# nihofm/volren

Measured on AMD Instinct MI355X. Metric: Msamples/s (pixels x spp / s), volume path tracing, higher is better.
Workload: dtype f32; 1 GPU; BASELINE configs[1] 'c2': smoke.brick, no transfer function, 1024x1024, 1024 spp, seed 42, fov 40; parallelism=1 GPU, 1 fused launch(es)/frame (sample pool budget 64 GiB)

## Files before the change

### volren_amd/csrc/capi.cpp

```cpp
#include "../../include/volren_amd.h"

#include <algorithm>
#include <cmath>
#include <cstring>
#include <filesystem>
#include <functional>
#include <iostream>
#include <stdexcept>
#include <memory>
#include <string>
#include <vector>

#include "imageio.h"
#include "renderer.h"
#include "sharded.h"
#include "vr_device.h"
#include "vr_math_probe.h"

struct vr_renderer {
    vr::RendererHIP impl;
    int device = 0;
};

struct vr_sharded {
// ... 107 lines not shown

int vr_load_envmap(vr_renderer* r, const char* path) {
    NEED(r);
    if (!path) return fail(VR_ERR_ARG, "null path");
    return guard([&] { use_device(r); r->impl.environment = std::make_shared<vr::Environment>(std::string(path)); r->impl.sample = 0; });
}

int vr_load_transferfunc(vr_renderer* r, const char* path) {
    NEED(r);
    if (!path) return fail(VR_ERR_ARG, "null path");
    return guard([&] {
        use_device(r);
        r->impl.transferfunc = std::make_shared<vr::TransferFunction>(std::string(path));
        r->impl.show_environment = false;
        r->impl.sample = 0;
    });
}

static void install_grid(vr_renderer* r, const char* name, const std::shared_ptr<vr::Grid>& grid, int unit_cube) {
    const std::string n = name ? name : "density";
    auto& R = r->impl;
    if (n == "density") {
        R.volume = std::make_shared<vr::Volume>(grid);
        if (unit_cube) { R.density_scale = 1.f; R.scale_and_move_to_unit_cube(); }
    } else {
        if (!R.volume || R.volume->grids.empty()) throw std::runtime_error("set the density grid before '" + n + "'");
        R.volume->update_grid_frame(R.volume->grid_frame_counter, grid, n);
    }
    R.sample = 0;
}

int vr_set_volume_dense(vr_renderer* r, const char* name, const float* voxels, int nx, int ny, int nz, const float* transform, int unit_cube) {
    NEED(r);
    if (!voxels || nx <= 0 || ny <= 0 || nz <= 0) return fail(VR_ERR_ARG, "bad dense grid arguments");
    return guard([&] {
        use_device(r);
        auto g = std::make_shared<vr::DenseGrid>((uint32_t)nx, (uint32_t)ny, (uint32_t)nz, voxels);
        if (transform) memcpy(g->transform.m, transform, 64);
        install_grid(r, name, g, unit_cube);
    });
}

int vr_volume_add_grid_frame_dense(vr_renderer* r, const char* name, const float* voxels, int nx, int ny, int nz, const float* transform) {
    NEED(r);
    if (!voxels || nx <= 0 || ny <= 0 || nz <= 0) return fail(VR_ERR_ARG, "bad dense grid arguments");
    return guard([&] {
        auto g = std::make_shared<vr::DenseGrid>((uint32_t)nx, (uint32_t)ny, (uint32_t)nz, voxels);
        if (transform) memcpy(g->transform.m, transform, 64);
        if (!r->impl.volume) r->impl.volume = std::make_shared<vr::Volume>();
        r->impl.volume->add_grid_frame(g, name ? name : "density");
        r->impl.sample = 0;
    });
}
int vr_volume_update_grid_frame_dense(vr_renderer* r, int frame, const char* name, const float* voxels, int nx, int ny, int nz, const float* transform) {
    NEED(r);
    if (!voxels || nx <= 0 || ny <= 0 || nz <= 0 || frame < 0) return fail(VR_ERR_ARG, "bad dense grid arguments");
    return guard([&] {
        if (!r->impl.volume || (size_t)frame >= r->impl.volume->n_grid_frames()) throw std::out_of_range("vr_volume_update_grid_frame_dense: no such frame");
        auto g = std::make_shared<vr::DenseGrid>((uint32_t)nx, (uint32_t)ny, (uint32_t)nz, voxels);
        if (transform) memcpy(g->transform.m, transform, 64);
        r->impl.volume->update_grid_frame((size_t)frame, g, name ? name : "density");
        r->impl.sample = 0;
    });
}
int vr_volume_n_grid_frames(vr_renderer* r, int* n) {
    NEED(r);
    if (!n) return fail(VR_ERR_ARG, "null output");
    *n = r->impl.volume ? (int)r->impl.volume->n_grid_frames() : 0;
    return VR_OK;
}

int vr_set_volume_dense_f16(vr_renderer* r, const char* name, const uint16_t* voxels, int nx, int ny, int nz, const float* transform, int unit_cube) {
    NEED(r);
    if (!voxels || nx <= 0 || ny <= 0 || nz <= 0) return fail(VR_ERR_ARG, "bad dense grid arguments");
    return guard([&] {
        use_device(r);
        auto g = std::make_shared<vr::DenseGridF16>((uint32_t)nx, (uint32_t)ny, (uint32_t)nz, voxels);
        if (transform) memcpy(g->transform.m, transform, 64);
        install_grid(r, name, g, unit_cube);
    });
}

int vr_set_volume_brick(vr_renderer* r, const char* name, const float* transform, const uint32_t nb[3], const float min_maj[2],
                        const uint32_t* indirection, const uint32_t* range, const uint32_t atlas_dim[3], const uint8_t* atlas,
                        int n_mips, const uint32_t* const* mips, const uint32_t (*mip_dims)[3], int unit_cube) {
    NEED(r);
    if (!nb || !min_maj || !indirection || !range || !atlas_dim || !atlas || n_mips < 0 || n_mips > 3) return fail(VR_ERR_ARG, "bad brick grid arguments");
    return guard([&] {
        use_device(r);
        auto g = std::make_shared<vr::BrickGrid>();
        if (transform) memcpy(g->transform.m, transform, 64);
        g->n_bricks = { nb[0], nb[1], nb[2] };
        g->min_maj = { min_maj[0], min_maj[1] };
        const size_t n = (size_t)nb[0] * nb[1] * nb[2];
        g->indirection = vr::Buf3D<uint32_t>(nb[0], nb[1], nb[2]);
        g->range = vr::Buf3D<uint32_t>(nb[0], nb[1], nb[2]);
        memcpy(g->indirection.data.data(), indirection, n * 4);
        memcpy(g->range.data.data(), range, n * 4);
        if ((atlas_dim[0] % 8) || (atlas_dim[1] % 8) || (atlas_dim[2] % 8)) throw std::runtime_error("atlas dimensions must be multiples of 8");
        g->atlas = vr::Buf3D<uint8_t>(atlas_dim[0], atlas_dim[1], atlas_dim[2]);
        memcpy(g->atlas.data.data(), atlas, g->atlas.data.size());
        uint64_t cnt = 0;
        for (size_t i = 0; i < n; ++i) cnt += (vr::half2float(range[i] & 0xFFFFu) != vr::half2float(range[i] >> 16));
        g->brick_counter = cnt;
        for (int m = 0; m < n_mips; ++m) {
            vr::Buf3D<uint32_t> b(mip_dims[m][0], mip_dims[m][1], mip_dims[m][2]);
            memcpy(b.data.data(), mips[m], b.data.size() * 4);
            g->range_mipmaps.push_back(std::move(b));
        }
        install_grid(r, name, g, unit_cube);
    });
}

int vr_set_envmap(vr_renderer* r, const float* rgb, int w, int h) {
    NEED(r);
    if (!rgb || w <= 0 || h <= 0) return fail(VR_ERR_ARG, "bad envmap arguments");
    return guard([&] { use_device(r); r->impl.environment = std::make_shared<vr::Environment>(rgb, w, h); r->impl.sample = 0; });
}

int vr_set_transferfunc(vr_renderer* r, const float* rgba, int n) {
    NEED(r);
    return guard([&] {
        use_device(r);
        if (n <= 0 || !rgba) { r->impl.transferfunc.reset(); r->impl.sample = 0; return; }
        std::vector<vr::vec4> lut;
        for (int i = 0; i < n; ++i) lut.emplace_back(rgba[4 * i], rgba[4 * i + 1], rgba[4 * i + 2], rgba[4 * i + 3]);
        r->impl.transferfunc = std::make_shared<vr::TransferFunction>(lut);
        r->impl.sample = 0;
    });
}

int vr_set_int(vr_renderer* r, const char* name, int v) {
    NEED(r);
    if (!name) return fail(VR_ERR_ARG, "null name");
    return guard([&] {
        auto& R = r->impl;
        const std::string n = name;
        if (n == "sample") { R.sample = v; R.drop_tile_samples(); }
        else if (n == "sppx") R.sppx = v;
        else if (n == "seed") R.seed = v;
        else if (n == "bounces") R.bounces = v;
        else if (n == "show_environment") R.show_environment = v != 0;
        else if (n == "tonemapping") R.tonemapping = v != 0;
        else if (n == "integrator") R.integrator = v;
        else if (n == "fast_math") R.fast_math = v != 0;
        else if (n == "variance") { if (v < 0 || v > 1) throw std::runtime_error("variance: 0 (off) or 1 (keep the per-pixel second moments)"); R.variance = v; }
        else if (n == "denoise_iterations") {
            if (v < 0 || v > vr::kDenoiseMaxIterations) throw std::runtime_error("denoise_iterations must be in [0, 10]");
            R.denoise_iterations = v;
        }
        else if (n == "coalesce_trace") { R.flush_pending(); R.coalesce_trace = v != 0; }
        else if (n == "majorant_layout") { if (v < -1 || v > 1) throw std::runtime_error("majorant_layout: -1 (per grid, chosen at commit), 0 (linear), 1 (4x4x4-cell blocks)"); R.majorant_layout = v; }
        else if (n == "tf_float_atlas") R.tf_float_atlas = v != 0;
        else if (n == "gpu_encoder") R.gpu_encoder = v != 0;
        else if (n == "sample_pool_mb") { if (v < 16 || v > 65536) throw std::runtime_error("sample_pool_mb must be in [16, 65536] (item indices of a sub-launch are 32-bit: < 2^32 RGBA32F items)"); R.sample_pool_bytes = (size_t)v << 20; }
        else if (n == "launch_target_ms") { if (v < 0) throw std::runtime_error("launch_target_ms must be >= 0 (0 = no sizing by time)"); R.launch_target_ms = v; }
        else if (n == "order_tiles") { if (v < 0 || v > 2) throw std::runtime_error("order_tiles: 0 (never), 1 (tile subsets), 2 (always)"); R.order_tiles = v; }
        else if (n == "grid_frame_counter") {
            if (!R.volume || v < 0 || (size_t)v >= R.volume->n_grid_frames()) throw std::runtime_error("grid_frame_counter out of range");
            R.volume->grid_frame_counter = (size_t)v;
        } else throw std::runtime_error("unknown int parameter: " + n);
    });
}

int vr_get_int(vr_renderer* r, const char* name, int* v) {
    NEED(r);
    if (!name || !v) return fail(VR_ERR_ARG, "null argument");
    return guard([&] {
        auto& R = r->impl;
        const std::string n = name;
        if (n == "sample") *v = R.sample;
        else if (n == "sppx") *v = R.sppx;
        else if (n == "seed") *v = R.seed;
        else if (n == "bounces") *v = R.bounces;
        else if (n == "show_environment") *v = R.show_environment ? 1 : 0;
        else if (n == "tonemapping") *v = R.tonemapping ? 1 : 0;
        else if (n == "integrator") *v = R.integrator;
        else if (n == "fast_math") *v = R.fast_math ? 1 : 0;
        else if (n == "variance") *v = R.variance;
        else if (n == "denoise_iterations") *v = R.denoise_iterations;
        else if (n == "coalesce_trace") *v = R.coalesce_trace ? 1 : 0;
        else if (n == "majorant_layout") *v = R.majorant_layout;
        else if (n == "majorant_blocked") {
            vr::SceneParams P; R.fill_params(P); *v = P.density.maj_blocked;
        }
        else if (n == "kernel_variant" || n == "kernel_variant_reason") {
            vr::SceneParams P; R.fill_params(P);
            int why = 0; const int variant = vr::pathtrace_variant_of(P, &why);
            *v = n == "kernel_variant" ? variant : why;
        }
        else if (n == "env_div_safe") *v = R.environment && R.environment->cdf_div_safe ? 1 : 0;
        else if (n == "env_compact") *v = R.environment && R.environment->envmap_rgbe ? 1 : 0;
        else if (n == "pending_samples") *v = R.pending_samples();
        else if (n == "tf_float_atlas") *v = R.tf_float_atlas ? 1 : 0;
        else if (n == "gpu_encoder") *v = R.gpu_encoder ? 1 : 0;
        else if (n == "sample_pool_mb") *v = (int)(R.sample_pool_bytes >> 20);
        else if (n == "launch_target_ms") *v = R.launch_target_ms;
        else if (n == "order_tiles") *v = R.order_tiles;
        else if (n == "grid_frame_counter") *v = R.volume ? (int)R.volume->grid_frame_counter : 0;
        else if (n == "n_grid_frames") *v = R.volume ? (int)R.volume->n_grid_frames() : 0;
        else if (n == "last_launches") *v = R.last_launches;
        else if (n == "adaptive_rounds") *v = R.adaptive_rounds;
        else if (n == "width") *v = R.resolution.x;
        else if (n == "height") *v = R.resolution.y;
        else throw std::runtime_error("unknown int parameter: " + n);
    });
}

namespace {
struct FloatField { float* ptr; int count; };
FloatField float_field(vr::RendererHIP& R, const std::string& n) {
    if (n == "tonemap_exposure") return { &R.tonemap_exposure, 1 };
    if (n == "tonemap_gamma") return { &R.tonemap_gamma, 1 };
    if (n == "albedo") return { &R.albedo.x, 3 };
    if (n == "phase") return { &R.phase, 1 };
    if (n == "density_scale") return { &R.density_scale, 1 };
    if (n == "emission_scale") return { &R.emission_scale, 1 };
    if (n == "vol_clip_min") return { &R.vol_clip_min.x, 3 };
    if (n == "vol_clip_max") return { &R.vol_clip_max.x, 3 };
    if (n == "cam_pos") return { &R.camera.pos.x, 3 };
    if (n == "cam_dir") return { &R.camera.dir.x, 3 };
    if (n == "cam_up") return { &R.camera.up.x, 3 };
    if (n == "cam_fov") return { &R.camera.fov_degree, 1 };
    if (n == "env_strength") { if (!R.environment) throw std::runtime_error("no environment"); return { &R.environment->strength, 1 }; }
    if (n == "env_transform") { if (!R.environment) throw std::runtime_error("no environment"); return { R.environment->transform.m, 9 }; }
    if (n == "tf_window_left") { if (!R.transferfunc) throw std::runtime_error("no transfer function"); return { &R.transferfunc->window_left, 1 }; }
    if (n == "tf_window_width") { if (!R.transferfunc) throw std::runtime_error("no transfer function"); return { &R.transferfunc->window_width, 1 }; }
    if (n == "volume_transform") { if (!R.volume) throw std::runtime_error("no volume"); return { R.volume->transform.m, 16 }; }
    if (n == "denoise_sigma") return { R.denoise_sigma, 5 };
    if (n == "denoise_alpha") return { &R.denoise_alpha, 1 };
    throw std::runtime_error("unknown float parameter: " + n);
}
}

int vr_set_float(vr_renderer* r, const char* name, const float* values, int count) {
    NEED(r);
    if (!name || !values) return fail(VR_ERR_ARG, "null argument");
    return guard([&] {
        auto& R = r->impl;
        const std::string n = name;
        if (n == "env_rot") {
            if (count != 1) throw std::runtime_error("env_rot takes 1 value");
            if (!R.environment) throw std::runtime_error("no environment");
            R.environment->transform = vr::rotation_axis(values[0], 1);
            return;
        }
        if (n == "albedo" && count == 1) { R.albedo = vr::vec3(values[0]); return; }
        if (n == "denoise_sigma") {
            if (count != 5) throw std::runtime_error("denoise_sigma takes 5 values (colour, normal, depth, coverage, albedo)");
            for (int i = 0; i < 5; ++i)
                if (!(values[i] >= vr::kDenoiseSigmaMin && values[i] <= vr::kDenoiseSigmaMax))
                    throw std::runtime_error("denoise_sigma: every value must be in [2^-60, 2^60]");
        }
        if (n == "denoise_alpha" && count == 1 && !(values[0] >= vr::kTemporalAlphaMin && values[0] <= vr::kTemporalAlphaMax))
            throw std::runtime_error("denoise_alpha must be in [2^-20, 1]");
        const FloatField f = float_field(R, n);
        if (count != f.count) throw std::runtime_error("wrong value count for " + n);
        memcpy(f.ptr, values, sizeof(float) * (size_t)count);
    });
}

int vr_get_float(vr_renderer* r, const char* name, float* values, int count) {
    NEED(r);
    if (!name || !values) return fail(VR_ERR_ARG, "null argument");
    return guard([&] {
        const FloatField f = float_field(r->impl, name);
        if (count != f.count) throw std::runtime_error(std::string("wrong value count for ") + name);
        memcpy(values, f.ptr, sizeof(float) * (size_t)count);
    });
}

int vr_commit(vr_renderer* r) { NEED(r); return guard([&] { use_device(r); r->impl.commit(); }); }
int vr_reset(vr_renderer* r) { NEED(r); return guard([&] { r->impl.reset(); }); }
int vr_scale_and_move_to_unit_cube(vr_renderer* r) { NEED(r); return guard([&] { r->impl.scale_and_move_to_unit_cube(); }); }

int vr_trace(vr_renderer* r) { NEED(r); return guard([&] { use_device(r); r->impl.trace(); }); }
int vr_flush(vr_renderer* r) { NEED(r); return guard([&] { use_device(r); r->impl.flush_pending(); }); }
int vr_render(vr_renderer* r, int spp) { NEED(r); return guard([&] { use_device(r); r->impl.render(spp); }); }

int vr_synchronize(vr_renderer* r) {
    NEED(r);
    return guard([&] {
        use_device(r);
        r->impl.synchronize();
        r->impl.check_watchdog();
    });
}

int vr_last_kernel_ms(vr_renderer* r, double* ms) {
    NEED(r);
    if (!ms) return fail(VR_ERR_ARG, "null argument");
    return guard([&] { use_device(r); *ms = r->impl.last_kernel_ms(); });
}

int vr_last_pathtrace_ms(vr_renderer* r, double* ms) {
    NEED(r);
    if (!ms) return fail(VR_ERR_ARG, "null output");
    return guard([&] { use_device(r); *ms = r->impl.last_pathtrace_ms(); });
}

int vr_framebuffer(vr_renderer* r, float* out) {
    NEED(r);
    if (!out) return fail(VR_ERR_ARG, "null argument");
    return guard([&] { use_device(r); r->impl.download(out); });
}
int vr_render_features(vr_renderer* r, int spp) {
    NEED(r);
    if (vr_device_count() <= 0) return fail(VR_ERR_NO_DEVICE, "no HIP device available (libvolren_amd has no CPU path)");
    return guard([&] { use_device(r); r->impl.render_features(spp); });
}
int vr_features(vr_renderer* r, float* out) {
    NEED(r);
    if (!out) return fail(VR_ERR_ARG, "null argument");
    if (vr_device_count() <= 0) return fail(VR_ERR_NO_DEVICE, "no HIP device available (libvolren_amd has no CPU path)");
    return guard([&] { use_device(r); r->impl.download_features(out); });
}
int vr_variance(vr_renderer* r, float* out) {
    NEED(r);
    if (!out) return fail(VR_ERR_ARG, "null argument");
    if (vr_device_count() <= 0) return fail(VR_ERR_NO_DEVICE, "no HIP device available (libvolren_amd has no CPU path)");
    return guard([&] { use_device(r); r->impl.download_variance(out); });
}
int vr_denoise(vr_renderer* r) {
    NEED(r);
    if (vr_device_count() <= 0) return fail(VR_ERR_NO_DEVICE, "no HIP device available (libvolren_amd has no CPU path)");
    return guard([&] { use_device(r); r->impl.denoise(); });
}
int vr_denoise_temporal(vr_renderer* r) {
    NEED(r);
    if (vr_device_count() <= 0) return fail(VR_ERR_NO_DEVICE, "no HIP device available (libvolren_amd has no CPU path)");
    return guard([&] { use_device(r); r->impl.denoise_temporal(); });
}
int vr_denoise_history_reset(vr_renderer* r) {
    NEED(r);
    if (vr_device_count() <= 0) return fail(VR_ERR_NO_DEVICE, "no HIP device available (libvolren_amd has no CPU path)");
    return guard([&] { use_device(r); r->impl.flush_pending(); r->impl.drop_history(); });
}
int vr_denoise_history(vr_renderer* r, float* rgba_out, float* var_out, float* length_out) {
    NEED(r);
    if (vr_device_count() <= 0) return fail(VR_ERR_NO_DEVICE, "no HIP device available (libvolren_amd has no CPU path)");
    return guard([&] { use_device(r); r->impl.download_history(rgba_out, var_out, length_out); });
}
// ... 277 lines not shown
```

### volren_amd/csrc/renderer.cpp

```cpp
#include "renderer.h"

#include <algorithm>
#include <cfloat>
#include <cmath>
#include <cstdlib>
#include <cstring>
#include <iostream>

#include "vr_adaptive.h"
#include "vr_device.h"
#include "vr_math.h"
#include "vr_probe.h"

namespace vr {

mat3 Camera::view_inverse() const {
    const vec3 f = normalize(dir);
    const vec3 s = normalize(cross(f, up));
    const vec3 u = cross(s, f);
    mat3 r(0.0f);
    r.m[0] = s.x; r.m[1] = s.y; r.m[2] = s.z;
    r.m[3] = u.x; r.m[4] = u.y; r.m[5] = u.z;
    r.m[6] = -f.x; r.m[7] = -f.y; r.m[8] = -f.z;
    return r;
// ... 299 lines not shown
}

static float camera_z(float fov_degree) { return -0.5f / tan_(0.5f * kPi * fov_degree / 180.f); }

void RendererHIP::fill_params(SceneParams& P) {
    if (!volume || volume->grids.empty() || density_grids.empty())
        throw std::runtime_error("RendererHIP::trace: no volume committed");
    if (volume->grid_frame_counter >= density_grids.size())
        throw std::runtime_error("RendererHIP::trace: grid_frame_counter out of range (commit() after changing the volume)");
    memset(&P, 0, sizeof P);
    Uniforms& u = P.u;
    u.bounces = bounces;
    u.seed = seed;
    u.show_environment = show_environment ? 1 : 0;
    copy3(u.cam_pos, camera.pos);
    u.cam_fov = camera.fov_degree;
    const mat3 ct = camera.view_inverse();
    memcpy(u.cam_transform, ct.m, sizeof ct.m);
    P.cam_z = camera_z(camera.fov_degree);
    const auto [bb_min, bb_max] = volume->AABB();
    const auto [mn, maj] = volume->minorant_majorant();
    copy3(u.vol_bb_min, bb_min + vol_clip_min * (bb_max - bb_min));
    copy3(u.vol_bb_max, bb_min + vol_clip_max * (bb_max - bb_min));
    u.vol_minorant = mn * density_scale;
    u.vol_majorant = maj * density_scale;
    u.vol_inv_majorant = 1.f / (maj * density_scale);
    copy3(u.vol_albedo, albedo);
    u.vol_phase_g = phase;
    u.vol_density_scale = density_scale;
    u.vol_emission_scale = emission_scale;
    u.vol_emission_norm = majorant_emission > 0.f ? 1.f / std::fmax(majorant_emission, 1e-4f) : 1.f;
    const BrickGridHIP& density = density_grids[volume->grid_frame_counter];
    const mat4 dt = volume->transform * density.transform;
    const mat4 dti = inverse(dt);
    memcpy(u.vol_density_transform, dt.m, sizeof dt.m);
    memcpy(u.vol_density_inv_transform, dti.m, sizeof dti.m);
    P.density = make_view(density);
    if (volume->grid_frame_counter < emission_grids.size()) {
        const BrickGridHIP& emission = emission_grids[volume->grid_frame_counter];
        const mat4 et = volume->transform * emission.transform;
        const mat4 eti = inverse(et);
        memcpy(u.vol_emission_transform, et.m, sizeof et.m);
        memcpy(u.vol_emission_inv_transform, eti.m, sizeof eti.m);
        const mat4 efd = eti * dt;
        memcpy(P.emission_from_density, efd.m, sizeof efd.m);
        const bool scale_ok = u.vol_density_scale >= 1.0f / 65536.0f && u.vol_density_scale <= 16777216.0f;
        P.paired = (integrator == 0 && environment->cdf_div_safe && scale_ok && density.atlas_paired && density.atlas_paired == emission.atlas_paired) ? 1 : 0;
        if (P.paired) P.density = make_view(density, true, majorant_layout < 0 ? density.maj_blocked : majorant_layout == 1);
        P.emission = make_view(emission, P.paired != 0);
        u.has_emission = 1;
    }
    if (transferfunc) {
        u.use_tf = 1;
        u.tf_size = transferfunc->size();
        u.tf_window_left = transferfunc->window_left;
        u.tf_window_width = transferfunc->window_width;
        P.tf_lut = transferfunc->lut_ssbo->as<float>();
    }
    const mat3 eit = inverse(environment->transform);
    memcpy(u.env_transform, environment->transform.m, sizeof eit.m);
    memcpy(u.env_inv_transform, eit.m, sizeof eit.m);
    u.env_strength = environment->strength;
    u.env_imp_inv_dim[0] = u.env_imp_inv_dim[1] = 1.f / (float)environment->dimension();
    u.env_imp_base_mip = (int)std::floor(std::log2((float)environment->dimension()));
    P.envmap = environment->envmap->as<float>();
    P.env_rgbe = environment->envmap_rgbe ? environment->envmap_rgbe->as<uint32_t>() : nullptr;
    P.env_w = environment->width; P.env_h = environment->height;
    P.env_avg_w = environment->avg_importance; P.env_avg_w_set = 1;
    P.impmap = environment->impmap->as<float>();
    P.imp_dim = (int)environment->dimension();
    P.env_cdf = environment->cdf->as<float>();
    P.env_div_safe = environment->cdf_div_safe ? 1 : 0;
    u.resolution[0] = resolution.x; u.resolution[1] = resolution.y;
    u.integrator = integrator;
}

void RendererHIP::update_majorants(const LaunchInputs& in, BrickGridHIP& g) {
    const MajKey& k = in.maj;
    if (k.density_scale == maj_key_.density_scale && k.tf_version == maj_key_.tf_version &&
        k.wl == maj_key_.wl && k.ww == maj_key_.ww && k.frame == maj_key_.frame && k.blocked == maj_key_.blocked)
        return;
    launch_majorants(in.P, g.range_words->as<uint32_t>(), g.nb, g.mip_off, g.n_mips, g.mshift, g.majorant->as<float>(), g.majorant16->as<uint16_t>(), in.stream);
    VR_HIP(hipGetLastError());
    maj_key_ = k;
}

void RendererHIP::set_tiles(const std::vector<int32_t>& tile_ids) {
    flush_pending();
    tiles_host_ = tile_ids;
    tiles_dev_.reset();
    if (tile_ids.empty()) return;
    if (resolution.x > 0) {
        const int n_all = tile_count(resolution.x, resolution.y);
        for (int32_t t : tile_ids)
            if (t < 0 || t >= n_all) throw std::runtime_error("set_tiles: tile id out of range");
    }
    tiles_dev_ = make_device_buffer(tile_ids.size() * sizeof(int32_t));
    tiles_dev_->upload(tile_ids.data(), tile_ids.size() * sizeof(int32_t));
}

std::vector<int32_t> RendererHIP::costliest_first(const SceneParams& P, const std::vector<int32_t>& tile_ids, int n_tiles) const {
    const Uniforms& u = P.u;
    const int W = u.resolution[0], H = u.resolution[1], tiles_x = vr::tiles_x(W);
    std::vector<int32_t> ids(tile_ids);
    if (ids.empty()) { ids.resize((size_t)n_tiles); for (int i = 0; i < n_tiles; ++i) ids[(size_t)i] = i; }
    auto chord = [&](float px, float py) {
        float d[3] = { (px - 0.5f * (float)W) / (float)H, (py - 0.5f * (float)H) / (float)H, P.cam_z };
        float w[3];
        for (int i = 0; i < 3; ++i) w[i] = u.cam_transform[i] * d[0] + u.cam_transform[3 + i] * d[1] + u.cam_transform[6 + i] * d[2];
        const float len = std::sqrt(w[0] * w[0] + w[1] * w[1] + w[2] * w[2]);
        float t0 = 0.f, t1 = FLT_MAX;
        for (int i = 0; i < 3; ++i) {
            const float inv = 1.f / (w[i] / len);
            const float a = (u.vol_bb_min[i] - u.cam_pos[i]) * inv, b = (u.vol_bb_max[i] - u.cam_pos[i]) * inv;
            t0 = std::fmax(t0, std::fmin(a, b)); t1 = std::fmin(t1, std::fmax(a, b));
        }
        return t1 > t0 ? t1 - t0 : 0.f;
    };
    std::vector<float> cost(ids.size());
    for (size_t k = 0; k < ids.size(); ++k) {
        const float x0 = (float)((ids[k] % tiles_x) * 16), y0 = (float)((ids[k] / tiles_x) * 16);
        const float x1 = std::fmin(x0 + 16.f, (float)W), y1 = std::fmin(y0 + 16.f, (float)H);
        cost[k] = std::fmax(std::fmax(std::fmax(chord(x0, y0), chord(x1, y0)), std::fmax(chord(x0, y1), chord(x1, y1))), chord(0.5f * (x0 + x1), 0.5f * (y0 + y1)));
    }
    std::vector<int32_t> perm(ids.size());
    for (size_t k = 0; k < perm.size(); ++k) perm[k] = (int32_t)k;
    const size_t seg = (ids.size() + 7) / 8;
    for (size_t b = 0; b < ids.size(); b += seg)
        std::stable_sort(perm.begin() + (ptrdiff_t)b, perm.begin() + (ptrdiff_t)std::min(ids.size(), b + seg), [&](int32_t x, int32_t y) { return cost[(size_t)x] > cost[(size_t)y]; });
    std::vector<int32_t> ordered(ids.size());
    for (size_t k = 0; k < ids.size(); ++k) ordered[k] = ids[(size_t)perm[k]];
    return ordered;
}

const int32_t* RendererHIP::tile_order(const SceneParams& P, const std::vector<int32_t>& ids, int n_tiles) {
    const Uniforms& u = P.u;
    uint64_t key = 1469598103934665603ull;
    auto mix = [&key](const void* p, size_t nbytes) { const uint8_t* b = static_cast<const uint8_t*>(p); for (size_t i = 0; i < nbytes; ++i) { key ^= b[i]; key *= 1099511628211ull; } };
    mix(u.cam_pos, sizeof u.cam_pos); mix(u.cam_transform, sizeof u.cam_transform); mix(&P.cam_z, sizeof P.cam_z);
    mix(u.vol_bb_min, sizeof u.vol_bb_min); mix(u.vol_bb_max, sizeof u.vol_bb_max); mix(u.resolution, sizeof u.resolution); mix(&n_tiles, sizeof n_tiles);
    if (!ids.empty()) mix(ids.data(), ids.size() * sizeof(int32_t));
    key = key ? key : 1;
    if (order_dev_ && order_key_ == key && order_dev_->size_bytes() == (size_t)n_tiles * sizeof(int32_t)) return order_dev_->as<int32_t>();
    const std::vector<int32_t> ordered = costliest_first(P, ids, n_tiles);
    ensure_buffer(order_dev_, ordered.size() * sizeof(int32_t));
    order_dev_->upload(ordered.data(), ordered.size() * sizeof(int32_t), stream);
    order_key_ = key;
    return order_dev_->as<int32_t>();
}

bool RendererHIP::LaunchInputs::same_launch_as(const LaunchInputs& o) const {
    return memcmp(&P, &o.P, sizeof P) == 0 && frame == o.frame && maj.density_scale == o.maj.density_scale && maj.tf_version == o.maj.tf_version &&
           maj.wl == o.maj.wl && maj.ww == o.maj.ww && maj.blocked == o.maj.blocked && memcmp(tuning.thr, o.tuning.thr, sizeof tuning.thr) == 0 && tuning.stats == o.tuning.stats &&
           tuning.samples_per_unit == o.tuning.samples_per_unit && tuning.blocks_per_cu == o.tuning.blocks_per_cu && order_tiles == o.order_tiles &&
           launch_target_ms == o.launch_target_ms && fast_math == o.fast_math && variance == o.variance && sample_pool_bytes == o.sample_pool_bytes && stream == o.stream;
}

void RendererHIP::capture(LaunchInputs& in) {
    if (!color) throw std::runtime_error("RendererHIP::trace: no framebuffer (call resize first)");
    if (integrator == 2 && !transferfunc) throw std::runtime_error("RendererHIP::trace: integrator 2 (direct volume rendering) needs a transfer function");
    if (integrator < 0 || integrator > 3) throw std::runtime_error("RendererHIP::trace: unknown integrator");
    if (fast_math && transferfunc) throw std::runtime_error("RendererHIP::trace: fast_math is not available while a transfer function is bound (it misses the 1e-3 bound there); set fast_math 0");
    if (!volume || volume->grids.empty() || density_grids.empty()) throw std::runtime_error("RendererHIP::trace: no volume committed");
    if (volume->grid_frame_counter >= density_grids.size()) throw std::runtime_error("RendererHIP::trace: grid_frame_counter out of range (commit() after changing the volume)");
    {
        BrickGridHIP& g = density_grids[volume->grid_frame_counter];
        const bool build = transferfunc && tf_float_atlas && !g.dense && g.atlas && g.rng && !g.atlas_f32 && !g.atlas_f32_failed;
        const bool drop = (!transferfunc || !tf_float_atlas) && (g.atlas_f32 || g.atlas_f32_failed);
        if (build || drop) flush_pending();
        if (build) {
            try {
                const size_t n_blocks = g.atlas->size_bytes() / kBrickBlockBytes, want = n_blocks * 512u * sizeof(float);
                auto drop_others = [&] { for (BrickGridHIP& other : density_grids) if (&other != &g) other.atlas_f32.reset(); };
                size_t free_b = 0, total_b = 0;
                if (hipMemGetInfo(&free_b, &total_b) != hipSuccess) { (void)hipGetLastError(); free_b = ~(size_t)0; }
                if (want > free_b / 2) drop_others();
                try { g.atlas_f32 = make_device_buffer(want); }
                catch (const std::exception&) { (void)hipGetLastError(); drop_others(); g.atlas_f32 = make_device_buffer(want); }
                launch_decode_atlas(g.rng->as<float>(), g.atlas->as<uint8_t>(), g.atlas_f32->as<float>(), n_blocks, stream);
                VR_HIP(hipGetLastError());
            } catch (const std::exception& e) {
                (void)hipGetLastError();
                g.atlas_f32.reset();
                g.atlas_f32_failed = true;
                std::cerr << "volren_amd: no room for the decoded float atlas (" << (g.atlas->size_bytes() / kBrickBlockBytes * 2048u >> 20) << " MiB): transfer-function taps read the byte atlas (" << e.what() << ")" << std::endl;
            }
        }
        if (drop) { g.atlas_f32.reset(); g.atlas_f32_failed = false; }
    }
    fill_params(in.P);
    in.frame = volume->grid_frame_counter;
    in.maj = MajKey{};
    in.maj.density_scale = density_scale;
    in.maj.tf_version = transferfunc ? transferfunc->version : 0;
    in.maj.wl = transferfunc ? transferfunc->window_left : 0.f;
    in.maj.ww = transferfunc ? transferfunc->window_width : 0.f;
    in.maj.frame = in.frame;
    in.maj.blocked = in.P.density.maj_blocked;
    in.tuning = tuning;
    in.order_tiles = order_tiles; in.launch_target_ms = launch_target_ms; in.fast_math = fast_math ? 1 : 0; in.variance = variance != 0 ? 1 : 0;
    in.sample_pool_bytes = sample_pool_bytes;
    in.stream = stream;
    in.env = environment; in.tf = transferfunc;
    in.keep[0] = environment->envmap; in.keep[1] = environment->impmap; in.keep[2] = environment->cdf;
    in.keep[3] = transferfunc ? transferfunc->lut_ssbo : DeviceBufferPtr();
    in.keep[4] = environment->envmap_rgbe;
}

int RendererHIP::samples_per_launch(const LaunchInputs& in, int n_tiles) const {
    const size_t per_sample = pathtrace_pool_floats(in.tuning, n_tiles, 1) * sizeof(float);
    int per_launch = (int)std::max<size_t>(1, in.sample_pool_bytes / per_sample);
    const size_t lim = (size_t)0xFFFFFFFFu / ((size_t)n_tiles * 256u);
    per_launch = (int)std::min<size_t>((size_t)per_launch, lim > 8 ? lim - 8 : 1);
    if (per_launch > 32) per_launch -= per_launch % 32;
    return per_launch;
}

void RendererHIP::submit_tile_set(const LaunchInputs& in, int first, int n) {
    if (n <= 0) return;
    const int n_tiles = tiles_dev_ ? (int)tiles_host_.size() : tile_count(in.P.u.resolution[0], in.P.u.resolution[1]);
    const bool ordered = in.order_tiles >= 2 || (in.order_tiles == 1 && tiles_dev_);
    const int32_t* tiles = ordered ? tile_order(in.P, tiles_host_, n_tiles) : (tiles_dev_ ? tiles_dev_->as<int32_t>() : nullptr);
    submit(in, first, n, tiles, n_tiles);
}

void RendererHIP::submit(const LaunchInputs& in, int first, int n, const int32_t* tiles, int n_tiles) {
    if (n <= 0) return;
    const SceneParams& P = in.P;
    hipStream_t stream = in.stream;
    const bool has_tf = P.u.use_tf != 0;
    update_majorants(in, density_grids.at(in.frame));
    int per_launch = std::min(samples_per_launch(in, n_tiles), n);
    for (;;) {
        const size_t need = pathtrace_pool_floats(in.tuning, n_tiles, per_launch) * sizeof(float);
        if (pool_ && pool_->size_bytes() >= need) break;
        if (pool_) { VR_HIP(hipStreamSynchronize(stream)); pool_.reset(); }
        try { pool_ = make_device_buffer(need); break; }
        catch (const std::exception&) {
            (void)hipGetLastError();
            if (per_launch <= 1) throw;
            per_launch = std::max(1, per_launch / 2);
            if (per_launch > 32) per_launch -= per_launch % 32;
        }
    }
    if (!workspace_) {
        workspace_ = make_device_buffer(pathtrace_workspace_floats() * sizeof(float));
        if (const char* e = std::getenv("VR_TEST_POISON_WORKSPACE"); e && *e == '1') VR_HIP(hipMemsetAsync(workspace_->get(), 0xFF, workspace_->size_bytes(), stream));
    }
    if (const char* e = std::getenv("VR_TEST_POISON_WORKSPACE"); e && *e == '2') {
        VR_HIP(hipMemsetAsync(workspace_->get(), 0xFF, workspace_->size_bytes(), stream));
        VR_HIP(hipMemsetAsync(pool_->get(), 0xFF, pool_->size_bytes(), stream));
    }
    const int integ = P.u.integrator;
    const bool pt_kernel = !(integ == 3 || (integ == 2 && has_tf));
    const double px_samples = (double)n_tiles * 256.0;
    const uint64_t key = [&] {
        uint64_t h = 1469598103934665603ull;
        auto mix = [&h](const void* p, size_t nbytes) { const uint8_t* b = static_cast<const uint8_t*>(p); for (size_t i = 0; i < nbytes; ++i) { h ^= b[i]; h *= 1099511628211ull; } };
        const Uniforms& u = P.u;
        mix(&u.bounces, sizeof u.bounces); mix(u.vol_albedo, sizeof u.vol_albedo); mix(&u.vol_phase_g, sizeof u.vol_phase_g); mix(&u.vol_density_scale, sizeof u.vol_density_scale);
        mix(&u.use_tf, sizeof u.use_tf); mix(&u.tf_window_left, sizeof u.tf_window_left); mix(&u.tf_window_width, sizeof u.tf_window_width); mix(&u.integrator, sizeof u.integrator);
        mix(&u.has_emission, sizeof u.has_emission); mix(u.resolution, sizeof u.resolution); mix(u.vol_bb_min, sizeof u.vol_bb_min); mix(u.vol_bb_max, sizeof u.vol_bb_max);
        const size_t frame = in.frame; mix(&frame, sizeof frame); mix(&n_tiles, sizeof n_tiles);
        const uint64_t tfv = in.maj.tf_version; mix(&tfv, sizeof tfv);
        return h ? h : 1ull;
    }();
    auto cap_by_rate = [&](int planned) {
        if (in.launch_target_ms <= 0 || rate_samples_per_ms_ <= 0.0) return planned;
        const double cap = rate_samples_per_ms_ * (double)in.launch_target_ms / px_samples;
        int c = cap >= (double)planned ? planned : std::max(1, (int)cap);
        if (c > 32) c -= c % 32;
        return c;
    };
    int probe = 0;
    if (pt_kernel && in.launch_target_ms > 0) {
        harvest_rate(false);
        const bool known = rate_samples_per_ms_ > 0.0 && rate_key_ == key;
        if (!known && px_samples * (double)std::min(per_launch, n) > (double)(1u << 26)) {
            rate_samples_per_ms_ = 0.0;
            probe = (int)std::min<double>(32.0, std::max(1.0, (double)(1u << 24) / px_samples));
            probe = std::min(probe, n);
        } else per_launch = cap_by_rate(per_launch);
    }
    float* moments = nullptr;
    if (in.variance) {
        const size_t bytes = color->size_bytes();
        if (ensure_buffer(moments_, bytes)) {
            VR_HIP(hipMemsetAsync(moments_->get(), 0, bytes, stream));
            if (first > 0) moments_n_ = -1;
        }
        moments = moments_->as<float>();
        moments_n_ = first == 0 ? n : (moments_n_ == first ? first + n : -1);
    } else {
        moments_n_ = -1;
    }
    if (!keep_timing_) {
        VR_HIP(hipEventRecord(ev0_, stream));
        last_launches = 0;
        pt_events_used_ = 0;
    }
    for (int done = 0; done < n;) {
        ++last_launches;
        const int m = probe > 0 ? probe : std::min(per_launch, n - done);
        hipEvent_t eb = nullptr, ee = nullptr;
        if (pt_kernel) {
            while (pt_events_.size() < pt_events_used_ + 2) { hipEvent_t e; VR_HIP(hipEventCreate(&e)); pt_events_.push_back(e); }
            eb = pt_events_[pt_events_used_]; ee = pt_events_[pt_events_used_ + 1];
// ... 432 lines not shown
```

### volren_amd/csrc/vr_device.h

```cpp
#pragma once

#include <hip/hip_runtime.h>
#include <stdint.h>

#include "vr_denoise.h"
#include "vr_scene.h"
#include "vr_temporal.h"
#include "vr_tiles.h"

namespace vr {

struct PathtraceTuning {
    int32_t thr[8] = { 64, 0, 56, 0, 60, 60, 64, 0 };
    unsigned long long* stats = nullptr;
    int32_t samples_per_unit = 0;
    int32_t blocks_per_cu = 0;
};
PathtraceTuning default_tuning();
size_t pathtrace_pool_floats(const PathtraceTuning& T, int32_t n_tiles, int32_t n_samples);
size_t pathtrace_workspace_floats();
void launch_pathtrace(const PathtraceTuning& T, const SceneParams& P, float* fb, float* sample_pool, float* workspace, uint32_t* unit_counter, const int32_t* tiles, int32_t n_tiles,
                      int32_t first_sample, int32_t n_samples, uint32_t* status, hipStream_t stream, bool fast_math = false,
                      hipEvent_t ev_kernel_begin = nullptr, hipEvent_t ev_kernel_end = nullptr,
                      float* moments = nullptr);
constexpr uint32_t kFeatureLostStatus = 4u;
void launch_features(const SceneParams& P, const int32_t* tiles, int32_t n_tiles, int32_t spp, float* out, uint32_t* status, hipStream_t stream);
enum PathtraceVariantReason : int {
    VR_VARIANT_INTEGRATOR = 1,
    VR_VARIANT_ENV_DIVISION = 2,
    VR_VARIANT_DENSITY_SCALE = 4,
    VR_VARIANT_GRID_FORMS = 8
};
int pathtrace_variant_of(const SceneParams& P, int* why);
void launch_denoise_prepare(const float* moments, const float* features, int32_t W, int32_t H, int32_t n, float vscale, const int32_t* counts, float* v, float* guide,
                            hipStream_t stream);
void launch_denoise_atrous(const float* cin, const float* vin, const float* guide, int32_t W, int32_t H, int32_t step, const DenoiseSigma& sg,
                           float* cout, float* vout, hipStream_t stream);
void launch_denoise_temporal(const float* color, float* v, const float* guide, const float* hist_color, const float* hist_record, bool same_cam,
                             const TemporalCamera& cur, const TemporalCamera& prev, int32_t W, int32_t H, float alpha, float* out_color, float* out_record,
                             hipStream_t stream);
void launch_adaptive_error(const float* fb, const float* moments, const int32_t* tiles, const int32_t* counts, int32_t n_tiles, int32_t W, int32_t H, float* out,
                           hipStream_t stream);

void launch_tonemap(float* fb, int32_t w, int32_t h, float exposure, float gamma, hipStream_t stream);

void launch_pack_tiles(const float* fb, int32_t w, int32_t h, const int32_t* tiles, int32_t n_tiles, float* packed, hipStream_t stream);
void launch_unpack_tiles(const float* packed, const int32_t* tiles, int32_t n_tiles, float* fb, int32_t w, int32_t h, hipStream_t stream);
void launch_build_impmap(const float* envmap_rgba, int32_t env_w, int32_t env_h, int32_t dim, float* pyramid, hipStream_t stream);

void launch_build_env_cdf(const float* pyramid, int32_t dim, float* table, uint32_t* unsafe_flag, hipStream_t stream);

void launch_majorants(const SceneParams& P, const uint32_t* range_words_all_mips, const int32_t nb[3], const int32_t mip_off[4], int32_t n_mips,
                      const int32_t mshift[3], float* out_padded, uint16_t* out16_padded, hipStream_t stream);

void launch_encode_ranges(const float* dense, const int32_t dim[3], const int32_t nb[3], uint32_t* range, uint32_t* flag, hipStream_t stream);
void launch_encode_bricks(const float* dense, const int32_t dim[3], const int32_t nb[3], const uint32_t* range, const uint32_t* flag,
                          BrickRec* recs, float* rng, uint8_t* atlas, hipStream_t stream);
void launch_range_mip(const uint32_t* src, const int32_t sdim[3], uint32_t* dst, const int32_t ddim[3], hipStream_t stream);

void launch_pair_atlas(const uint8_t* atlas_density, const uint8_t* atlas_emission, uint8_t* out, size_t n_records, hipStream_t stream);

void launch_decode_atlas(const float* rng, const uint8_t* atlas, float* out, size_t n_records, hipStream_t stream);
void launch_math_probe(int32_t fn, const float* a, const float* b, float* out, int32_t n, hipStream_t stream);
void launch_math_sweep(int32_t fn, uint32_t first, float b, float* out, int32_t n, hipStream_t stream);
void launch_fast_math_sweep(int32_t fn, uint32_t first, float* out, int32_t n, hipStream_t stream);
void launch_probe(const SceneParams& P, int32_t what, int32_t form, const uint32_t* in, float* out, uint32_t n, hipStream_t stream);

}
```

### volren_amd/csrc/vr_launch.hip

```cpp
#include <hip/hip_runtime.h>

#include <algorithm>
#include <cstdlib>
#include <map>
#include <mutex>
#include <stdexcept>
#include <string>

#include "vr_device.h"
#include "vr_pathtrace.h"

namespace vr {

template <int INTEGRATOR>
__global__ void __launch_bounds__(256)
item_kernel(const SceneParams P, float* __restrict__ sbuf, const LaunchDesc D) {
    const uint32_t per_unit = (uint32_t)(D.spu * 64);
    const uint32_t g = blockIdx.x * 256u + threadIdx.x;
    const uint32_t u = g / per_unit, item = g - u * per_unit;
    if (u >= D.n_units) return;
    const WorkUnit wu = make_unit(D, P.u.resolution[0], u, sbuf);
    if ((int32_t)item >= wu.n_items) return;
    const int32_t px = wu.px0 + (int32_t)(item & 7u), py = wu.py0 + (int32_t)((item >> 3) & 7u);
    if (px >= P.u.resolution[0] || py >= P.u.resolution[1]) return;
    float L[4];
    if (INTEGRATOR == 2) dvr_sample(P, px, py, wu.first_sample + (int32_t)(item >> 6), L);
    else raymarch_path_sample(P, px, py, wu.first_sample + (int32_t)(item >> 6), L);
    reinterpret_cast<float4*>(sbuf)[wu.base + item] = pack4(L);
}

template <bool MOMENTS>
__global__ void __launch_bounds__(256)
accumulate_kernel(const float* __restrict__ sbuf, float* __restrict__ fb, float* __restrict__ moments, const int32_t* __restrict__ tiles, int32_t n_tiles,
                  int32_t W, int32_t H, int32_t first_sample, int32_t n_samples, int32_t spu) {
    const TilePixel q = wave_tiled_pixel(tiles ? tiles[blockIdx.x] : (int32_t)blockIdx.x, threadIdx.x, W);
    if (q.px >= W || q.py >= H) return;
    float4* texel = reinterpret_cast<float4*>(fb) + (size_t)q.py * W + q.px;
    float4* mtexel = MOMENTS ? reinterpret_cast<float4*>(moments) + (size_t)q.py * W + q.px : nullptr;
    float acc[4] = { 0.0f, 0.0f, 0.0f, 0.0f }, S[4] = { 0.0f, 0.0f, 0.0f, 0.0f };
    if (first_sample > 1) {
        unpack4(*texel, acc);
        if (MOMENTS) unpack4(*mtexel, S);
    }
    const float4* sb = reinterpret_cast<const float4*>(sbuf);
    for (int32_t k = 0; k < n_samples; ++k) {
        const int32_t chunk = k / spu, sl = k - chunk * spu;
        float L[4];
        unpack4(sb[pool_slot<size_t>((size_t)chunk, n_tiles, (size_t)blockIdx.x, (uint32_t)q.sub, spu, (size_t)sl, (uint32_t)q.lane)], L);
        const float a = 1.0f / (float)(first_sample + k);
        for (int32_t c = 0; c < 4; ++c) {
            const float x = sanitize(L[c]);
            const float mu = acc[c], mu1 = mix_(mu, x, a);
            if (MOMENTS) S[c] = mix_(S[c], (x - mu) * (x - mu1), a);
            acc[c] = mu1;
        }
    }
    *texel = pack4(acc);
    if (MOMENTS) *mtexel = pack4(S);
}

template <bool TF>
__global__ void __launch_bounds__(256)
features_kernel(const SceneParams P, const int32_t* __restrict__ tiles, int32_t spp, float* __restrict__ out, uint32_t* __restrict__ status) {
    const int32_t W = P.u.resolution[0], H = P.u.resolution[1];
    const TilePixel q = wave_tiled_pixel(tiles ? tiles[blockIdx.x] : (int32_t)blockIdx.x, threadIdx.x, W);
    if (q.px >= W || q.py >= H) return;
    float f[8];
    if (!feature_pixel<TF>(P, q.px, q.py, spp, f)) atomicOr(status, kFeatureLostStatus);
    float4* o = reinterpret_cast<float4*>(out) + 2u * ((size_t)q.py * W + q.px);
    o[0] = pack4(f);
    o[1] = pack4(f + 4);
}
void launch_features(const SceneParams& P, const int32_t* tiles, int32_t n_tiles, int32_t spp, float* out, uint32_t* status, hipStream_t stream) {
    if (n_tiles <= 0 || spp <= 0) return;
    if (P.u.use_tf) hipLaunchKernelGGL(features_kernel<true>, dim3((unsigned)n_tiles), dim3(256), 0, stream, P, tiles, spp, out, status);
    else hipLaunchKernelGGL(features_kernel<false>, dim3((unsigned)n_tiles), dim3(256), 0, stream, P, tiles, spp, out, status);
}

constexpr int32_t kMaxSamplesPerUnit = 8;
static int32_t samples_per_unit(const PathtraceTuning& T, int variant) { return T.samples_per_unit > 0 ? T.samples_per_unit : ((variant == 1 || variant == 2 || variant == 4) ? 4 : kMaxSamplesPerUnit); }
constexpr int kPtVariants = 5;

PathtraceTuning default_tuning() {
    static std::once_flag once;
    static int32_t env_spu = 0, env_blocks = 0;
    std::call_once(once, [] {
        if (const char* e = getenv("VR_SPU")) env_spu = std::max(1, atoi(e));
        if (const char* e = getenv("VR_BLOCKS_PER_CU")) env_blocks = std::max(0, atoi(e));
    });
    PathtraceTuning T;
    T.samples_per_unit = env_spu;
    T.blocks_per_cu = env_blocks;
    return T;
}

size_t pathtrace_pool_floats(const PathtraceTuning& T, int32_t n_tiles, int32_t n_samples) {
    size_t padded = 0;
    for (int variant = 0; variant < kPtVariants; ++variant) {
        const int32_t spu = std::min(n_samples, samples_per_unit(T, variant));
        padded = std::max(padded, (size_t)((n_samples + spu - 1) / spu) * (size_t)spu);
    }
    return padded * (size_t)n_tiles * 4u * 64u * 4u;
}

extern "C" {
#define VR_PT_DECL(N) \
    int vr_pt_occupancy_##N(int tf, int stats); \
    void vr_pt_launch_##N(int tf, int stats, unsigned grid, hipStream_t stream, const void* P, float* sbuf, float* cold_ws, const void* D, const void* S, uint32_t* status, unsigned long long* stats_buf);
VR_PT_DECL(0) VR_PT_DECL(1) VR_PT_DECL(2) VR_PT_DECL(3) VR_PT_DECL(4) VR_PT_DECL(0_fast) VR_PT_DECL(1_fast) VR_PT_DECL(2_fast) VR_PT_DECL(3_fast) VR_PT_DECL(4_fast)
#undef VR_PT_DECL
}
typedef int (*PtOccupancy)(int, int);
typedef void (*PtLaunch)(int, int, unsigned, hipStream_t, const void*, float*, float*, const void*, const void*, uint32_t*, unsigned long long*);
static const PtOccupancy kPtOccupancy[2][kPtVariants] = { { vr_pt_occupancy_0, vr_pt_occupancy_1, vr_pt_occupancy_2, vr_pt_occupancy_3, vr_pt_occupancy_4 },
                                                          { vr_pt_occupancy_0_fast, vr_pt_occupancy_1_fast, vr_pt_occupancy_2_fast, vr_pt_occupancy_3_fast, vr_pt_occupancy_4_fast } };
static const PtLaunch kPtLaunch[2][kPtVariants] = { { vr_pt_launch_0, vr_pt_launch_1, vr_pt_launch_2, vr_pt_launch_3, vr_pt_launch_4 },
                                                    { vr_pt_launch_0_fast, vr_pt_launch_1_fast, vr_pt_launch_2_fast, vr_pt_launch_3_fast, vr_pt_launch_4_fast } };

int pathtrace_variant_of(const SceneParams& P, int* why) {
    const bool scale_ok = P.u.vol_density_scale >= 1.0f / 65536.0f && P.u.vol_density_scale <= 16777216.0f;
    int reason = 0;
    if (P.u.integrator != 0) reason |= VR_VARIANT_INTEGRATOR;
    if (!P.env_div_safe) reason |= VR_VARIANT_ENV_DIVISION;
    if (!scale_ok) reason |= VR_VARIANT_DENSITY_SCALE;
    int variant;
    if (reason) variant = 3;
    else if (P.u.has_emission) {
        const bool mixed = P.density.dense || P.emission.dense || (VR_PAIRED_ATLAS && !P.paired);
        if (mixed) reason |= VR_VARIANT_GRID_FORMS;
        variant = mixed ? 3 : (P.density.maj_blocked ? 4 : 2);
    } else variant = P.density.dense ? 1 : 0;
    if (why) *why = reason;
    return variant;
}
static int pathtrace_variant(const SceneParams& P) {
    int why = 0;
    const int variant = pathtrace_variant_of(P, &why);
    if (why & (VR_VARIANT_ENV_DIVISION | VR_VARIANT_DENSITY_SCALE)) {
        static std::once_flag once;
        std::call_once(once, [&] {
            fprintf(stderr, "volren_amd: note: this scene is rendered by the run-time kernel variant (slower; results unchanged):%s%s\n",
                    (why & VR_VARIANT_ENV_DIVISION) ? " the environment's warp table has thresholds below 2^-76 (vr_get_int env_div_safe = 0);" : "",
                    (why & VR_VARIANT_DENSITY_SCALE) ? " the density scale lies outside [2^-16, 2^24];" : "");
        });
    }
    return variant;
}

static int resident_blocks(const PathtraceTuning& T, int mode, int variant, bool tf, bool stats) {
    int dev = 0, cus = 0;
    if (hipGetDevice(&dev) != hipSuccess) return 1024;
    static std::mutex mu;
    static std::map<uint32_t, std::pair<int, int>> cache;
    const uint32_t key = ((uint32_t)dev << 8) | ((uint32_t)mode << 5) | ((uint32_t)variant << 2) | (tf ? 2u : 0u) | (stats ? 1u : 0u);
    std::pair<int, int> v;
    {
        std::lock_guard<std::mutex> lock(mu);
        auto it = cache.find(key);
        if (it == cache.end()) {
            if (hipDeviceGetAttribute(&cus, hipDeviceAttributeMultiprocessorCount, dev) != hipSuccess || cus <= 0) cus = 256;
            it = cache.emplace(key, std::make_pair(cus, kPtOccupancy[mode][variant](tf, stats))).first;
        }
        v = it->second;
    }
    const int per_cu = T.blocks_per_cu > 0 ? T.blocks_per_cu : v.second;
    return std::min(v.first * per_cu, kMaxWorkgroups * 4 / kWgWaves);
}

size_t pathtrace_workspace_floats() { return kColdMainFloats + (size_t)kMaxWorkgroups * 4u * (size_t)kColdSideWaveFloats; }

void launch_pathtrace(const PathtraceTuning& T, const SceneParams& P, float* fb, float* sample_pool, float* workspace, uint32_t* unit_counter, const int32_t* tiles, int32_t n_tiles,
                      int32_t first_sample, int32_t n_samples, uint32_t* status, hipStream_t stream, bool fast_math, hipEvent_t ev_kernel_begin, hipEvent_t ev_kernel_end,
                      float* moments) {
    if (n_tiles <= 0 || n_samples <= 0) return;
    SchedParams S;
    for (int i = 0; i < ST_COUNT; ++i) S.thr[i] = T.thr[i];
    LaunchDesc D;
    D.tiles = tiles; D.n_tiles = n_tiles; D.first_sample = first_sample; D.n_samples = n_samples;
    const int variant = pathtrace_variant(P);
    D.spu = std::min(n_samples, samples_per_unit(T, variant));
    const int32_t chunks = (n_samples + D.spu - 1) / D.spu;
    if ((uint64_t)chunks * (uint64_t)n_tiles * 4u * (uint64_t)(D.spu * 64) > 0xFFFFFFFFull)
        throw std::runtime_error("launch_pathtrace: " + std::to_string(n_tiles) + " tiles x " + std::to_string(n_samples) + " samples do not fit the 32-bit item index of one launch");
    D.n_units = (uint32_t)chunks * (uint32_t)n_tiles * 4u;
    D.chunks = (uint32_t)chunks;
    D.seg_len = (D.n_units + kQueueSegments - 1u) / kQueueSegments;
    D.unit_counter = unit_counter;
    S.max_iters = kMaxIdleIters;
    if (S.thr[ST_COLLIDE] <= 0) S.thr[ST_COLLIDE] = (P.u.use_tf || P.u.has_emission) ? 32 : 24;
    const bool tf = P.u.use_tf != 0, stats = T.stats != nullptr;
    const int mode = fast_math ? 1 : 0;
    const int blocks = resident_blocks(T, mode, variant, tf, stats);
    const uint32_t groups_needed = (D.n_units + (uint32_t)kWgWaves - 1u) / (uint32_t)kWgWaves;
    const dim3 grid((unsigned)std::min<uint32_t>((uint32_t)blocks, groups_needed > 0 ? groups_needed : 1u)), block(256);
    if (P.u.integrator == 3 || (P.u.integrator == 2 && P.u.use_tf)) {
        const uint64_t items = (uint64_t)D.n_units * (uint64_t)(D.spu * 64);
        const auto integrate = P.u.integrator == 2 ? item_kernel<2> : item_kernel<3>;
        hipLaunchKernelGGL(integrate, dim3((unsigned)((items + 255) / 256)), block, 0, stream, P, sample_pool, D);
    } else {
        (void)hipMemsetAsync(unit_counter, 0, kQueueSegments * sizeof(uint32_t), stream);
        if (ev_kernel_begin) (void)hipEventRecord(ev_kernel_begin, stream);
        kPtLaunch[mode][variant](tf, stats, grid.x, stream, &P, sample_pool, workspace, &D, &S, status, T.stats);
        if (ev_kernel_end) (void)hipEventRecord(ev_kernel_end, stream);
    }
    const auto accumulate = moments ? accumulate_kernel<true> : accumulate_kernel<false>;
    hipLaunchKernelGGL(accumulate, dim3((unsigned)n_tiles), block, 0, stream, sample_pool, fb, moments, tiles, n_tiles, P.u.resolution[0], P.u.resolution[1],
                       first_sample, n_samples, D.spu);
}

}
```

### volren_amd/csrc/vr_pathtrace.h

```cpp
#pragma once

#include <hip/hip_runtime.h>

#include <type_traits>

#include "vr_tiles.h"
#include "vr_trace.h"

namespace vr {

struct SchedParams {
    int32_t thr[ST_COUNT];
    uint32_t max_iters;
};

constexpr uint32_t kQueueSegments = 8u;
constexpr uint32_t kMaxIdleIters = 1u << 26;
constexpr uint64_t kMaxIdleTicks = 7200000000ull;
struct LaunchDesc {
    const int32_t* tiles;
    int32_t n_tiles, first_sample, n_samples, spu;
    uint32_t n_units, chunks, seg_len;
    uint32_t* unit_counter;
};
// ... 411 lines not shown

#ifndef VR_STATS_LEVEL
#define VR_STATS_LEVEL 2
#endif
    constexpr bool STATS_T = STATS && VR_STATS_LEVEL >= 2;
    const unsigned long long t_begin_rt = STATS_T ? __builtin_amdgcn_s_memrealtime() : 0ull;
    uint32_t iters = 0u, idle_iters = 0u;
    if (VR_PRIO_EVENTS != VR_PRIO_HOT) __builtin_amdgcn_s_setprio(VR_PRIO_HOT);
    uint32_t t_last = (uint32_t)__builtin_readcyclecounter(), t_elapsed = 0u;
    __shared__ uint32_t lds_stat[STATS ? kWgWaves * 32 : 1];
    if (STATS) { if (lane < 32) lds_stat[wave * 32 + lane] = 0u; __builtin_amdgcn_wave_barrier(); }
    auto stat_add = [&](int i, uint32_t n) __attribute__((always_inline)) { if (lane == 0) lds_stat[wave * 32 + i] += n; };
    uint32_t t_blk = 0u;
    const unsigned long long t_start = STATS_T ? __builtin_readcyclecounter() : 0ull;
#ifndef VR_STAT_SCHED
#define VR_STAT_SCHED 0
#endif
#if VR_STAT_SCHED
    uint32_t t_tail = 0u;
    bool have_tail = false;
#endif
    unsigned long long t_exhausted = 0ull;
#define VR_STAT(ST, N) do { if (STATS) { stat_add(2 * (ST), 1u); stat_add(2 * (ST) + 1, (uint32_t)(N)); if (STATS_T) t_blk = (uint32_t)__builtin_readcyclecounter(); } } while (0)
#define VR_STAT_END(ST) do { if (STATS_T) { stat_add(18 + (ST), (uint32_t)__builtin_readcyclecounter() - t_blk); } } while (0)
#define VR_PUSH(QI, CNT, COND, SLOTV) do { \
        const uint64_t m_ = wave_ballot(COND); \
        if (m_) { if (COND) q[(QI) * NS + (CNT) + (int32_t)lane_rank(m_)] = (uint8_t)(SLOTV); (CNT) += popc(m_); } \
    } while (0)

#ifndef VR_READY_FIFO
#define VR_READY_FIFO 0
#endif
#if VR_READY_FIFO
#define VR_PUSH_READY(COND, SLOTV) do { \
        const uint64_t m_ = wave_ballot(COND); \
        if (m_) { if (COND) { int32_t p_ = rdy_head + cnt_ready + (int32_t)lane_rank(m_); p_ = p_ >= NS ? p_ - NS : p_; q[Q_READY * NS + p_] = (uint8_t)(SLOTV); } cnt_ready += popc(m_); } \
    } while (0)
#else
#define VR_PUSH_READY(COND, SLOTV) VR_PUSH(Q_READY, cnt_ready, COND, SLOTV)
#endif
#define VR_ROUTE_ST(BS, STV) do { \
         \
        const int32_t s_ = (BS) >= 0 ? (STV) : -1; \
        VR_PUSH_READY((uint32_t)(s_ - ST_MARCH) < 2u, BS);                         \
        VR_PUSH(Q_NEE, cnt_nee, s_ == ST_NEE, BS); \
        VR_PUSH(Q_POST, cnt_post, s_ == ST_POSTNEE, BS); \
        VR_PUSH(Q_ESC, cnt_esc, s_ == ST_ESCAPE, BS); \
        const bool lost_ = s_ == ST_BEGIN || s_ > ST_ESCAPE || s_ < -1; \
        if (wave_ballot(lost_)) { if (lost_) atomicOr(event_args().status, 2u); } \
        const int32_t free0_ = cnt_free; \
        VR_PUSH(Q_FREE, cnt_free, s_ == ST_NEW || lost_, BS); \
        if (cnt_free != free0_) { idle_iters = 0u; t_elapsed = 0u; }           \
    } while (0)
#define VR_ROUTE(BS) VR_ROUTE_ST(BS, l.state)
#define VR_ROUTE_B(BS) VR_ROUTE_ST(BS, b.state)

    for (;;) {
        ++iters;
        bool give_up = ++idle_iters > kMaxIdleIters;
        if ((iters & 1023u) == 0u) {
            const uint32_t now = (uint32_t)__builtin_readcyclecounter(), d = now - t_last;
            t_last = now;
            if (d < (1u << 31)) t_elapsed += d >> 10;
            give_up = give_up || t_elapsed > (uint32_t)(kMaxIdleTicks >> 10);
        }
        if (give_up) {
            if (lane == 0) atomicOr(event_args().status, 1u);
            break;
        }
#if VR_STAT_SCHED
        uint32_t t_sec = STATS_T ? (uint32_t)__builtin_readcyclecounter() : 0u;
        if (STATS_T && have_tail) stat_add(26 + 4, t_sec - t_tail);
#define VR_SECTION(K) do { if (STATS_T) { const uint32_t n_ = (uint32_t)__builtin_readcyclecounter(); stat_add(26 + (K), n_ - t_sec); t_sec = n_; } } while (0)
#else
#define VR_SECTION(K) do { } while (0)
#endif
        {
            const uint64_t idle = wave_ballot(slot < 0);
            const int32_t take = min(popc(idle), cnt_ready);
            if (take > 0) {
                if (STATS) stat_add(14, 1u);
                if (slot < 0) {
                    const int32_t r = (int32_t)lane_rank(idle);
                    if (r < take) {
#if VR_READY_FIFO
                        int32_t p_ = rdy_head + r; p_ = p_ >= NS ? p_ - NS : p_;
                        slot = q[Q_READY * NS + p_]; hs.load_resume(l, slot, kWorld ? event_args().P.u.vol_density_inv_transform : nullptr);
#else
                        slot = q[Q_READY * NS + cnt_ready - 1 - r]; hs.load_resume(l, slot, kWorld ? event_args().P.u.vol_density_inv_transform : nullptr);
#endif
                        if (emission_on && !l.shadow) {
                            if (kLazyEm && l.first) { l.ethr = v3{ 1.0f, 1.0f, 1.0f }; l.eL = hs.load_first_radiance(slot); }
                            else { const ColdT c = VR_COLD(slot); l.ethr = ld3(c, C_THR); l.eL = ld3(c, C_L); }
                        }
                    }
                }
                cnt_ready -= take;
#if VR_READY_FIFO
                rdy_head += take; rdy_head = rdy_head >= NS ? rdy_head - NS : rdy_head;
#endif
            }
        }
        VR_SECTION(0);
#if !VR_STAT_SCHED
        if (STATS_T) { stat_add(26, (uint32_t)popc(wave_ballot(slot >= 0))); stat_add(27, (uint32_t)cnt_ready); stat_add(28, (uint32_t)cnt_nee); stat_add(29, (uint32_t)cnt_post); stat_add(30, (uint32_t)cnt_esc); stat_add(31, (uint32_t)cnt_free); }
#endif
#ifndef VR_HOT_PAIRS
#define VR_HOT_PAIRS 4
#endif
#ifndef VR_HOT_PAIRS_TF_EMISSION
#define VR_HOT_PAIRS_TF_EMISSION 4
#endif
        constexpr int kHotPairs = (K::tf && K::emission == 1) ? (VR_HOT_PAIRS_TF_EMISSION < VR_HOT_PAIRS ? VR_HOT_PAIRS_TF_EMISSION : VR_HOT_PAIRS) : VR_HOT_PAIRS;

#ifndef VR_HOT_PAIR_MIN
#define VR_HOT_PAIR_MIN 44
#endif
#ifndef VR_DRAIN
#define VR_DRAIN 0
#endif
#ifndef VR_BALLOT_VALID
#define VR_BALLOT_VALID 1
#endif
        const uint64_t holds_path = wave_ballot(slot >= 0);
#ifndef VR_CLEAN_FORMS
#define VR_CLEAN_FORMS VR_CLEAN_FLAG
#endif
#ifndef VR_CLEAN_FORMS_TF_EMISSION
#define VR_CLEAN_FORMS_TF_EMISSION 1
#endif
        constexpr bool kCleanForms = VR_CLEAN_FORMS && ((K::tf && K::emission == 1) ? VR_CLEAN_FORMS_TF_EMISSION != 0 : true);
        const bool all_clean = kCleanForms && (holds_path & wave_ballot((int32_t)f2u(l.far) < 0)) == 0ull;
#ifndef VR_EARLY_MARCH
#define VR_EARLY_MARCH 0
#endif
        constexpr bool kEarlyMarch = VR_EARLY_MARCH != 0 && VR_MARCH_SPECULATIVE && VR_MARCH_STEPS == 2 && K::global == 0 && !K::tf && K::emission == 0 && !K::maj_reuse && maj_lds_cells<K>() == 0;
        MarchIO pre;
        march_idle(pre); pre.maj1 = pre.maj2 = 0u;
        auto hot_pair = [&](auto clean_tag, const int hot_rep_, const int n_copies_) __attribute__((always_inline)) -> bool {
            constexpr bool CLEAN = decltype(clean_tag)::value;
#if VR_BALLOT_VALID
            if (hot_rep_ > 0 && popc_s(holds_path & wave_ballot((uint32_t)(l.state - ST_MARCH) < 2u)) < (VR_DRAIN && exhausted ? 1 : VR_HOT_PAIR_MIN)) return false;
#else
            if (hot_rep_ > 0 && popc(wave_ballot(slot >= 0 && (uint32_t)(l.state - ST_MARCH) < 2u)) < VR_HOT_PAIR_MIN) return false;
#endif
            if (STATS_T) t_blk = (uint32_t)__builtin_readcyclecounter();
            const bool is_m = slot >= 0 && l.state == ST_MARCH;
#if VR_MARCH_SPECULATIVE
            MarchIO mio;
            if (kEarlyMarch && hot_rep_ > 0) mio = pre;
            else {
            march_idle(mio);
            if (is_m) march_prep<K::dense, K::majb, CLEAN>(l, P, mio);
            if constexpr (kMajCells > 0) march_load_lds<K::tf, MajT>(P, mio, lds_maj, maj_first);
            else if constexpr (K::maj_reuse) march_load_reuse<K::tf>(P, mio, l);
            else march_load<K::tf>(P, mio);
#if VR_MARCH_LOADS_PINNED
            asm volatile("" : "+v"(mio.maj1), "+v"(mio.maj2));
#endif
            }
            if (is_m) march_finish<K::tf, K::maj_reuse, CLEAN>(l, P, mio);
#else
            for (int32_t k = 0; k < 2; ++k)
                if (slot >= 0 && l.state == ST_MARCH) do_march<K::tf, K::dense, K::majb>(l, P);
#endif
            if (STATS) { const int32_t nm = popc(wave_ballot(is_m)); if (nm) { stat_add(2 * ST_MARCH, 1u); stat_add(2 * ST_MARCH + 1, (uint32_t)nm); } }
            if (STATS_T) { const uint32_t t_now = (uint32_t)__builtin_readcyclecounter(); stat_add(18 + ST_MARCH, t_now - t_blk); t_blk = t_now; }
#if VR_DIAG_PAD_VALU > 0
            {
                float pad_ = l.t;
#pragma unroll
                for (int k_ = 0; k_ < VR_DIAG_PAD_VALU; ++k_) asm volatile("v_add_f32 %0, 1.0, %0" : "+v"(pad_));
                asm volatile("" :: "v"(pad_));
            }
#endif
#if VR_DIAG_PAD_SLEEP > 0
            __builtin_amdgcn_s_sleep(VR_DIAG_PAD_SLEEP);
#endif
            const bool is_c = slot >= 0 && l.state == ST_COLLIDE;
#if VR_BALLOT_VALID
            const int32_t n_c = popc(holds_path & wave_ballot(l.state == ST_COLLIDE));
            const int32_t n_m = popc(holds_path & wave_ballot(l.state == ST_MARCH));
#else
            const int32_t n_c = popc(wave_ballot(is_c));
            const int32_t n_m = popc(wave_ballot(slot >= 0 && l.state == ST_MARCH));
#endif
            const bool run_c = n_c > 0 && n_c >= min(VR_THR_COLLIDE, (n_c + n_m + 1) >> 1);
            if (kEarlyMarch) {
                CollideIO<K> cio;
                collide_idle<K>(cio);
                if (run_c) {
                    if (is_c) collide_prep<K, CLEAN>(l, P, P, cio);
                    collide_load<K>(P, P, cio);
                }
                const bool early = hot_rep_ + 1 < n_copies_;
                if (early) {
                    const bool spec = run_c && is_c;
                    Hot ls = l;
                    ls.mipq = spec ? (l.mipq > 8 ? l.mipq - 8 : 0) : l.mipq;
                    march_idle(pre);
                    if (slot >= 0 && (l.state == ST_MARCH || spec)) march_prep<K::dense, K::majb, CLEAN>(ls, P, pre);
                    march_load<K::tf>(P, pre);
                    if (VR_EARLY_MARCH == 1) asm volatile("" : "+v"(cio.d.raw), "+v"(cio.d.rmin), "+v"(cio.d.rdiff));
                }
                if (run_c) {
                    if (is_c) { ColdT c = VR_COLD(slot); collide_finish<K, ColdT, true>(l, c, P, P, cio, P.tf_lut); }
                    if (STATS) { stat_add(2 * ST_COLLIDE, 1u); stat_add(2 * ST_COLLIDE + 1, (uint32_t)n_c); }
                }
                if (early) asm volatile("" : "+v"(pre.maj1), "+v"(pre.maj2));
            } else
            if (run_c) {
                CollideIO<K> cio;
                collide_idle<K>(cio);
                const SceneParams& PE = VR_EMISSION_BY_POINTER && K::emission != 0 ? event_args().P : P;
#ifndef VR_COLLIDE_BY_POINTER
#define VR_COLLIDE_BY_POINTER 1
#endif
                const SceneParams& PF = (VR_COLLIDE_BY_POINTER && K::tf && (K::global == 2 || K::emission == 1)) ? event_args().P : P;
                if (is_c) collide_prep<K, CLEAN>(l, PF, PE, cio);
                collide_load<K>(PF, PE, cio);
                if (is_c) {
                    ColdT c = VR_COLD(slot);
                    if (lut_in_lds) collide_finish<K, ColdT, true>(l, c, PF, PE, cio, lds_lut);
                    else collide_finish<K, ColdT, true>(l, c, PF, PE, cio, PF.tf_lut);
                }
                if (STATS) { stat_add(2 * ST_COLLIDE, 1u); stat_add(2 * ST_COLLIDE + 1, (uint32_t)n_c); }
            }
            __builtin_amdgcn_s_waitcnt(0x0F70);
            if (STATS_T) stat_add(18 + ST_COLLIDE, (uint32_t)__builtin_readcyclecounter() - t_blk);
            return true;
        };
        if constexpr (kCleanForms) {
            if (all_clean) {
#pragma unroll
                for (int hot_rep_ = 0; hot_rep_ < kHotPairs; ++hot_rep_) if (!hot_pair(std::true_type{}, hot_rep_, kHotPairs)) break;
            } else hot_pair(std::false_type{}, 0, 1);
        } else {
#pragma unroll
            for (int hot_rep_ = 0; hot_rep_ < kHotPairs; ++hot_rep_) if (!hot_pair(std::false_type{}, hot_rep_, kHotPairs)) break;
        }
        VR_SECTION(1);
        {
            const int32_t ps = (slot >= 0 && l.state != ST_MARCH && l.state != ST_COLLIDE) ? l.state : -1;
            if (wave_ballot(ps >= 0)) {
                if (STATS) stat_add(15, 1u);
                if (ps >= 0) {
                    hs.save_marched(l, slot);
                    if (emission_on && !l.shadow) {
                        if (kLazyEm && l.first) hs.save_first_radiance(l.eL, slot);
                        else { ColdT c = VR_COLD(slot); st3(c, C_L, l.eL); }
                    }
                }
                VR_PUSH(Q_NEE, cnt_nee, ps == ST_NEE, slot);
                VR_PUSH(Q_POST, cnt_post, ps == ST_POSTNEE, slot);
                VR_PUSH(Q_ESC, cnt_esc, ps == ST_ESCAPE, slot);
                if (ps >= 0) slot = -1;
            }
        }
        VR_SECTION(2);
        int32_t n;
        const int32_t n_live = popc(wave_ballot(slot >= 0)) + cnt_ready;
        const bool hungry = n_live < VR_THR_HUNGRY;
        const int32_t c_new = exhausted ? 0 : cnt_free;
        int32_t big = c_new;
        if (cnt_nee > big) big = cnt_nee;
        if (cnt_post > big) big = cnt_post;
        if (cnt_esc > big) big = cnt_esc;
        const bool drain_all = VR_DRAIN && exhausted;
        const bool want_new = c_new > 0 && (c_new >= VR_THR_NEW || (hungry && c_new == big));
        const bool want_nee = cnt_nee > 0 && (cnt_nee >= VR_THR_NEE || (hungry && (cnt_nee == big || drain_all)));
        const bool want_post = cnt_post > 0 && (cnt_post >= VR_THR_POST || (hungry && (cnt_post == big || drain_all)));
        const bool want_esc = cnt_esc > 0 && (cnt_esc >= VR_THR_ESC || (hungry && (cnt_esc == big || drain_all)));
        if (want_new || want_nee || want_post || want_esc) {
#if VR_BATCH_REGS
            Hot b;
#else
            const int32_t my_slot = slot;
            const float my_majorant = l.majorant;
            if (my_slot >= 0) { hs.save(l, my_slot); if (emission_on && !l.shadow) { ColdT c = VR_COLD(my_slot); st3(c, C_L, l.eL); } }
            __builtin_amdgcn_wave_barrier();
            Hot& b = l;
#endif
            if (VR_PRIO_EVENTS != VR_PRIO_HOT) __builtin_amdgcn_s_setprio(VR_PRIO_EVENTS);
            if (want_esc) {
                n = min(64, cnt_esc);
                VR_STAT(ST_ESCAPE, n);
                int32_t bs = -1;
                if (lane < n) { bs = q[Q_ESC * NS + cnt_esc - 1 - lane]; hs.load(b, bs); if (kLazyEm && b.first) b.eL = hs.load_first_radiance(bs); }
                if (kItemInRegs) b.item = item_fetch(banks, lane, bs);
                if constexpr (kColdRegs) {
                    ColdLocal c;
                    cold_clear(c);
                    cold_fetch<kColdEscR>(c, cb, lane, bs);
                    if (lane < n) {
                        const KernelArgs& E = event_args();
                        WorkUnit w; w.out = E.sbuf;
                        do_escape<ColdLocal, false>(b, c, E.P, w);
                    }
                } else
                if (lane < n) {
                    const ColdT c = VR_COLD(b.first ? 0 : bs);
                    const KernelArgs& E = event_args();
                    WorkUnit w; w.out = E.sbuf;
                    do_escape<ColdT, kItemInRegs, kLazyEm, kWorld>(b, c, E.P, w);
                }
                cnt_esc -= n;
                VR_ROUTE_B(bs);
                VR_STAT_END(ST_ESCAPE);
            }
            if (want_post) {
                n = min(64, cnt_post);
                VR_STAT(ST_POSTNEE, n);
                int32_t bs = -1;
                if (lane < n) { bs = q[Q_POST * NS + cnt_post - 1 - lane]; hs.load(b, bs); }
                if (kShleInRegs) b.shle = shle_fetch(banks, lane, bs);
                if (kItemInRegs) b.item = item_fetch(banks, lane, bs);
                if constexpr (kColdRegs) {
                    ColdLocal c;
                    cold_clear(c);
                    cold_fetch<kColdPostR>(c, cb, lane, bs);
                    if (lane < n) {
                        const KernelArgs& E = event_args();
                        WorkUnit w; w.out = E.sbuf;
                        do_postnee<K, ColdLocal, false, false>(b, c, E.P, w);
                        hs.save(b, bs);
                    }
                    cold_store<kColdPostW, false>(cb, cold_stage(stage, lane, bs, false), lane, c);
                } else
                if (lane < n) {
                    ColdT c = VR_COLD(bs);
                    const KernelArgs& E = event_args();
                    WorkUnit w; w.out = E.sbuf;
                    do_postnee<K, ColdT, kShleInRegs, kItemInRegs>(b, c, E.P, w);
                    hs.save(b, bs);
                }
                cnt_post -= n;
                VR_ROUTE_B(bs);
                VR_STAT_END(ST_POSTNEE);
            }
            if (want_new) {
                if (cursor == (uint32_t)wu.n_items) {
                    const KernelArgs& E = event_args();
                    uint32_t j = 0xFFFFFFFFu;
                    while (seg_tries < kQueueSegments) {
                        const uint32_t k = ((blockIdx.x & (kQueueSegments - 1u)) + seg_tries) & (kQueueSegments - 1u);
                        const uint32_t lo = k * E.D.seg_len, hi = min(lo + E.D.seg_len, E.D.n_units);
                        uint32_t v = 0xFFFFFFFFu;
                        if (lo < hi) { if (lane == 0) v = atomicAdd(E.D.unit_counter + k, 1u); v = __builtin_amdgcn_readfirstlane(v); }
                        if (lo < hi && v < hi - lo) { j = lo + v; break; }
                        ++seg_tries;
                    }
                    if (j == 0xFFFFFFFFu) { exhausted = true; if (STATS_T) t_exhausted = __builtin_amdgcn_s_memrealtime(); }
                    else { wu = make_unit(E.D, E.P.u.resolution[0], j, nullptr); cursor = 0u; idle_iters = 0u; t_elapsed = 0u; }
                }
                n = min(min(64, cnt_free), (int32_t)((uint32_t)wu.n_items - cursor));
// ... 95 lines not shown
```

### volren_amd/csrc/vr_pathtrace.hip

```cpp
#include <hip/hip_runtime.h>
#include <stdint.h>

#ifndef VR_PT_VARIANT
#error "compile with -DVR_PT_VARIANT=0..4"
#endif
#ifdef VR_FAST_MATH
#define vr vr_fastmath
#define VR_PT_SUFFIX _fast
#else
#define VR_PT_SUFFIX
#endif

#if VR_PT_VARIANT == 3 && !defined(VR_BATCH_REGS)
#define VR_BATCH_REGS 0
#endif
#if VR_PT_VARIANT == 3 && !defined(VR_HOT_PAIRS)
#define VR_HOT_PAIRS 1
#endif
#if VR_PT_VARIANT == 3 && !defined(VR_CLEAN_FORMS)
#define VR_CLEAN_FORMS 0
#endif
#include "vr_pathtrace.h"

namespace vr {

#if VR_PT_VARIANT == 0
template <bool TF> using Cfg = TraceCfg<TF, 0, 0, 0>;
#elif VR_PT_VARIANT == 1
template <bool TF> using Cfg = TraceCfg<TF, 0, 0, 1>;
#elif VR_PT_VARIANT == 2
template <bool TF> using Cfg = TraceCfg<TF, 0, 1, 0>;
#elif VR_PT_VARIANT == 4
template <bool TF> using Cfg = TraceCfg<TF, 0, 1, 0, 1>;
#else
template <bool TF> using Cfg = TraceCfg<TF, 2, 2, 2, 2>;
#endif

typedef void (*PtKernel)(const KernelArgs);
static PtKernel pick(bool tf, bool stats) {
    return tf ? (stats ? pathtrace_kernel<Cfg<true>, true> : pathtrace_kernel<Cfg<true>, false>)
              : (stats ? pathtrace_kernel<Cfg<false>, true> : pathtrace_kernel<Cfg<false>, false>);
}

}

#define VR_PT_CAT3(a, b, c) a##b##c
#define VR_PT_CAT(a, b, c) VR_PT_CAT3(a, b, c)

extern "C" int VR_PT_CAT(vr_pt_occupancy_, VR_PT_VARIANT, VR_PT_SUFFIX)(int tf, int stats) {
    int per_cu = 0;
    if (hipOccupancyMaxActiveBlocksPerMultiprocessor(&per_cu, vr::pick(tf != 0, stats != 0), 64 * vr::kWgWaves, 0) != hipSuccess || per_cu <= 0) per_cu = 16 / vr::kWgWaves;
    return per_cu;
}
extern "C" void VR_PT_CAT(vr_pt_launch_, VR_PT_VARIANT, VR_PT_SUFFIX)(int tf, int stats, unsigned grid, hipStream_t stream, const void* P, float* sbuf, float* cold_ws,
                                                                       const void* D, const void* S, uint32_t* status, unsigned long long* stats_buf) {
    vr::KernelArgs A;
    A.P = *static_cast<const vr::SceneParams*>(P);
    A.D = *static_cast<const vr::LaunchDesc*>(D);
    A.S = *static_cast<const vr::SchedParams*>(S);
    A.sbuf = sbuf; A.cold_ws = cold_ws; A.status = status; A.stats = stats_buf;
    hipLaunchKernelGGL(vr::pick(tf != 0, stats != 0), dim3(grid), dim3(64 * vr::kWgWaves), 0, stream, A);
}
```

### volren_amd/csrc/vr_scene.h

```cpp
#pragma once

#include <stdint.h>

namespace vr {

struct alignas(16) BrickRec { uint32_t slot; float rmin; float rdiff; uint32_t range; };

#if defined(__HIPCC__)
#define VR_SCENE_HD __host__ __device__ inline
#else
#define VR_SCENE_HD inline
#endif

VR_SCENE_HD int32_t ceil_log2(uint32_t v) { int32_t s = 0; while (s < 31 && (1u << s) < v) ++s; return s; }
VR_SCENE_HD uint32_t majorant_level_offset(uint32_t k, uint32_t mip) { const uint32_t s = 9u - 3u * mip; return ((0x49u >> s) << s) << (k - 6u); }
VR_SCENE_HD size_t majorant_padded_cells(uint32_t k) { return (size_t)majorant_level_offset(k, 3u) + ((size_t)1 << (k - 9u)); }
VR_SCENE_HD size_t majorant_table_cells(uint32_t k) { return majorant_padded_cells(k) + 1u; }
#ifndef VR_MAJORANT_BLOCKED
#define VR_MAJORANT_BLOCKED 0
#endif
VR_SCENE_HD uint32_t majorant_cell_index(uint32_t cx, uint32_t cy, uint32_t cz, uint32_t sx, uint32_t sy, uint32_t mip, bool blocked) {
    if (blocked && mip <= 1u)
        return (((((cz >> 2) << (sy - 2u)) + (cy >> 2)) << (sx - 2u)) + (cx >> 2)) * 64u + (((cz & 3u) << 4) | ((cy & 3u) << 2) | (cx & 3u));
    return (((cz << sy) + cy) << sx) + cx;
}

#ifndef VR_BRICK_HEADERS
#define VR_BRICK_HEADERS 1
#endif
constexpr uint32_t kBrickLineVoxels = VR_BRICK_HEADERS ? 120u : 128u, kBrickLineHeader = VR_BRICK_HEADERS ? 8u : 0u;
constexpr uint32_t kBrickBlockBytes = VR_BRICK_HEADERS ? 640u : 512u;
VR_SCENE_HD uint32_t brick_voxel_line(uint32_t off) { return VR_BRICK_HEADERS ? (off * 547u) >> 16 : off >> 7; }
VR_SCENE_HD uint32_t brick_voxel_byte(uint32_t off) { return off + kBrickLineHeader * (brick_voxel_line(off) + 1u); }

#ifndef VR_PAIRED_ATLAS
#define VR_PAIRED_ATLAS 1
#endif
constexpr uint32_t kPairLineVoxels = 56u, kPairLineHeader = 16u, kPairBlockBytes = 1280u;
VR_SCENE_HD uint32_t pair_voxel_line(uint32_t off) { return (off * 1171u) >> 16; }
VR_SCENE_HD uint32_t pair_voxel_byte(uint32_t off, uint32_t c) { const uint32_t l = pair_voxel_line(off); return l * 128u + kPairLineHeader + 2u * (off - l * kPairLineVoxels) + c; }

VR_SCENE_HD size_t dense_blocked_index(uint32_t x, uint32_t y, uint32_t z, uint32_t blocks_x, uint32_t blocks_y) {
    return (((size_t)(z >> 2) * blocks_y + (y >> 2)) * blocks_x + (x >> 2)) * 64u + (((z & 3u) << 4) | ((y & 3u) << 2) | (x & 3u));
}

#ifndef VR_ENV_TEXEL_FLOATS
#define VR_ENV_TEXEL_FLOATS 3
#endif
constexpr int32_t kEnvTexelFloats = VR_ENV_TEXEL_FLOATS;
constexpr int32_t kEnvCdfBlockFloats = 16, kEnvCdfLastBlockFloats = 32, kEnvCdfLastChildFloats = 7, kEnvCdfLastChild0 = 4;
VR_SCENE_HD size_t env_cdf_pair_base(int32_t s, int32_t p) { return (size_t)s + (((size_t)1 << (2 * s)) * ((((size_t)1) << (4 * p)) - 1)) / 15; }
VR_SCENE_HD size_t env_cdf_last_pair_floats(int32_t s, int32_t n_pairs) {
    const size_t f = (size_t)kEnvCdfBlockFloats * env_cdf_pair_base(s, n_pairs - 1);
    return (f + (size_t)kEnvCdfLastBlockFloats - 1u) / (size_t)kEnvCdfLastBlockFloats * (size_t)kEnvCdfLastBlockFloats;
}
VR_SCENE_HD size_t env_cdf_index(int32_t top, int32_t k, uint32_t x, uint32_t y) {
    const int32_t s = (top & 1) ? 0 : 1;
    if (k < s) return 0;
    const int32_t kk = k - s, p = kk >> 1, ku = 2 * p + s, n_pairs = (top + 1 - s) / 2;
    const uint32_t c = 2u * (y & 1u) + (x & 1u);
    if (p == n_pairs - 1) {
        const size_t base = env_cdf_last_pair_floats(s, n_pairs);
        if (kk & 1) return base + (size_t)kEnvCdfLastBlockFloats * (((size_t)(y >> 1) << ku) + (x >> 1)) + (size_t)kEnvCdfLastChild0 + (size_t)kEnvCdfLastChildFloats * c;
        return base + (size_t)kEnvCdfLastBlockFloats * (((size_t)y << ku) + x);
    }
    const size_t blk = env_cdf_pair_base(s, p);
    if (kk & 1) return (size_t)kEnvCdfBlockFloats * (blk + ((size_t)(y >> 1) << ku) + (x >> 1)) + 3u + 3u * c;
    return (size_t)kEnvCdfBlockFloats * (blk + ((size_t)y << ku) + x);
}
VR_SCENE_HD size_t env_cdf_table_floats(int32_t top) {
    if (top < 1) return kEnvCdfBlockFloats;
    const int32_t s = (top & 1) ? 0 : 1, n_pairs = (top + 1 - s) / 2, ku = 2 * (n_pairs - 1) + s;
    return env_cdf_last_pair_floats(s, n_pairs) + ((size_t)kEnvCdfLastBlockFloats << (2 * ku));
}

struct GridView {
    const BrickRec* bricks;
    const uint8_t* atlas;
    const float* majorant;
    const uint16_t* majorant16;
    const float* atlas_f32;
    const float* rng;
    int32_t nb[3];
    int32_t mshift[3];
    float mlim[3];
    int32_t n_mips;
    int32_t maj_blocked;
    int32_t maj_outside;
    const uint16_t* dense;
    int32_t dim[3];
    int32_t dblk[2];
};

struct Uniforms {
    int32_t bounces, seed, show_environment;
    float cam_pos[3], cam_fov, cam_transform[9];
    float vol_bb_min[3], vol_bb_max[3];
    float vol_minorant, vol_majorant, vol_inv_majorant;
    float vol_albedo[3], vol_phase_g, vol_density_scale, vol_emission_scale, vol_emission_norm;
    float vol_density_transform[16], vol_density_inv_transform[16];
    float vol_emission_transform[16], vol_emission_inv_transform[16];
    uint32_t tf_size; float tf_window_left, tf_window_width;
    float env_transform[9], env_inv_transform[9], env_strength, env_imp_inv_dim[2];
    int32_t env_imp_base_mip;
    int32_t resolution[2];
    int32_t use_tf, has_emission, integrator;
};

struct SceneParams {
    Uniforms u;
    GridView density;
    GridView emission;
    float emission_from_density[16];
    int32_t paired;
    const float* tf_lut;
    const float* envmap;
    const uint32_t* env_rgbe;
    int32_t env_w, env_h;
    float env_avg_w;
    int32_t env_avg_w_set;
    const float* impmap;
    int32_t imp_dim;
    const float* env_cdf;
    int32_t env_div_safe;
    float cam_z;
};

}
```

### volren_amd/csrc/vr_trace.h

```cpp
#pragma once

#include "vr_math.h"
#include "vr_scene.h"

#if defined(VR_HOST_TRACE) && !defined(__HIP_DEVICE_COMPILE__)
namespace vr {
enum TraceClass : int32_t { TR_MAJORANT = 0, TR_TAP = 1, TR_ENV_WARP = 2, TR_ENV_TEXEL = 3 };
void host_trace(int32_t cls, const void* table, size_t a, size_t b);
}
#define VR_TRACE(CLS, TABLE, A, B) ::vr::host_trace((CLS), (TABLE), (size_t)(A), (size_t)(B))
#else
#define VR_TRACE(CLS, TABLE, A, B) do { } while (0)
#endif

namespace vr {

enum LaneState : int32_t {
    ST_NEW = 0,
    ST_BEGIN = 1,
    ST_MARCH = 2,
    ST_COLLIDE = 3,
    ST_NEE = 4,
    ST_POSTNEE = 5,
    ST_ESCAPE = 6,
    ST_DONE = 7,
    ST_COUNT = 8
};

#ifndef VR_MARCH_STEPS
#define VR_MARCH_STEPS 2
#endif
#ifndef VR_MAJ_REUSE
#define VR_MAJ_REUSE 0
#endif
template <bool TF, int GLOBAL, int EMISSION, int DENSE, int MAJB = 0>
struct TraceCfg {
    static constexpr bool tf = TF;
    static constexpr int global = GLOBAL, emission = EMISSION, dense = DENSE, majb = MAJB;
    static constexpr int edense = EMISSION == 1 ? DENSE : 2;
    static constexpr int pair_d = (VR_PAIRED_ATLAS && EMISSION == 1 && DENSE == 0) ? 1 : 0, pair_e = pair_d ? 2 : 0;
    static constexpr bool maj_reuse = VR_MARCH_STEPS == 2 && (VR_MAJ_REUSE == 2 || (VR_MAJ_REUSE == 1 && MAJB == 1));
};

#ifndef VR_WORLD_SLOT
#define VR_WORLD_SLOT 1
#endif
#ifndef VR_WORLD_SLOT_EMISSION
#define VR_WORLD_SLOT_EMISSION 0
#endif
template <class K> constexpr bool world_slot() { return VR_WORLD_SLOT != 0 && !K::tf && K::global == 0 && (K::emission == 0 || VR_WORLD_SLOT_EMISSION != 0); }

struct WorkUnit {
    int32_t px0, py0;
    int32_t first_sample;
    int32_t n_items;
    uint32_t base;
    float* out;
};

static_assert(ST_POSTNEE == ST_ESCAPE - 1, "segment_end_state");
VR_HD int32_t segment_end_state(int32_t shadow) { return ST_ESCAPE - shadow; }

struct Hot {
    uint32_t seed;
    v3 ipos, idir, ri;
    v3 wpos, wdir;
    float t, far, tau, majorant, Tr;
    int32_t mipq;
    int32_t shadow;
    int32_t state;
    int32_t first;
    v3 ethr, eL;
    v3 shle;
    uint32_t item;
    int32_t maj_idx;
    uint32_t maj_raw;
};
struct FirstStash { v3 dir; uint32_t item; };
#ifndef VR_C_STRIDE
#define VR_C_STRIDE 16
#endif
enum ColdField : int32_t {
    C_POS = 0, C_SHPDF = 3, C_THR = 4, C_FPL = 7, C_L = 8, C_NPATHS = 11, C_DIR = 12, C_FP = 15,
    C_SIDE = 16, C_SHLE = 16, C_ITEM = 19,
    C_COL = 20,
    C_COUNT = 23, C_STRIDE = VR_C_STRIDE, C_SIDE_STRIDE = 4
};
template <class Cold> VR_HD v3 ld3(const Cold& c, int32_t f) { return v3{ c.ld(f), c.ld(f + 1), c.ld(f + 2) }; }
template <class Cold> VR_HD void st3(Cold& c, int32_t f, v3 v) { c.st(f, v.x); c.st(f + 1, v.y); c.st(f + 2, v.z); }
template <class Cold> VR_HD uint32_t ldu(const Cold& c, int32_t f) { return f2u(c.ld(f)); }
struct Quad { v3 a; float b; };
template <class Cold> VR_HD Quad ld4(const Cold& c, int32_t f3, int32_t f1) { return Quad{ ld3(c, f3), c.ld(f1) }; }
template <class Cold> VR_HD void stu(Cold& c, int32_t f, uint32_t v) { c.st(f, u2f(v)); }

#ifndef VR_TEA_UNROLL
#define VR_TEA_UNROLL 32
#endif
VR_HD uint32_t tea32(uint32_t v0, uint32_t v1) {
    uint32_t s0 = 0u;
#pragma unroll VR_TEA_UNROLL
    for (int n = 0; n < 32; ++n) {
        s0 += 0x9e3779b9u;
        v0 += ((v1 << 4) + 0xA341316Cu) ^ (v1 + s0) ^ ((v1 >> 5) + 0xC8013EA4u);
        v1 += ((v0 << 4) + 0xAD90777Du) ^ (v0 + s0) ^ ((v0 >> 5) + 0x7E95761Eu);
    }
    return v0;
}
VR_HD float rng(uint32_t& s) {
    s = s * 1664525u + 1013904223u;
    return (float)(s & 0x00FFFFFFu) * (1.0f / 16777216.0f);
}
VR_HD void rng_skip9(uint32_t& s) {
    constexpr uint32_t a = 1664525u, c = 1013904223u;
    constexpr uint32_t a2 = a * a, a4 = a2 * a2, a8 = a4 * a4, a9 = a8 * a;
    constexpr uint32_t g2 = a + 1u, g4 = g2 * (a2 + 1u), g8 = g4 * (a4 + 1u), g9 = g8 * a + 1u;
    s = a9 * s + g9 * c;
}

template <int DENSE>
VR_HD bool grid_is_dense(const GridView& g) { return DENSE == 2 ? g.dense != nullptr : DENSE == 1; }
struct TapAddr { uint32_t cell, off; bool in; };
struct TapData { float rmin, rdiff; uint32_t raw; };
template <int DENSE = 2>
VR_HD TapAddr tap_addr(const GridView& g, int32_t x, int32_t y, int32_t z) {
    TapAddr a;
    const bool nonneg = (x | y | z) >= 0;
    if (grid_is_dense<DENSE>(g)) {
        a.in = nonneg && (uint32_t)x < (uint32_t)g.dim[0] && (uint32_t)y < (uint32_t)g.dim[1] && (uint32_t)z < (uint32_t)g.dim[2];
#if defined(VR_WHATIF_WRAP)
        x &= VR_WHATIF_WRAP - 1; y &= VR_WHATIF_WRAP - 1; z &= VR_WHATIF_WRAP - 1;
#endif
        a.cell = (mul24((uint32_t)z >> 2, (uint32_t)g.dblk[1]) + ((uint32_t)y >> 2)) * (uint32_t)g.dblk[0] + ((uint32_t)x >> 2);
        a.off = (((uint32_t)z & 3u) << 4) | (((uint32_t)y & 3u) << 2) | ((uint32_t)x & 3u);
    } else {
        const uint32_t bx = (uint32_t)x >> 3, by = (uint32_t)y >> 3, bz = (uint32_t)z >> 3;
        a.in = nonneg && bx < (uint32_t)g.nb[0] && by < (uint32_t)g.nb[1] && bz < (uint32_t)g.nb[2];
        a.cell = mul24(mul24(bz, (uint32_t)g.nb[1]) + by, (uint32_t)g.nb[0]) + bx;
        a.off = (((uint32_t)z & 7u) << 6) | (((uint32_t)y & 7u) << 3) | ((uint32_t)x & 7u);
    }
    if (!a.in) { a.cell = 0u; a.off = 0u; }
    return a;
}
#ifndef VR_TAP_LINE_INDEX
#define VR_TAP_LINE_INDEX 1
#endif
template <int DENSE = 2, int PAIR = 0>
VR_HD TapData tap_load(const GridView& g, TapAddr a) {
    TapData d;
    VR_TRACE(1, g.atlas ? (const void*)g.atlas : (const void*)g.dense, a.cell, a.off);
    if (PAIR != 0) {
        const uint32_t line = pair_voxel_line(a.off);
#if VR_TAP_LINE_INDEX
        const uint8_t* ln = g.atlas + ((size_t)(a.cell * (kPairBlockBytes / 128u) + line) << 7);
#else
        const uint8_t* ln = g.atlas + ((size_t)a.cell * kPairBlockBytes + (size_t)(line * 128u));
#endif
        const float* rec = reinterpret_cast<const float*>(ln) + (PAIR == 2 ? 2 : 0);
#if defined(VR_TAP_NT) && defined(__HIP_DEVICE_COMPILE__)
        d.rmin = __builtin_nontemporal_load(rec); d.rdiff = __builtin_nontemporal_load(rec + 1);
        d.raw = __builtin_nontemporal_load(ln + (kPairLineHeader + 2u * (a.off - line * kPairLineVoxels) + (PAIR == 2 ? 1u : 0u)));
#else
        d.rmin = rec[0]; d.rdiff = rec[1];
        d.raw = ln[kPairLineHeader + 2u * (a.off - line * kPairLineVoxels) + (PAIR == 2 ? 1u : 0u)];
#endif
        return d;
    }
    if (grid_is_dense<DENSE>(g)) {
        d.rmin = 0.0f; d.rdiff = 0.0f;
#if defined(VR_DENSE_TAP_NT) && defined(__HIP_DEVICE_COMPILE__)
        d.raw = __builtin_nontemporal_load(g.dense + ((size_t)a.cell * 64u + a.off));
#else
        d.raw = g.dense[(size_t)a.cell * 64u + a.off];
#endif
    } else {
#if VR_BRICK_HEADERS
        const uint32_t line = brick_voxel_line(a.off);
#if VR_TAP_LINE_INDEX
        const uint8_t* ln = g.atlas + ((size_t)(a.cell * (kBrickBlockBytes / 128u) + line) << 7);
#else
        const uint8_t* ln = g.atlas + ((size_t)a.cell * kBrickBlockBytes + (size_t)(line * 128u));
#endif
        const float* rec = reinterpret_cast<const float*>(ln);
        d.rmin = rec[0]; d.rdiff = rec[1];
        d.raw = ln[kBrickLineHeader + a.off - line * kBrickLineVoxels];
#else
        const float* rec = g.rng + 2u * (size_t)a.cell;
        d.rmin = rec[0]; d.rdiff = rec[1];
        d.raw = g.atlas[(size_t)a.cell * 512u + a.off];
#endif
#if defined(VR_DIAG_EXTRA_RNG) && defined(__HIP_DEVICE_COMPILE__)
        {
            const uint32_t n_ = (uint32_t)g.nb[0] * (uint32_t)g.nb[1] * (uint32_t)g.nb[2];
            uint32_t c_ = a.cell * 2654435761u; c_ = c_ % n_;
            float x_ = g.rng[2u * (size_t)c_];
            asm volatile("" :: "v"(x_));
        }
#endif
    }
    return d;
}
template <int DENSE = 2>
VR_HD float tap_value(const GridView& g, TapData d, bool in) {
    const float v = grid_is_dense<DENSE>(g) ? half2float(d.raw) : d.rmin + unorm8(d.raw) * d.rdiff;
    return in ? v : 0.0f;
}
template <int DENSE = 2>
VR_HD float brick_value(const GridView& g, int32_t x, int32_t y, int32_t z) {
    const TapAddr a = tap_addr<DENSE>(g, x, y, z);
    return tap_value<DENSE>(g, tap_load<DENSE>(g, a), a.in);
}
#ifndef VR_MAJ_OUTSIDE_CELL
#define VR_MAJ_OUTSIDE_CELL 1
#endif
#ifndef VR_MAJ_LEVEL_TEST
#define VR_MAJ_LEVEL_TEST 0
#endif
#ifndef VR_CLEAN_FLAG
#define VR_CLEAN_FLAG 1
#endif
constexpr float kCleanBound = 1048576.0f;
VR_HD float seg_far(const Hot& h) { return VR_CLEAN_FLAG ? abs_(h.far) : h.far; }
VR_HD bool seg_clean(const Hot& h) { return VR_CLEAN_FLAG ? (int32_t)f2u(h.far) >= 0 : false; }
VR_HD int32_t cvt_flr(float x) {
#if defined(__HIP_DEVICE_COMPILE__)
    int32_t r; asm("v_cvt_flr_i32_f32 %0, %1" : "=v"(r) : "v"(x)); return r;
#else
    return (int32_t)floor_(x);
#endif
}
template <int DENSE = 2, int MAJB = 2, bool CLEAN = false>
VR_HD int32_t majorant_index(const GridView& g, v3 ipos, int32_t mip) {
    const uint32_t sh = 3u + (uint32_t)mip;
    const uint32_t sx = (uint32_t)g.mshift[0] - (uint32_t)mip, sy = (uint32_t)g.mshift[1] - (uint32_t)mip;
    const uint32_t off = majorant_level_offset((uint32_t)(g.mshift[0] + g.mshift[1] + g.mshift[2]), (uint32_t)mip);
    const bool blocked = MAJB == 2 ? g.maj_blocked != 0 : MAJB == 1;
    if (CLEAN && VR_MAJ_OUTSIDE_CELL) {
        const uint32_t bx = (uint32_t)cvt_flr(ipos.x) >> sh, by = (uint32_t)cvt_flr(ipos.y) >> sh, bz = (uint32_t)cvt_flr(ipos.z) >> sh;
        const uint32_t sz = (uint32_t)g.mshift[2] - (uint32_t)mip;
        const bool inside = ((bx >> sx) | (by >> sy) | (bz >> sz)) == 0u;
        return inside ? (int32_t)(off + majorant_cell_index(bx, by, bz, sx, sy, (uint32_t)mip, blocked)) : g.maj_outside;
    }
    const bool inside = (VR_MAJ_LEVEL_TEST ? (mip <= g.n_mips) : true) & (ipos.x >= 0.0f) & (ipos.x < g.mlim[0]) & (ipos.y >= 0.0f) & (ipos.y < g.mlim[1]) & (ipos.z >= 0.0f) & (ipos.z < g.mlim[2]);
    const uint32_t bx = (uint32_t)(int32_t)ipos.x >> sh, by = (uint32_t)(int32_t)ipos.y >> sh, bz = (uint32_t)(int32_t)ipos.z >> sh;
    return inside ? (int32_t)(off + majorant_cell_index(bx, by, bz, sx, sy, (uint32_t)mip, blocked)) : (VR_MAJ_OUTSIDE_CELL ? g.maj_outside : -1);
}
template <bool TF>
VR_HD uint32_t majorant_fetch(const GridView& g, int32_t idx) {
    const int32_t i = VR_MAJ_OUTSIDE_CELL ? idx : (idx < 0 ? 0 : idx);
#if VR_MAJ_OUTSIDE_CELL && defined(__clang__)
    __builtin_assume(i >= 0);
#endif
    VR_TRACE(0, g.majorant16, i, TF ? 4 : 2);
    return TF ? f2u(g.majorant[i]) : (uint32_t)g.majorant16[i];
}
template <bool TF>
VR_HD float majorant_value(const SceneParams& P, uint32_t raw) { return TF ? u2f(raw) : P.u.vol_density_scale * half2float(raw); }
template <bool TF>
VR_HD float majorant_of(const SceneParams& P, int32_t idx, uint32_t raw) {
    const float m = majorant_value<TF>(P, raw);
    return VR_MAJ_OUTSIDE_CELL ? m : (idx >= 0 ? m : 0.0f);
}
template <bool TF, int DENSE = 2, int MAJB = 2>
VR_HD float majorant_at(const SceneParams& P, v3 ipos, int32_t mip) {
    const int32_t idx = majorant_index<DENSE, MAJB>(P.density, ipos, mip);
    return majorant_of<TF>(P, idx, majorant_fetch<TF>(P.density, idx));
}
VR_HD int32_t nan_guard(int32_t ix, float fx, float fy, float fz) {
#if defined(__HIP_DEVICE_COMPILE__)
    return ((fx != fx) | (fy != fy) | (fz != fz)) ? -1 : ix;
#else
    return ix;
#endif
}

struct AxisCells { uint32_t c[2], o[2]; bool in[2]; };
VR_HD AxisCells axis_cells(int32_t i0, int32_t i1, uint32_t extent_voxels, uint32_t log2_cell) {
    AxisCells a;
    const int32_t i[2] = { i0, i1 };
    const uint32_t mask = (1u << log2_cell) - 1u;
#pragma unroll
    for (int t = 0; t < 2; ++t) {
        a.in[t] = i[t] >= 0 && (uint32_t)i[t] < extent_voxels;
        a.c[t] = a.in[t] ? (uint32_t)i[t] >> log2_cell : 0u;
        a.o[t] = a.in[t] ? (uint32_t)i[t] & mask : 0u;
    }
    return a;
}
struct TriIO { TapAddr a[8]; TapData d[8]; float fx, fy, fz; uint32_t in_mask; };
template <int DENSE = 2, bool GUARD = true>
VR_HD void trilinear_prep(const GridView& g, v3 ipos, TriIO& io) {
    const float qx = ipos.x - 0.5f, qy = ipos.y - 0.5f, qz = ipos.z - 0.5f;
    const float flx = floor_(qx), fly = floor_(qy), flz = floor_(qz);
    io.fx = qx - flx; io.fy = qy - fly; io.fz = qz - flz;
    const int32_t ix0 = voxel_index(flx, 0), ix1 = voxel_index(flx, 1);
    const int32_t ix = GUARD ? nan_guard(ix0, flx, fly, flz) : ix0, iy = voxel_index(fly, 0), iz = voxel_index(flz, 0);
    const int32_t x1 = GUARD ? nan_guard(ix1, flx, fly, flz) : ix1, y1 = voxel_index(fly, 1), z1 = voxel_index(flz, 1);
    const bool dense = grid_is_dense<DENSE>(g);
    const uint32_t lg = dense ? 2u : 3u;
    const AxisCells X = axis_cells(ix, x1, dense ? (uint32_t)g.dim[0] : (uint32_t)g.nb[0] << 3, lg);
    const AxisCells Y = axis_cells(iy, y1, dense ? (uint32_t)g.dim[1] : (uint32_t)g.nb[1] << 3, lg);
    const AxisCells Z = axis_cells(iz, z1, dense ? (uint32_t)g.dim[2] : (uint32_t)g.nb[2] << 3, lg);
    io.in_mask = 0u;
#pragma unroll
    for (int k = 0; k < 2; ++k)
#pragma unroll
        for (int j = 0; j < 2; ++j) {
            const uint32_t row = dense ? (mul24(Z.c[k], (uint32_t)g.dblk[1]) + Y.c[j]) * (uint32_t)g.dblk[0]
                                       : mul24(mul24(Z.c[k], (uint32_t)g.nb[1]) + Y.c[j], (uint32_t)g.nb[0]);
#pragma unroll
            for (int i = 0; i < 2; ++i) {
                TapAddr& a = io.a[4 * k + 2 * j + i];
                a.cell = row + X.c[i];
                a.off = dense ? ((Z.o[k] << 4) | (Y.o[j] << 2) | X.o[i]) : ((Z.o[k] << 6) | (Y.o[j] << 3) | X.o[i]);
                a.in = true;
                io.in_mask |= (X.in[i] & Y.in[j] & Z.in[k]) ? 1u << (4 * k + 2 * j + i) : 0u;
            }
        }
}
template <int DENSE = 2, int PAIR = 0>
VR_HD void trilinear_load(const GridView& g, TriIO& io) {
    if (!grid_is_dense<DENSE>(g) && g.atlas_f32) {
#pragma unroll
        for (int n = 0; n < 8; ++n) { io.d[n].rmin = 0.0f; io.d[n].rdiff = 0.0f; io.d[n].raw = f2u(g.atlas_f32[(size_t)io.a[n].cell * 512u + io.a[n].off]); }
        return;
    }
#pragma unroll
    for (int n = 0; n < 8; ++n) io.d[n] = tap_load<DENSE, PAIR>(g, io.a[n]);
}
VR_HD void trilinear_idle(TriIO& io) {
#pragma unroll
    for (int n = 0; n < 8; ++n) { io.a[n].cell = 0u; io.a[n].off = 0u; io.a[n].in = false; }
    io.fx = io.fy = io.fz = 0.0f; io.in_mask = 0u;
}
template <int DENSE = 2>
VR_HD float trilinear_value(const GridView& g, const TriIO& io) {
    float v[8];
    if (!grid_is_dense<DENSE>(g) && g.atlas_f32) {
#pragma unroll
        for (int n = 0; n < 8; ++n) v[n] = ((io.in_mask >> n) & 1u) ? u2f(io.d[n].raw) : 0.0f;
    } else {
#pragma unroll
        for (int n = 0; n < 8; ++n) v[n] = tap_value<DENSE>(g, io.d[n], (io.in_mask >> n) & 1u);
    }
    const float lx0 = mix_(v[0], v[1], io.fx);
    const float lx1 = mix_(v[2], v[3], io.fx);
    const float hx0 = mix_(v[4], v[5], io.fx);
    const float hx1 = mix_(v[6], v[7], io.fx);
    return mix_(mix_(lx0, lx1, io.fy), mix_(hx0, hx1, io.fy), io.fz);
}
template <int DENSE = 2>
VR_HD float density_trilinear_raw(const GridView& g, v3 ipos) {
    TriIO io;
    trilinear_prep<DENSE>(g, ipos, io);
    trilinear_load<DENSE>(g, io);
    return trilinear_value<DENSE>(g, io);
}

struct AxisWeights { float w2, s2, w3, s3, w4, s4, fl; };
VR_HD AxisWeights tricubic_axis_weights(float q) {
    AxisWeights a;
    const float fl = floor_(q);
    const float t = q - fl, t2 = t * t;
    const float k = 1.0f / 6.0f;
    float sum = k * (-t * t2 + 3.0f * t2 - 3.0f * t + 1.0f);
    a.w2 = k * (3.0f * t * t2 - 6.0f * t2 + 4.0f);
    sum = a.w2 + sum; a.s2 = max_(1e-3f, sum);
    a.w3 = k * (-3.0f * t * t2 + 3.0f * t2 + 3.0f * t + 1.0f);
    sum = a.w3 + sum; a.s3 = max_(1e-3f, sum);
    a.w4 = k * t * t2;
    sum = a.w4 + sum; a.s4 = max_(1e-3f, sum);
    a.fl = fl;
    return a;
}
struct LcgJump { uint32_t A, C; };
constexpr LcgJump lcg_jump(int j) {
    uint32_t A = 1u, C = 0u;
    for (int i = 0; i < j; ++i) { A = A * 1664525u; C = C * 1664525u + 1013904223u; }
    return LcgJump{ A, C };
}
#ifndef VR_TAP_ABS_BAND
#define VR_TAP_ABS_BAND 1
#endif
#ifndef VR_TAP_PRESHIFT
#define VR_TAP_PRESHIFT 1
#endif
#ifndef VR_TAP_CHAIN
#define VR_TAP_CHAIN 0
#endif
#if VR_TAP_ABS_BAND
struct AxisFast { float w2, s2, w3, s3, w4, fl; };
constexpr float kTapDrawScale = VR_TAP_PRESHIFT ? 256.0f : 1.0f;
constexpr float kTapScale = 16777216.0f * kTapDrawScale, kTapInvScale = 1.0f / kTapScale, kTapBand = 160.0f * kTapDrawScale;
VR_HD AxisFast tricubic_axis_fast(float q) {
    AxisFast a;
    a.fl = floor_(q);
    const float t = q - a.fl, t2 = t * t, u = 1.0f - t;
    a.w4 = (t2 * t) * kTapScale;
    a.w2 = fma_(fma_(3.0f * kTapScale, t, -6.0f * kTapScale), t2, 4.0f * kTapScale);
    a.w3 = fma_(fma_(fma_(-3.0f * kTapScale, t, 3.0f * kTapScale), t, 3.0f * kTapScale), t, kTapScale);
    a.s2 = fma_(a.w2, kTapInvScale, (u * u) * u);
    a.s3 = fma_(a.w3, kTapInvScale, a.s2);
    return a;
}
VR_HD void tricubic_fast_test(float k, float w, float s, bool& yes, bool& no) {
    const float x = fma_(k, s, -w);
    yes = x < -kTapBand;
    no = x > kTapBand;
}
#else
struct AxisFast { float w2, s2, w3, s3, w4, fl; };
VR_HD AxisFast tricubic_axis_fast(float q) {
    AxisFast a;
    a.fl = floor_(q);
    const float t = q - a.fl, t2 = t * t, u = 1.0f - t;
    a.w4 = t2 * t;
    a.w2 = fma_(fma_(3.0f, t, -6.0f), t2, 4.0f);
    a.w3 = fma_(fma_(fma_(-3.0f, t, 3.0f), t, 3.0f), t, 1.0f);
    a.s2 = (u * u) * u + a.w2;
    a.s3 = a.s2 + a.w3;
    return a;
}
constexpr float kTapLo = 16777152.0f;
constexpr float kTapHi = 16777280.0f;
VR_HD void tricubic_fast_test(float k, float w, float s, bool& yes, bool& no) {
    const float x = k * s;
    yes = x < fma_(w, kTapLo, -1e-20f);
    no = x > fma_(w, kTapHi, 1e-20f);
}
#endif
#ifndef VR_TAP_FAST
#if defined(__HIP_DEVICE_COMPILE__)
#define VR_TAP_FAST 1
#else
#define VR_TAP_FAST 0
#endif
#endif

template <bool FAST, bool GUARD = true>
VR_HD void tricubic_tap_t(v3 ipos, uint32_t& seed, int32_t& tx, int32_t& ty, int32_t& tz) {
    int32_t jx = 0, jy = 0, jz = 0;
    float flx, fly, flz;
#if VR_FAST_DEVICE
    const AxisWeights ax = tricubic_axis_weights(ipos.x - 0.5f);
    const AxisWeights ay = tricubic_axis_weights(ipos.y - 0.5f);
    const AxisWeights az = tricubic_axis_weights(ipos.z - 0.5f);
    flx = ax.fl; fly = ay.fl; flz = az.fl;
    {
        const uint32_t lo24 = seed & 0x00FFFFFFu;
#define VR_TAPF(J, V, W, S, N) do { \
            constexpr LcgJump g_ = lcg_jump(N); \
            const float k_ = (float)((mul24(lo24, g_.A & 0x00FFFFFFu) + g_.C) & 0x00FFFFFFu); \
            J = k_ * (S) < (W) * 16777216.0f ? V : J; \
        } while (0)
        VR_TAPF(jx, 1, ax.w2, ax.s2, 1); VR_TAPF(jy, 1, ay.w2, ay.s2, 2); VR_TAPF(jz, 1, az.w2, az.s2, 3);
        VR_TAPF(jx, 2, ax.w3, ax.s3, 4); VR_TAPF(jy, 2, ay.w3, ay.s3, 5); VR_TAPF(jz, 2, az.w3, az.s3, 6);
        VR_TAPF(jx, 3, ax.w4, ax.s4, 7); VR_TAPF(jy, 3, ay.w4, ay.s4, 8); VR_TAPF(jz, 3, az.w4, az.s4, 9);
#undef VR_TAPF
        rng_skip9(seed);
    }
#else
    bool exact = true;
    if constexpr (FAST) {
        const AxisFast fx = tricubic_axis_fast(ipos.x - 0.5f), fy = tricubic_axis_fast(ipos.y - 0.5f), fz = tricubic_axis_fast(ipos.z - 0.5f);
        flx = fx.fl; fly = fy.fl; flz = fz.fl;
        const uint32_t seed0 = seed;
#if VR_TAP_ABS_BAND && VR_TAP_PRESHIFT
        const uint32_t sh8 = seed << 8;
        float amin = __builtin_inff();
#if VR_TAP_CHAIN
        uint32_t st_ = sh8;
#if defined(__HIP_DEVICE_COMPILE__)
#define VR_TAP_KEEP(X) asm("" : "+v"(X))
#else
#define VR_TAP_KEEP(X) do { } while (0)
#endif
#define VR_TAP(J, V, W, S, N) do { \
            st_ = st_ * 1664525u + (1013904223u << 8); \
            VR_TAP_KEEP(st_); \
            const float x_ = fma_((float)st_, S, -(W));      \
            J = x_ < -kTapBand ? V : J; \
// ... 286 lines not shown
    const v3 tmin = v3{ min_(lo.x, hi.x), min_(lo.y, hi.y), min_(lo.z, hi.z) };
    const v3 tmax = v3{ max_(lo.x, hi.x), max_(lo.y, hi.y), max_(lo.z, hi.z) };
    tnear = max_(0.0f, max_(tmin.x, max_(tmin.y, tmin.z)));
    tfar = min_(tmax.x, min_(tmax.y, tmax.z));
    return tnear <= tfar;
}

#ifndef VR_DDA_INT_DIM
#define VR_DDA_INT_DIM 1
#endif
template <bool CLEAN = false>
VR_HD float step_dda(v3 p, v3 ri, int32_t mip) {
#if VR_DDA_INT_DIM
    const float dim = u2f((uint32_t)(130 + mip) << 23);
#else
    const float dim = (float)(8 << mip);
#endif
    const float idim = u2f((uint32_t)(124 - mip) << 23);
    const float ox = ri.x >= 0.0f ? dim + 0.5f : -0.5f;
    const float oy = ri.y >= 0.0f ? dim + 0.5f : -0.5f;
    const float oz = ri.z >= 0.0f ? dim + 0.5f : -0.5f;
    const float tx = (floor_(p.x * idim) * dim + ox - p.x) * ri.x;
    const float ty = (floor_(p.y * idim) * dim + oy - p.y) * ri.y;
    const float tz = (floor_(p.z * idim) * dim + oz - p.z) * ri.z;
    if (CLEAN) return __builtin_fminf(tx, __builtin_fminf(ty, tz));
    return min_(tx, min_(ty, tz));
}


VR_HD void hot_init(Hot& h) {
    h.seed = 0u; h.item = 0u;
    h.ipos = h.idir = h.ri = h.ethr = h.eL = h.shle = h.wpos = h.wdir = v3{ 0, 0, 0 };
    h.t = h.far = h.tau = h.majorant = h.Tr = 0.0f;
    h.mipq = 0;
    h.shadow = 0;
    h.state = ST_NEW;
    h.first = 0;
    h.maj_idx = -2; h.maj_raw = 0u;
}

#ifndef VR_SAMPLE_NT
#define VR_SAMPLE_NT 1
#endif
VR_HD void write_sample(const WorkUnit& wu, uint32_t item, v3 L, uint32_t n_paths) {
    float* o = wu.out + 4u * (size_t)item;
#if defined(__HIP_DEVICE_COMPILE__) && VR_SAMPLE_NT
    typedef float vr_f4 __attribute__((ext_vector_type(4)));
    __builtin_nontemporal_store(vr_f4{ L.x, L.y, L.z, n_paths > 0u ? 1.0f : 0.0f }, reinterpret_cast<vr_f4*>(o));
#elif defined(__HIP_DEVICE_COMPILE__)
    *reinterpret_cast<float4*>(o) = make_float4(L.x, L.y, L.z, n_paths > 0u ? 1.0f : 0.0f);
#else
    o[0] = L.x; o[1] = L.y; o[2] = L.z; o[3] = n_paths > 0u ? 1.0f : 0.0f;
#endif
}

VR_HD void accumulate_sample(float acc[4], const float L[4], int32_t current_sample) {
    const float a = 1.0f / (float)current_sample;
    acc[0] = mix_(acc[0], sanitize(L[0]), a);
    acc[1] = mix_(acc[1], sanitize(L[1]), a);
    acc[2] = mix_(acc[2], sanitize(L[2]), a);
    acc[3] = mix_(acc[3], sanitize(L[3]), a);
}

template <class K>
VR_HD bool begin_segment(Hot& h, const SceneParams& P, v3 pos, v3 d, int32_t shadow) {
    h.wpos = pos; h.wdir = d;
    h.shadow = shadow;
    h.Tr = 1.0f;
    h.mipq = 12;
    float tnear, tfar;
    if (!intersect_box(pos, d, P.u.vol_bb_min, P.u.vol_bb_max, tnear, tfar)) {
        h.state = segment_end_state(shadow);
        return false;
    }
    h.ipos = mat4_point(P.u.vol_density_inv_transform, pos);
    h.idir = mat4_dir(P.u.vol_density_inv_transform, d);
    h.far = tfar;
    if (K::global == 2 ? P.u.integrator != 0 : K::global == 1) {
        h.ri = v3{ 0, 0, 0 };
        h.tau = 0.0f;
        if (VR_CLEAN_FLAG) h.far = -tfar;
        h.t = tnear + neg_log_1m(rng(h.seed)) * P.u.vol_inv_majorant;
        if (h.t < tfar) { h.majorant = P.u.vol_majorant; h.state = ST_COLLIDE; }
        else h.state = segment_end_state(shadow);
        return true;
    }
    h.ri = rcp3_exact(h.idir);
    h.t = tnear + 1e-6f;
    h.tau = neg_log_1m(rng(h.seed));
    h.state = ST_MARCH;
#if VR_CLEAN_FLAG
    {
        const float ax = abs_(h.idir.x), ay = abs_(h.idir.y), az = abs_(h.idir.z), amax = __builtin_fmaxf(ax, __builtin_fmaxf(ay, az));
        const bool clean = (int)(abs_(h.ipos.x) < kCleanBound) & (int)(abs_(h.ipos.y) < kCleanBound) & (int)(abs_(h.ipos.z) < kCleanBound) &
                           (int)(ax * tfar < kCleanBound) & (int)(ay * tfar < kCleanBound) & (int)(az * tfar < kCleanBound) &
                           (int)(amax < kCleanBound) & (int)(amax >= 1.0f / kCleanBound);
        h.far = clean ? tfar : -tfar;
    }
#endif
    return true;
}

template <class K, class Cold, bool LAZY_EM = false>
VR_HD void do_new(Hot& h, Cold& c, const SceneParams& P, const WorkUnit& wu, uint32_t item) {
    const int32_t W = P.u.resolution[0], H = P.u.resolution[1];
    const int32_t px = wu.px0 + (int32_t)(item & 7u), py = wu.py0 + (int32_t)((item >> 3) & 7u);
    const int32_t smp = wu.first_sample + (int32_t)(item >> 6);
    if (px >= W || py >= H) return;
    h.seed = tea32((uint32_t)P.u.seed * (uint32_t)(py * W + px), (uint32_t)smp);
    const float jx = rng(h.seed), jy = rng(h.seed);
    const float fx = (((float)px + jx) - (float)W * 0.5f) / (float)H;
    const float fy = (((float)py + jy) - (float)H * 0.5f) / (float)H;
    const v3 dir = normalize(mat3_mul(P.u.cam_transform, normalize(v3{ fx, fy, P.cam_z })));
    const v3 pos = v3{ P.u.cam_pos[0], P.u.cam_pos[1], P.u.cam_pos[2] };
    const bool hit = begin_segment<K>(h, P, pos, dir, 0);
    const bool lazy = LAZY_EM || !hit || !(K::emission == 2 ? P.u.has_emission != 0 : K::emission == 1);
    if (!lazy) {
        st3(c, C_POS, pos); st3(c, C_DIR, dir);
        st3(c, C_L, v3{ 0, 0, 0 }); st3(c, C_THR, v3{ 1, 1, 1 });
        stu(c, C_NPATHS, 0u); c.st(C_FP, 0.0f); stu(c, C_ITEM, wu.base + item);
    }
    h.first = lazy ? 1 : 0;
    h.ipos = v3{ lazy ? dir.x : h.ipos.x, lazy ? dir.y : h.ipos.y, lazy ? dir.z : h.ipos.z };
    h.Tr = lazy ? u2f(wu.base + item) : h.Tr;
}
VR_HD void first_resume(Hot& h, const SceneParams& P) {
    h.ipos = mat4_point(P.u.vol_density_inv_transform, v3{ P.u.cam_pos[0], P.u.cam_pos[1], P.u.cam_pos[2] });
    h.Tr = 1.0f;
}

#ifndef VR_MARCH_STEPS
#define VR_MARCH_STEPS 2
#endif
constexpr int32_t kMarchSteps = VR_MARCH_STEPS;
#if VR_MARCH_STEPS == 2
struct MarchIO { float dt1, dt2, t1; uint32_t maj1, maj2; int32_t i1, i2; bool go1, go2; };
VR_HD void march_idle(MarchIO& io) { io.i1 = io.i2 = VR_MAJ_OUTSIDE_CELL ? 0 : -1; io.dt1 = io.dt2 = io.t1 = 0.0f; io.go1 = io.go2 = false; }
template <int DENSE = 2, int MAJB = 2, bool CLEAN = false>
VR_HD void march_prep(const Hot& h, const SceneParams& P, MarchIO& io) {
    const float far = seg_far(h);
    io.go1 = h.t < far;
    const v3 c1 = axpy(h.ipos, h.t, h.idir);
    const int32_t m1 = round_mip_q(h.mipq);
    io.i1 = majorant_index<DENSE, MAJB, CLEAN>(P.density, c1, m1);
    io.dt1 = step_dda<CLEAN>(c1, h.ri, m1);
    io.t1 = h.t + io.dt1;
    const int32_t q2 = h.mipq < 12 ? h.mipq + 1 : 12;
    const int32_t m2 = round_mip_q(q2);
    io.go2 = io.t1 < far;
    const v3 c2 = axpy(h.ipos, io.t1, h.idir);
    io.i2 = majorant_index<DENSE, MAJB, CLEAN>(P.density, c2, m2);
    io.dt2 = step_dda<CLEAN>(c2, h.ri, m2);
}
template <bool TF>
VR_HD void march_load(const SceneParams& P, MarchIO& io) {
    io.maj1 = majorant_fetch<TF>(P.density, io.i1);
    io.maj2 = majorant_fetch<TF>(P.density, io.i2);
}
template <bool TF>
VR_HD void march_load_reuse(const SceneParams& P, MarchIO& io, const Hot& h) {
    const bool same = io.i1 == h.maj_idx;
    const uint32_t m1 = majorant_fetch<TF>(P.density, same ? 0 : io.i1);
    io.maj1 = same ? h.maj_raw : m1;
    io.maj2 = majorant_fetch<TF>(P.density, io.i2);
}
template <bool TF, class T>
VR_HD uint32_t majorant_fetch_lds(const GridView& g, int32_t idx, const T* lds, int32_t first, bool all_resident) {
    const int32_t i = idx < 0 ? 0 : idx;
    const bool in_lds = i >= first;
    const T s = lds[in_lds ? i - first : 0];
    const uint32_t sv = TF ? f2u((float)s) : (uint32_t)s;
    if (all_resident) return sv;
    const uint32_t gv = majorant_fetch<TF>(g, in_lds ? 0 : i);
    return in_lds ? sv : gv;
}
template <bool TF, class T>
VR_HD void march_load_lds(const SceneParams& P, MarchIO& io, const T* lds, int32_t first) {
    const bool all_resident = first == 0;
    io.maj1 = majorant_fetch_lds<TF, T>(P.density, io.i1, lds, first, all_resident);
    io.maj2 = majorant_fetch_lds<TF, T>(P.density, io.i2, lds, first, all_resident);
}
template <bool TF, bool REUSE = false, bool CLEAN = false>
VR_HD void march_finish(Hot& h, const SceneParams& P, const MarchIO& io) {
    if (!io.go1) { h.state = segment_end_state(h.shadow); return; }
    float t = io.t1, maj = majorant_of<TF>(P, io.i1, io.maj1);
    float tau = h.tau - maj * io.dt1;
    int32_t q = h.mipq < 12 ? h.mipq + 1 : 12;
    if (REUSE) { const bool keep = VR_MAJ_OUTSIDE_CELL || io.i1 >= 0; h.maj_idx = keep ? io.i1 : h.maj_idx; h.maj_raw = keep ? io.maj1 : h.maj_raw; }
    if (tau > 0.0f) {
        if (!io.go2) { h.t = t; h.tau = tau; h.mipq = q; h.state = segment_end_state(h.shadow); return; }
        maj = majorant_of<TF>(P, io.i2, io.maj2);
        if (REUSE) { const bool keep = VR_MAJ_OUTSIDE_CELL || io.i2 >= 0; h.maj_idx = keep ? io.i2 : h.maj_idx; h.maj_raw = keep ? io.maj2 : h.maj_raw; }
        t = io.t1 + io.dt2;
        tau = tau - maj * io.dt2;
        q = q < 12 ? q + 1 : 12;
        if (tau > 0.0f) { h.t = t; h.tau = tau; h.mipq = q; return; }
    }
    t += (CLEAN && !TF) ? div_core(tau, maj) : tau / maj;
    h.t = t; h.tau = tau; h.mipq = q;
    if (t >= seg_far(h)) { h.state = segment_end_state(h.shadow); return; }
    h.majorant = maj;
    h.state = ST_COLLIDE;
}
#else
struct MarchIO {
    float dt[kMarchSteps], t[kMarchSteps];
    uint32_t maj[kMarchSteps];
    int32_t idx[kMarchSteps];
    bool go[kMarchSteps];
};
VR_HD void march_idle(MarchIO& io) {
#pragma unroll
    for (int k = 0; k < kMarchSteps; ++k) { io.idx[k] = VR_MAJ_OUTSIDE_CELL ? 0 : -1; io.dt[k] = io.t[k] = 0.0f; io.go[k] = false; }
}
template <int DENSE = 2, int MAJB = 2, bool CLEAN = false>
VR_HD void march_prep(const Hot& h, const SceneParams& P, MarchIO& io) {
    float t = h.t;
    int32_t q = h.mipq;
#pragma unroll
    for (int k = 0; k < kMarchSteps; ++k) {
        io.go[k] = t < seg_far(h);
        const v3 c = axpy(h.ipos, t, h.idir);
        const int32_t m = round_mip_q(q);
        io.idx[k] = majorant_index<DENSE, MAJB, CLEAN>(P.density, c, m);
        io.dt[k] = step_dda<CLEAN>(c, h.ri, m);
        t = t + io.dt[k];
        io.t[k] = t;
        q = q < 12 ? q + 1 : 12;
    }
}
template <bool TF>
VR_HD void march_load(const SceneParams& P, MarchIO& io) {
#pragma unroll
    for (int k = 0; k < kMarchSteps; ++k) io.maj[k] = majorant_fetch<TF>(P.density, io.idx[k]);
}
template <bool TF, class T>
VR_HD void march_load_lds(const SceneParams&, MarchIO&, const T*, int32_t) { static_assert(sizeof(T) == 0, "VR_MAJ_LDS is written for VR_MARCH_STEPS == 2"); }
template <bool TF>
VR_HD void march_load_reuse(const SceneParams& P, MarchIO& io, const Hot&) { march_load<TF>(P, io); }
template <bool TF, bool REUSE = false, bool CLEAN = false>
VR_HD void march_finish(Hot& h, const SceneParams& P, const MarchIO& io) {
    static_assert(!REUSE, "majorant reuse is written for VR_MARCH_STEPS == 2");
    float tau = h.tau, maj = 0.0f, t = h.t;
    int32_t q = h.mipq;
#pragma unroll
    for (int k = 0; k < kMarchSteps; ++k) {
        if (!io.go[k]) { h.t = t; h.tau = tau; h.mipq = q; h.state = segment_end_state(h.shadow); return; }
        maj = majorant_of<TF>(P, io.idx[k], io.maj[k]);
        t = io.t[k];
        tau = tau - maj * io.dt[k];
        q = q < 12 ? q + 1 : 12;
        if (!(tau > 0.0f)) goto tentative_collision;
    }
    h.t = t; h.tau = tau; h.mipq = q;
    return;
tentative_collision:
    t += (CLEAN && !TF) ? div_core(tau, maj) : tau / maj;
    h.t = t; h.tau = tau; h.mipq = q;
    if (t >= seg_far(h)) { h.state = segment_end_state(h.shadow); return; }
    h.majorant = maj;
    h.state = ST_COLLIDE;
}
#endif
template <bool TF, int DENSE = 2, int MAJB = 2>
VR_HD void do_march(Hot& h, const SceneParams& P) {
    if (!(h.t < seg_far(h))) { h.state = segment_end_state(h.shadow); return; }
    const v3 curr = axpy(h.ipos, h.t, h.idir);
    const int32_t m = round_mip_q(h.mipq);
    const float majorant = majorant_at<TF, DENSE, MAJB>(P, curr, m);
    const float dt = step_dda(curr, h.ri, m);
    h.t += dt;
    h.tau -= majorant * dt;
    h.mipq = h.mipq < 12 ? h.mipq + 1 : 12;
    if (h.tau > 0.0f) return;
    h.t += h.tau / majorant;
    if (h.t >= seg_far(h)) { h.state = segment_end_state(h.shadow); return; }
    h.majorant = majorant;
    h.state = ST_COLLIDE;
}

template <class K> struct CollideIO {
    TapAddr a; TapData d;
    TriIO tri;
    TapAddr ea; TapData ed;
};
template <class K, bool CLEAN = false>
VR_HD void collide_prep(Hot& h, const SceneParams& P, const SceneParams& PE, CollideIO<K>& io) {
    const v3 ip = axpy(h.ipos, h.t, h.idir);
    if (K::tf) {
        trilinear_prep<K::dense, !CLEAN>(P.density, ip, io.tri);
    } else {
        int32_t tx, ty, tz;
        tricubic_tap<!CLEAN>(ip, h.seed, tx, ty, tz);
        io.a = tap_addr<K::dense>(P.density, tx, ty, tz);
    }
    io.ea.cell = io.ea.off = 0u; io.ea.in = false;
    if (!h.shadow) {
        if (K::emission == 2 ? P.u.has_emission != 0 : K::emission == 1) {
            const v3 ie = mat4_point(PE.emission_from_density, ip);
            int32_t ex, ey, ez;
            tricubic_tap(ie, h.seed, ex, ey, ez);
            io.ea = tap_addr<K::edense>(PE.emission, ex, ey, ez);
        } else {
            rng_skip9(h.seed);
        }
    }
}
template <class K>
VR_HD void collide_idle(CollideIO<K>& io) {
    io.a.cell = io.a.off = 0u; io.a.in = false;
    io.ea.cell = io.ea.off = 0u; io.ea.in = false;
    if (K::tf) trilinear_idle(io.tri);
}
template <class K, bool CLEAN = false>
VR_HD void collide_prep(Hot& h, const SceneParams& P, CollideIO<K>& io) { collide_prep<K, CLEAN>(h, P, P, io); }
template <class K>
VR_HD void collide_load(const SceneParams& P, const SceneParams& PE, CollideIO<K>& io) {
    if (K::tf) trilinear_load<K::dense, K::pair_d>(P.density, io.tri);
    else io.d = tap_load<K::dense, K::pair_d>(P.density, io.a);
    if (K::emission == 2 ? P.u.has_emission != 0 : K::emission == 1) io.ed = tap_load<K::edense, K::pair_e>(PE.emission, io.ea);
}
template <class K>
VR_HD void collide_load(const SceneParams& P, CollideIO<K>& io) { collide_load<K>(P, P, io); }
template <class K, class Cold, bool CACHED = false>
VR_HD void collide_finish(Hot& h, Cold& c, const SceneParams& P, const SceneParams& PE, const CollideIO<K>& io, const float* tf_lut) {
    constexpr bool USE_TF = K::tf;
    const Uniforms& u = P.u;
    const bool global = K::global == 2 ? u.integrator != 0 : K::global == 1;
    float d;
    float rgba[4] = { 0, 0, 0, 0 };
    if (USE_TF) {
        tf_lookup_at(u, tf_lut, (u.vol_density_scale * trilinear_value<K::dense>(P.density, io.tri)) * u.vol_inv_majorant, rgba);
        d = u.vol_majorant * rgba[3];
    } else {
        d = u.vol_density_scale * tap_value<K::dense>(P.density, io.d, io.a.in);
    }
    if (!h.shadow) {
        const float P_real = d * u.vol_inv_majorant;
        if (K::emission == 2 ? u.has_emission != 0 : K::emission == 1) {
            const float tt = tap_value<K::edense>(PE.emission, io.ed, io.ea.in) * u.vol_emission_norm;
            const v3 e3 = v3{ tt, sqr(tt), sqr(sqr(tt)) };
            const v3 em = v3{ u.vol_emission_scale * sqr(e3.x), u.vol_emission_scale * sqr(e3.y), u.vol_emission_scale * sqr(e3.z) };
            const v3 oma = v3{ 1.0f - u.vol_albedo[0], 1.0f - u.vol_albedo[1], 1.0f - u.vol_albedo[2] };
            const v3 thr = CACHED ? h.ethr : ld3(c, C_THR);
            const v3 L0 = CACHED ? h.eL : ld3(c, C_L);
            const v3 L1 = global ? L0 + ((thr * oma) * em) * P_real : L0 + (((thr * oma) * em) * d) * u.vol_inv_majorant;
            if (CACHED) h.eL = L1; else st3(c, C_L, L1);
        }
        if (global ? rng(h.seed) < P_real : rng(h.seed) * h.majorant < d) {
            if (USE_TF) st3(c, C_COL, v3{ rgba[0], rgba[1], rgba[2] });
            h.state = ST_NEE;
            return;
        }
    } else if (global) {
        h.Tr *= 1.0f - d * u.vol_inv_majorant;
        if (h.Tr < 0.1f) {
            const float prob = 1.0f - h.Tr;
            if (rng(h.seed) < prob) { h.Tr = 0.0f; h.state = ST_POSTNEE; return; }
            h.Tr /= 1.0f - prob;
        }
    } else {
        if (rng(h.seed) * h.majorant < d) {
            const float ratio = (K::global == 0 && !K::tf) ? div_core(u.vol_majorant, h.majorant) : u.vol_majorant / h.majorant;
            h.Tr *= max_(0.0f, 1.0f - ratio);
            if (h.Tr < 0.1f) {
                const float prob = 1.0f - h.Tr;
                if (rng(h.seed) < prob) { h.Tr = 0.0f; h.state = ST_POSTNEE; return; }
                h.Tr /= 1.0f - prob;
            }
        }
    }
    if (global) {
        h.t = h.t + neg_log_1m(rng(h.seed)) * u.vol_inv_majorant;
        if (!(h.t < seg_far(h))) h.state = segment_end_state(h.shadow);
        return;
    }
    h.tau = neg_log_1m(rng(h.seed));
    h.mipq = h.mipq > 8 ? h.mipq - 8 : 0;
    h.state = ST_MARCH;
}
template <class K, class Cold, bool CACHED = false>
VR_HD void collide_finish(Hot& h, Cold& c, const SceneParams& P, const CollideIO<K>& io, const float* tf_lut) { collide_finish<K, Cold, CACHED>(h, c, P, P, io, tf_lut); }
template <class K, class Cold, bool CLEAN = false>
VR_HD void do_collide(Hot& h, Cold& c, const SceneParams& P) {
    CollideIO<K> io;
    collide_prep<K, CLEAN>(h, P, io);
    collide_load<K>(P, io);
    collide_finish<K>(h, c, P, io, P.tf_lut);
}

template <class K, class Cold, bool SHLE_IN_HOT = false, bool ITEM_IN_HOT = false, bool FIRST_L_IN_HOT = false>
VR_HD void do_nee(Hot& h, Cold& c, const Cold& crd, const SceneParams& P) {
    const bool first = h.first != 0;
    constexpr bool WS = world_slot<K>();
    if (!WS) {
        v3 dir = ld3(crd, C_DIR), pos0 = ld3(crd, C_POS), thr = ld3(crd, C_THR);
        h.first = 0;
        const float r0 = rng(h.seed), r1 = rng(h.seed);
        float pdf;
        v3 w_i, Le;
        sample_environment<K::global != 2, K::global != 2>(P, r0, r1, w_i, Le, pdf);
        dir = v3{ first ? h.ipos.x : dir.x, first ? h.ipos.y : dir.y, first ? h.ipos.z : dir.z };
        pos0 = v3{ first ? P.u.cam_pos[0] : pos0.x, first ? P.u.cam_pos[1] : pos0.y, first ? P.u.cam_pos[2] : pos0.z };
        thr = v3{ first ? 1.0f : thr.x, first ? 1.0f : thr.y, first ? 1.0f : thr.z };
        const v3 pos = axpy(pos0, h.t, dir);
        const v3 alb = v3{ P.u.vol_albedo[0], P.u.vol_albedo[1], P.u.vol_albedo[2] };
        if (K::global == 2 ? P.u.integrator != 0 : K::global == 1) thr = K::tf ? thr * (ld3(c, C_COL) * alb) : thr * alb;
        else { thr = thr * alb; if (K::tf) thr = thr * ld3(c, C_COL); }
        if (first) {
            st3(c, C_L, FIRST_L_IN_HOT ? h.eL : v3{ 0, 0, 0 }); stu(c, C_NPATHS, 0u);
            st3(c, C_DIR, dir);
            c.st(C_FP, 0.0f);
            if (!ITEM_IN_HOT) stu(c, C_ITEM, f2u(h.Tr));
        }
        const bool lit = pdf > 0.0f;
        const float f_p = phase_hg(dot(-dir, w_i), P.u.vol_phase_g);
        st3(c, C_POS, pos); c.st(C_SHPDF, lit ? pdf : 0.0f);
        st3(c, C_THR, thr); c.st(C_FPL, lit ? f_p : 0.0f);
        if (lit) {
            if (SHLE_IN_HOT) h.shle = Le; else st3(c, C_SHLE, Le);
            begin_segment<K>(h, P, pos, w_i, 1);
        } else {
            h.shadow = 0;
            h.state = ST_POSTNEE;
        }
        return;
    }
    v3 dir, pos0, thr;
    if (WS) {
        dir = h.wdir; pos0 = h.wpos; thr = v3{ 1.0f, 1.0f, 1.0f };
    } else {
        dir = ld3(crd, C_DIR); pos0 = ld3(crd, C_POS); thr = ld3(crd, C_THR);
        dir = v3{ first ? h.ipos.x : dir.x, first ? h.ipos.y : dir.y, first ? h.ipos.z : dir.z };
        pos0 = v3{ first ? P.u.cam_pos[0] : pos0.x, first ? P.u.cam_pos[1] : pos0.y, first ? P.u.cam_pos[2] : pos0.z };
        thr = v3{ first ? 1.0f : thr.x, first ? 1.0f : thr.y, first ? 1.0f : thr.z };
    }
    const v3 pos = axpy(pos0, h.t, dir);
    if (WS) {
        if (first) st3(c, C_THR, thr);
    } else
    {
        const v3 alb = v3{ P.u.vol_albedo[0], P.u.vol_albedo[1], P.u.vol_albedo[2] };
        if (K::global == 2 ? P.u.integrator != 0 : K::global == 1) thr = K::tf ? thr * (ld3(c, C_COL) * alb) : thr * alb;
        else { thr = thr * alb; if (K::tf) thr = thr * ld3(c, C_COL); }
    }
    if (first) {
        st3(c, C_L, FIRST_L_IN_HOT ? h.eL : v3{ 0, 0, 0 }); stu(c, C_NPATHS, 0u);
        if (!WS) st3(c, C_DIR, dir);
        c.st(C_FP, 0.0f);
        if (!ITEM_IN_HOT) stu(c, C_ITEM, f2u(h.Tr));
    }
    h.first = 0;
    const float r0 = rng(h.seed), r1 = rng(h.seed);
    float pdf;
    v3 w_i, Le;
    sample_environment<K::global != 2, K::global != 2>(P, r0, r1, w_i, Le, pdf);
    if (WS) {
        const bool lit = pdf > 0.0f;
        st3(c, C_DIR, dir); c.st(C_SHPDF, lit ? pdf : 0.0f);
        if (lit) {
            if (SHLE_IN_HOT) h.shle = Le; else st3(c, C_SHLE, Le);
            begin_segment<K>(h, P, pos, w_i, 1);
        } else {
            h.wpos = pos;
            h.shadow = 0;
            h.state = ST_POSTNEE;
        }
        return;
    }
    const bool lit = pdf > 0.0f;
    const float f_p = phase_hg(dot(-dir, w_i), P.u.vol_phase_g);
    st3(c, C_POS, pos); c.st(C_SHPDF, lit ? pdf : 0.0f);
    st3(c, C_THR, thr); c.st(C_FPL, lit ? f_p : 0.0f);
    if (lit) {
        if (SHLE_IN_HOT) h.shle = Le; else st3(c, C_SHLE, Le);
        begin_segment<K>(h, P, pos, w_i, 1);
    } else {
        h.shadow = 0;
        h.state = ST_POSTNEE;
    }
}

template <class K, class Cold, bool SHLE_IN_HOT = false, bool ITEM_IN_HOT = false>
VR_HD void do_postnee(Hot& h, Cold& c, const SceneParams& P, const WorkUnit& wu) {
    constexpr bool WS = world_slot<K>();
    const Quad q_l = ld4(c, C_L, C_NPATHS), q_p = WS ? Quad{ h.wpos, 0.0f } : ld4(c, C_POS, C_SHPDF);
    const Quad q_t = ld4(c, C_THR, WS ? C_FP : C_FPL), q_d = ld4(c, C_DIR, WS ? C_SHPDF : C_FP);
    v3 L = q_l.a;
    const float sh_pdf = WS ? q_d.b : q_p.b;
    v3 thr = q_t.a;
    if (WS) thr = thr * v3{ P.u.vol_albedo[0], P.u.vol_albedo[1], P.u.vol_albedo[2] };
    const float fpl_kept = WS ? 0.0f : q_t.b;
    if (sh_pdf > 0.0f) {
        const float f_p = WS ? phase_hg(dot(-q_d.a, h.wdir), P.u.vol_phase_g) : fpl_kept;
        const float mis = P.u.show_environment > 0 ? power_heuristic(sh_pdf, f_p) : 1.0f;
        L = L + ((((thr * mis) * f_p) * h.Tr) * (SHLE_IN_HOT ? h.shle : ld3(c, C_SHLE))) / sh_pdf;
    }
    const uint32_t n_paths = f2u(q_l.b) + 1u;
    if (n_paths >= (uint32_t)P.u.bounces) { write_sample(wu, ITEM_IN_HOT ? h.item : ldu(c, C_ITEM), L, n_paths); h.state = ST_NEW; return; }
    const float rr = luma(thr);
    if (rr < 0.1f) {
        const float prob = 1.0f - rr;
        if (rng(h.seed) < prob) { write_sample(wu, ITEM_IN_HOT ? h.item : ldu(c, C_ITEM), L, n_paths); h.state = ST_NEW; return; }
        thr = thr / (1.0f - prob);
        if (!WS) { st3(c, C_THR, thr); c.st(C_FPL, fpl_kept); }
    }
    const v3 dir = q_d.a;
    const float s0 = rng(h.seed), s1 = rng(h.seed);
    const v3 sd = sample_phase_hg(dir, P.u.vol_phase_g, s0, s1);
    const float f_p_next = phase_hg(dot(-dir, sd), P.u.vol_phase_g);
    if (WS) {
        st3(c, C_L, L); stu(c, C_NPATHS, n_paths);
        st3(c, C_THR, thr); c.st(C_FP, f_p_next);
    } else {
        st3(c, C_L, L); stu(c, C_NPATHS, n_paths);
        st3(c, C_DIR, sd); c.st(C_FP, f_p_next);
    }
    begin_segment<K>(h, P, q_p.a, sd, 0);
}

template <class Cold, bool ITEM_IN_HOT = false, bool FIRST_L_IN_HOT = false, bool WS = false>
VR_HD void do_escape(Hot& h, const Cold& c, const SceneParams& P, const WorkUnit& wu) {
    const bool first = h.first != 0;
    v3 L = ld3(c, C_L), thr = ld3(c, C_THR), dir = ld3(c, C_DIR);
    uint32_t n_paths = ldu(c, C_NPATHS), item = ITEM_IN_HOT ? h.item : ldu(c, C_ITEM);
    const float f_p = c.ld(C_FP);
    v3 Le_early = v3{ 0.0f, 0.0f, 0.0f };
    if (WS && P.u.show_environment > 0) Le_early = lookup_environment(P, h.wdir);
    const v3 L_first = FIRST_L_IN_HOT ? h.eL : v3{ 0.0f, 0.0f, 0.0f };
    L = v3{ first ? L_first.x : L.x, first ? L_first.y : L.y, first ? L_first.z : L.z };
    thr = v3{ first ? 1.0f : thr.x, first ? 1.0f : thr.y, first ? 1.0f : thr.z };
    if (WS) dir = h.wdir;
    else dir = v3{ first ? h.ipos.x : dir.x, first ? h.ipos.y : dir.y, first ? h.ipos.z : dir.z };
    n_paths = first ? 0u : n_paths;
    item = first ? f2u(h.Tr) : item;
    h.first = 0;
    if (P.u.show_environment > 0) {
        const v3 Le = WS ? Le_early : lookup_environment(P, dir);
        float mis = 1.0f;
        if (n_paths > 0u) {
            const float avg_w = env_average_importance(P);
            const float pdf_env = (luma(Le) / avg_w) * kInv4Pi;
            mis = power_heuristic(f_p, pdf_env);
        }
        L = L + (thr * mis) * Le;
    }
    write_sample(wu, item, L, n_paths);
    h.state = ST_NEW;
}

VR_HD void dvr_sample(const SceneParams& P, int32_t px, int32_t py, int32_t smp, float out[4]) {
    const Uniforms& u = P.u;
    const int32_t W = u.resolution[0], H = u.resolution[1];
    uint32_t seed = tea32((uint32_t)u.seed * (uint32_t)(py * W + px), (uint32_t)smp);
    const float jx = rng(seed), jy = rng(seed);
    const float fx = (((float)px + jx) - (float)W * 0.5f) / (float)H;
    const float fy = (((float)py + jy) - (float)H * 0.5f) / (float)H;
    const v3 dir = normalize(mat3_mul(u.cam_transform, normalize(v3{ fx, fy, P.cam_z })));
    const v3 pos = v3{ u.cam_pos[0], u.cam_pos[1], u.cam_pos[2] };
    v3 L = v3{ 0, 0, 0 };
    float tnear, tfar;
    if (!intersect_box(pos, dir, u.vol_bb_min, u.vol_bb_max, tnear, tfar)) {
        const v3 e = lookup_environment(P, dir);
        out[0] = e.x; out[1] = e.y; out[2] = e.z; out[3] = 0.0f;
        return;
    }
    const v3 ipos = mat4_point(u.vol_density_inv_transform, pos);
    const v3 idir = mat4_dir(u.vol_density_inv_transform, dir);
    const float dt = (tfar - tnear) / 64.0f;
    tnear += rng(seed) * dt;
    float Tr = 1.0f;
    for (int32_t i = 0; i < 64; ++i) {
        float rgba[4];
        const v3 ip = axpy(ipos, min_(tnear + (float)i * dt, tfar), idir);
        tf_lookup(P, (u.vol_density_scale * density_trilinear_raw(P.density, ip)) * u.vol_inv_majorant, rgba);
        const float dtau = rgba[3] * u.vol_majorant * dt;
        L = L + (v3{ rgba[0], rgba[1], rgba[2] } * dtau) * Tr;
        Tr *= exp_(-dtau);
        if (Tr <= 1e-6f) { out[0] = L.x; out[1] = L.y; out[2] = L.z; out[3] = 1.0f - Tr; return; }
    }
    const v3 e = lookup_environment(P, dir);
    L = L + e * Tr;
    out[0] = L.x; out[1] = L.y; out[2] = L.z; out[3] = 1.0f - Tr;
}

enum FeatureResult : int32_t { FEAT_MISS = 0, FEAT_HIT = 1, FEAT_LOST = 2 };
constexpr uint32_t kFeatureMaxSteps = 1u << 20;
struct FeatureCold {
    float v[C_COUNT];
    VR_HD float ld(int32_t f) const { return v[f]; }
    VR_HD void st(int32_t f, float x) { v[f] = x; }
};
template <bool TF>
VR_HD int32_t feature_sample(const SceneParams& P, int32_t px, int32_t py, int32_t smp, float& t, v3& albedo, v3& normal) {
    using K = TraceCfg<TF, 0, 2, 2, 2>;
    const Uniforms& u = P.u;
    const int32_t W = u.resolution[0], H = u.resolution[1];
    Hot h;
    hot_init(h);
    h.seed = tea32((uint32_t)u.seed * (uint32_t)(py * W + px), (uint32_t)smp);
    const float jx = rng(h.seed), jy = rng(h.seed);
    const float fx = (((float)px + jx) - (float)W * 0.5f) / (float)H;
    const float fy = (((float)py + jy) - (float)H * 0.5f) / (float)H;
    const v3 dir = normalize(mat3_mul(u.cam_transform, normalize(v3{ fx, fy, P.cam_z })));
    const v3 pos = v3{ u.cam_pos[0], u.cam_pos[1], u.cam_pos[2] };
    if (!begin_segment<K>(h, P, pos, dir, 0)) return FEAT_MISS;
    FeatureCold c;
    for (int32_t i = 0; i < C_COUNT; ++i) c.v[i] = 0.0f;
    for (uint32_t steps = 0u; h.state == ST_MARCH || h.state == ST_COLLIDE; ++steps) {
        if (steps >= kFeatureMaxSteps) return FEAT_LOST;
        if (h.state == ST_MARCH) {
            const float t0 = h.t, tau0 = h.tau;
            const int32_t mip0 = h.mipq;
            do_march<TF, 2, 2>(h, P);
            if (h.state == ST_MARCH && h.t == t0 && h.tau == tau0 && h.mipq == mip0) return FEAT_MISS;
        } else {
            do_collide<K, FeatureCold, false>(h, c, P);
        }
    }
    if (h.state != ST_NEE) return FEAT_MISS;
    t = h.t;
    albedo = v3{ u.vol_albedo[0], u.vol_albedo[1], u.vol_albedo[2] };
    if (TF) albedo = albedo * ld3(c, C_COL);
    const v3 ip = axpy(h.ipos, h.t, h.idir);
    const v3 g = v3{ density_trilinear_raw(P.density, v3{ ip.x + 1.0f, ip.y, ip.z }) - density_trilinear_raw(P.density, v3{ ip.x - 1.0f, ip.y, ip.z }),
                     density_trilinear_raw(P.density, v3{ ip.x, ip.y + 1.0f, ip.z }) - density_trilinear_raw(P.density, v3{ ip.x, ip.y - 1.0f, ip.z }),
                     density_trilinear_raw(P.density, v3{ ip.x, ip.y, ip.z + 1.0f }) - density_trilinear_raw(P.density, v3{ ip.x, ip.y, ip.z - 1.0f }) };
    const float* m = u.vol_density_inv_transform;
    const v3 n = v3{ (m[0] * g.x + m[1] * g.y) + m[2] * g.z, (m[4] * g.x + m[5] * g.y) + m[6] * g.z, (m[8] * g.x + m[9] * g.y) + m[10] * g.z };
    normal = (n.x == 0.0f && n.y == 0.0f && n.z == 0.0f) ? v3{ 0, 0, 0 } : -normalize(n);
    return FEAT_HIT;
}
template <bool TF>
VR_HD bool feature_pixel(const SceneParams& P, int32_t px, int32_t py, int32_t spp, float out[8]) {
    int32_t hits = 0;
    v3 sa = v3{ 0, 0, 0 }, sn = v3{ 0, 0, 0 };
    float sd = 0.0f;
    bool ok = true;
    for (int32_t s = 1; s <= spp; ++s) {
        float t = 0.0f;
        v3 a, n;
        const int32_t r = feature_sample<TF>(P, px, py, s, t, a, n);
        if (r == FEAT_LOST) { ok = false; break; }
        if (r != FEAT_HIT) continue;
        ++hits;
        sa = sa + a; sn = sn + n; sd += t;
    }
    for (int32_t i = 0; i < 8; ++i) out[i] = 0.0f;
    if (hits == 0) return ok;
    const float fh = (float)hits;
    out[0] = sa.x / fh; out[1] = sa.y / fh; out[2] = sa.z / fh; out[3] = fh / (float)spp;
    out[4] = sn.x / fh; out[5] = sn.y / fh; out[6] = sn.z / fh; out[7] = sd / fh;
    return ok;
}

VR_HD float raymarch_density(const SceneParams& P, v3 ip, uint32_t& seed) {
    int32_t tx, ty, tz;
    tricubic_tap(ip, seed, tx, ty, tz);
    return P.u.vol_density_scale * brick_value<2>(P.density, tx, ty, tz);
}
VR_HD float transmittance_raymarch(const SceneParams& P, v3 wpos, v3 wdir, uint32_t& seed) {
    const Uniforms& u = P.u;
    float tnear, tfar;
    if (!intersect_box(wpos, wdir, u.vol_bb_min, u.vol_bb_max, tnear, tfar)) return 1.0f;
    const v3 ipos = mat4_point(u.vol_density_inv_transform, wpos);
    const v3 idir = mat4_dir(u.vol_density_inv_transform, wdir);
    const float dt = (tfar - tnear) / 64.0f;
    tnear += rng(seed) * dt;
    float tau = 0.0f;
    for (int32_t i = 0; i < 64; ++i) {
        const float d = raymarch_density(P, axpy(ipos, min_(tnear + (float)i * dt, tfar), idir), seed);
        if (u.use_tf) {
            float rgba[4];
            tf_lookup(P, d * u.vol_inv_majorant, rgba);
            tau += rgba[3] * u.vol_majorant * dt;
        } else {
            tau += d * dt;
        }
    }
    return exp_(-tau);
}
VR_HD bool sample_volume_raymarch(const SceneParams& P, v3 wpos, v3 wdir, float& t, v3& throughput, uint32_t& seed) {
    const Uniforms& u = P.u;
    float tnear, tfar;
    if (!intersect_box(wpos, wdir, u.vol_bb_min, u.vol_bb_max, tnear, tfar)) return false;
    const v3 ipos = mat4_point(u.vol_density_inv_transform, wpos);
    const v3 idir = mat4_dir(u.vol_density_inv_transform, wdir);
    const float tau_target = neg_log_1m(rng(seed));
    const float dt = (tfar - tnear) / 64.0f;
    tnear += rng(seed) * dt;
    float tau = 0.0f;
    for (int32_t i = 0; i < 64; ++i) {
        t = min_(tnear + (float)i * dt, tfar);
        const float d = raymarch_density(P, axpy(ipos, t, idir), seed);
        float rgba[4] = { 0, 0, 0, 0 };
        if (u.use_tf) {
            tf_lookup(P, d * u.vol_inv_majorant, rgba);
            tau += rgba[3] * u.vol_majorant * dt;
        } else {
            tau += d * dt;
        }
        if (tau >= tau_target) {
            const v3 alb = u.use_tf ? v3{ rgba[0] * u.vol_albedo[0], rgba[1] * u.vol_albedo[1], rgba[2] * u.vol_albedo[2] }
                                    : v3{ u.vol_albedo[0], u.vol_albedo[1], u.vol_albedo[2] };
            throughput = throughput * alb;
            return true;
        }
    }
    return false;
}
VR_HD void raymarch_path_sample(const SceneParams& P, int32_t px, int32_t py, int32_t smp, float out[4]) {
    const Uniforms& u = P.u;
    const int32_t W = u.resolution[0], H = u.resolution[1];
    uint32_t seed = tea32((uint32_t)u.seed * (uint32_t)(py * W + px), (uint32_t)smp);
    const float jx = rng(seed), jy = rng(seed);
    const float fx = (((float)px + jx) - (float)W * 0.5f) / (float)H;
    const float fy = (((float)py + jy) - (float)H * 0.5f) / (float)H;
    v3 dir = normalize(mat3_mul(u.cam_transform, normalize(v3{ fx, fy, P.cam_z })));
    v3 pos = v3{ u.cam_pos[0], u.cam_pos[1], u.cam_pos[2] };
    v3 L = v3{ 0, 0, 0 }, thr = v3{ 1, 1, 1 };
    bool free_path = true;
    uint32_t n_paths = 0u;
    float t = 0.0f, f_p = 0.0f;
    while (sample_volume_raymarch(P, pos, dir, t, thr, seed)) {
        pos = axpy(pos, t, dir);
        const float r0 = rng(seed), r1 = rng(seed);
        float pdf;
        v3 w_i, Le;
        sample_environment(P, r0, r1, w_i, Le, pdf);
        if (pdf > 0.0f) {
            f_p = phase_hg(dot(-dir, w_i), u.vol_phase_g);
            const float mis = u.show_environment > 0 ? power_heuristic(pdf, f_p) : 1.0f;
            const float Tr = transmittance_raymarch(P, pos, w_i, seed);
            L = L + ((((thr * mis) * f_p) * Tr) * Le) / pdf;
        }
        if (++n_paths >= (uint32_t)u.bounces) { free_path = false; break; }
        const float rr = luma(thr);
        if (rr < 0.1f) {
            const float prob = 1.0f - rr;
            if (rng(seed) < prob) { free_path = false; break; }
            thr = thr / (1.0f - prob);
        }
        const float s0 = rng(seed), s1 = rng(seed);
        const v3 sd = sample_phase_hg(dir, u.vol_phase_g, s0, s1);
        f_p = phase_hg(dot(-dir, sd), u.vol_phase_g);
        dir = sd;
    }
    if (free_path && u.show_environment > 0) {
        const v3 Le = lookup_environment(P, dir);
        float mis = 1.0f;
        if (n_paths > 0u) {
            const float avg_w = env_average_importance(P);
            mis = power_heuristic(f_p, (luma(Le) / avg_w) * kInv4Pi);
        }
        L = L + (thr * mis) * Le;
    }
    out[0] = L.x; out[1] = L.y; out[2] = L.z; out[3] = n_paths > 0u ? 1.0f : 0.0f;
}

template <class K, class Cold>
VR_HD void lane_step(Hot& h, Cold& c, const SceneParams& P, const WorkUnit& wu, uint32_t& next_item, FirstStash& stash) {
    if (h.first && (h.state == ST_NEE || h.state == ST_ESCAPE)) { h.ipos = stash.dir; h.Tr = u2f(stash.item); }
    switch (h.state) {
    case ST_NEW:
        if (next_item >= (uint32_t)wu.n_items) { h.state = ST_DONE; break; }
        do_new<K>(h, c, P, wu, next_item++);
        if (h.first) { stash.dir = h.ipos; stash.item = f2u(h.Tr); first_resume(h, P); }
        break;
    case ST_MARCH: { MarchIO io; if (seg_clean(h)) march_prep<K::dense, K::majb, true>(h, P, io); else march_prep<K::dense, K::majb, false>(h, P, io); march_load<K::tf>(P, io); if (seg_clean(h)) march_finish<K::tf, false, true>(h, P, io); else march_finish<K::tf, false, false>(h, P, io); break; }
    case ST_COLLIDE: if (seg_clean(h)) do_collide<K, Cold, true>(h, c, P); else do_collide<K, Cold, false>(h, c, P); break;
    case ST_NEE: do_nee<K>(h, c, c, P); break;
    case ST_POSTNEE: do_postnee<K>(h, c, P, wu); break;
    case ST_ESCAPE: do_escape<Cold, false, false, world_slot<K>()>(h, c, P, wu); break;
    default: break;
    }
}

}
```

### volren_amd/renderer.py

```python
import ctypes as C

import numpy as np

from . import _lib

_INT_FIELDS = ("sample", "sppx", "seed", "bounces", "show_environment", "tonemapping", "integrator", "grid_frame_counter",
               "sample_pool_mb", "gpu_encoder", "fast_math", "tf_float_atlas", "launch_target_ms", "order_tiles", "coalesce_trace", "majorant_layout",
               "variance", "denoise_iterations")
_FLOAT_FIELDS = {"tonemap_exposure": 1, "tonemap_gamma": 1, "albedo": 3, "phase": 1, "density_scale": 1,
                 "emission_scale": 1, "vol_clip_min": 3, "vol_clip_max": 3, "env_strength": 1, "env_transform": 9,
                 "tf_window_left": 1, "tf_window_width": 1, "cam_pos": 3, "cam_dir": 3, "cam_up": 3, "cam_fov": 1,
                 "volume_transform": 16, "denoise_sigma": 5, "denoise_alpha": 1}


def _f32(a):
    return np.ascontiguousarray(a, dtype=np.float32)


class Renderer:

    def __init__(self, width, height, device=0, _borrowed=None):
        object.__setattr__(self, "_h", None)
        L = _lib.load()
        object.__setattr__(self, "_owned", _borrowed is None)
        if _borrowed is None:
            h = C.c_void_p()
            _lib.check(L.vr_create(C.byref(h), int(device), int(width), int(height)))
        else:
            h = C.c_void_p(_borrowed)
        object.__setattr__(self, "_h", h)
        object.__setattr__(self, "_L", L)
        object.__setattr__(self, "width", int(width))
        object.__setattr__(self, "height", int(height))

    def close(self):
        if self._h is not None:
            if self._owned:
                self._L.vr_destroy(self._h)
            object.__setattr__(self, "_h", None)

    def __del__(self):
        try:
            self.close()
        except Exception:
            pass

    def get_int(self, name):
        v = C.c_int()
        _lib.check(self._L.vr_get_int(self._h, name.encode(), C.byref(v)))
        return v.value

    def __getattr__(self, name):
        if name in _INT_FIELDS or name in ("n_grid_frames", "last_launches", "pending_samples", "majorant_blocked", "env_div_safe", "env_compact", "kernel_variant", "kernel_variant_reason",
                                              "adaptive_rounds"):
            v = C.c_int()
            _lib.check(self._L.vr_get_int(self._h, name.encode(), C.byref(v)))
            return bool(v.value) if name in ("show_environment", "tonemapping") else v.value
        if name in _FLOAT_FIELDS:
            n = _FLOAT_FIELDS[name]
            buf = (C.c_float * n)()
            _lib.check(self._L.vr_get_float(self._h, name.encode(), buf, n))
            return buf[0] if n == 1 else np.array(buf[:], np.float32)
        raise AttributeError(name)

    def __setattr__(self, name, value):
        if name in _INT_FIELDS:
            _lib.check(self._L.vr_set_int(self._h, name.encode(), int(value)))
        elif name in _FLOAT_FIELDS or name == "env_rot":
            v = _f32(np.atleast_1d(value)).reshape(-1)
            _lib.check(self._L.vr_set_float(self._h, name.encode(), v.ctypes.data_as(C.POINTER(C.c_float)), v.size))
        else:
            object.__setattr__(self, name, value)

    def has_fast_math(self):
        return True

    def load_volume(self, path):
        _lib.check(self._L.vr_load_volume(self._h, str(path).encode()))

    def set_volume_path(self, path):
        _lib.check(self._L.vr_set_volume_path(self._h, str(path).encode()))

    def volume_aabb(self, name="density"):
        out = (C.c_float * 6)()
        _lib.check(self._L.vr_volume_aabb(self._h, name.encode(), out))
        return np.array(out[:3], np.float32), np.array(out[3:], np.float32)

    def volume_minorant_majorant(self, name="density"):
        out = (C.c_float * 2)()
        _lib.check(self._L.vr_volume_minorant_majorant(self._h, name.encode(), out))
        return float(out[0]), float(out[1])

    def load_envmap(self, path):
        _lib.check(self._L.vr_load_envmap(self._h, str(path).encode()))

    def load_transferfunc(self, path):
        _lib.check(self._L.vr_load_transferfunc(self._h, str(path).encode()))

    def set_volume_dense(self, voxels_zyx, transform=None, name="density", unit_cube=True, commit=True):
        v = _f32(voxels_zyx)
        nz, ny, nx = v.shape
        t = _f32(transform).reshape(16) if transform is not None else None
        _lib.check(self._L.vr_set_volume_dense(self._h, name.encode(), v.ctypes.data, nx, ny, nz,
                                               t.ctypes.data if t is not None else None, 1 if unit_cube else 0))
        if commit:
            self.commit()

    def volume_add_grid_frame(self, voxels_zyx, name="density", transform=None):
        v = _f32(voxels_zyx)
        nz, ny, nx = v.shape
        t = _f32(transform).reshape(16) if transform is not None else None
        _lib.check(self._L.vr_volume_add_grid_frame_dense(self._h, name.encode(), v.ctypes.data, nx, ny, nz, t.ctypes.data if t is not None else None))

    def volume_update_grid_frame(self, frame, voxels_zyx, name="density", transform=None):
        v = _f32(voxels_zyx)
        nz, ny, nx = v.shape
        t = _f32(transform).reshape(16) if transform is not None else None
        _lib.check(self._L.vr_volume_update_grid_frame_dense(self._h, int(frame), name.encode(), v.ctypes.data, nx, ny, nz, t.ctypes.data if t is not None else None))

    def volume_n_grid_frames(self):
        n = C.c_int()
        _lib.check(self._L.vr_volume_n_grid_frames(self._h, C.byref(n)))
        return n.value

    def set_volume_dense_f16(self, voxels_zyx, transform=None, name="density", unit_cube=True, commit=True):
        v = np.ascontiguousarray(voxels_zyx, dtype=np.float16)
        nz, ny, nx = v.shape
        t = _f32(transform).reshape(16) if transform is not None else None
        _lib.check(self._L.vr_set_volume_dense_f16(self._h, name.encode(), v.ctypes.data, nx, ny, nz,
                                                   t.ctypes.data if t is not None else None, 1 if unit_cube else 0))
        if commit:
            self.commit()

    def set_volume_brick(self, transform, n_bricks, min_maj, indirection, rng, atlas_dim, atlas, mips=(), name="density",
                         unit_cube=True, commit=True):
        t = _f32(transform).reshape(16)
        nb = np.asarray(n_bricks, np.uint32)
        mm = _f32(min_maj)
        ind = np.ascontiguousarray(indirection, np.uint32)
        rg = np.ascontiguousarray(rng, np.uint32)
        ad = np.asarray(atlas_dim, np.uint32)
        at = np.ascontiguousarray(atlas, np.uint8)
        mip_arrays = [np.ascontiguousarray(a, np.uint32) for _, a in mips]
        mip_ptrs = (C.c_void_p * max(1, len(mips)))(*[a.ctypes.data for a in mip_arrays])
        mip_dims = np.asarray([d for d, _ in mips], np.uint32).reshape(-1, 3) if mips else np.zeros((1, 3), np.uint32)
        _lib.check(self._L.vr_set_volume_brick(self._h, name.encode(), t.ctypes.data, nb.ctypes.data, mm.ctypes.data,
                                               ind.ctypes.data, rg.ctypes.data, ad.ctypes.data, at.ctypes.data,
                                               len(mips), C.cast(mip_ptrs, C.c_void_p), mip_dims.ctypes.data, 1 if unit_cube else 0))
        if commit:
            self.commit()

    def set_envmap(self, rgb_top_first):
        a = _f32(rgb_top_first)
        _lib.check(self._L.vr_set_envmap(self._h, a.ctypes.data, a.shape[1], a.shape[0]))

    def set_transferfunc(self, lut):
        if lut is None:
            _lib.check(self._L.vr_set_transferfunc(self._h, None, 0))
            return
        a = _f32(lut)
        _lib.check(self._L.vr_set_transferfunc(self._h, a.ctypes.data, a.shape[0]))

    def commit(self):
        _lib.check(self._L.vr_commit(self._h))

    def reset(self):
        _lib.check(self._L.vr_reset(self._h))

    def resize(self, w, h):
        _lib.check(self._L.vr_resize(self._h, int(w), int(h)))
        object.__setattr__(self, "width", int(w))
        object.__setattr__(self, "height", int(h))

    def scale_and_move_to_unit_cube(self):
        _lib.check(self._L.vr_scale_and_move_to_unit_cube(self._h))

    def trace(self):
        _lib.check(self._L.vr_trace(self._h))

    def flush(self):
        _lib.check(self._L.vr_flush(self._h))

    def render(self, spp=0, sync=True):
        _lib.check(self._L.vr_render(self._h, int(spp)))
        if sync:
            self.synchronize()

    def synchronize(self):
        _lib.check(self._L.vr_synchronize(self._h))

    def last_kernel_ms(self):
        ms = C.c_double()
        _lib.check(self._L.vr_last_kernel_ms(self._h, C.byref(ms)))
        return ms.value

    def last_pathtrace_ms(self):
        ms = C.c_double()
        _lib.check(self._L.vr_last_pathtrace_ms(self._h, C.byref(ms)))
        return ms.value

    def framebuffer(self):
        out = np.empty((self.height, self.width, 4), np.float32)
        _lib.check(self._L.vr_framebuffer(self._h, out.ctypes.data))
        return out

    def fbo_data(self):
# ... 218 lines not shown
```

Before: 5508 Msamples/s.

## Use 32-bit gather offsets for small grid tables and add wide-address kernel builds

Adds 32-bit offset addressing for majorant and atlas/dense table loads in variants 0 and 1, selected when every table is under 4 GiB. Larger tables, or a new wide_addressing setting, dispatch to new 64-bit builds. The aim is to cut 64-bit address arithmetic and VGPR pressure in the hot march and collide loads. It also adds a shadow-ray shortcut, on for non-fast builds, that ends transmittance at 0 on a real collision when the local majorant is within the global one, skipping ratio tracking there.

```diff
diff --git a/volren_amd/csrc/capi.cpp b/volren_amd/csrc/capi.cpp
--- a/volren_amd/csrc/capi.cpp
+++ b/volren_amd/csrc/capi.cpp
@@ -283,6 +283,7 @@
         else if (n == "coalesce_trace") { R.flush_pending(); R.coalesce_trace = v != 0; }
         else if (n == "majorant_layout") { if (v < -1 || v > 1) throw std::runtime_error("majorant_layout: -1 (per grid, chosen at commit), 0 (linear), 1 (4x4x4-cell blocks)"); R.majorant_layout = v; }
         else if (n == "tf_float_atlas") R.tf_float_atlas = v != 0;
+        else if (n == "wide_addressing") { if (v < 0 || v > 1) throw std::runtime_error("wide_addressing: 0 (by the tables' sizes), 1 (always the kernels with 64-bit gather addresses)"); R.tuning.wide_addressing = v; }
         else if (n == "gpu_encoder") R.gpu_encoder = v != 0;
         else if (n == "sample_pool_mb") { if (v < 16 || v > 65536) throw std::runtime_error("sample_pool_mb must be in [16, 65536] (item indices of a sub-launch are 32-bit: < 2^32 RGBA32F items)"); R.sample_pool_bytes = (size_t)v << 20; }
         else if (n == "launch_target_ms") { if (v < 0) throw std::runtime_error("launch_target_ms must be >= 0 (0 = no sizing by time)"); R.launch_target_ms = v; }
@@ -319,6 +320,11 @@
             vr::SceneParams P; R.fill_params(P);
             int why = 0; const int variant = vr::pathtrace_variant_of(P, &why);
             *v = n == "kernel_variant" ? variant : why;
+        }
+        else if (n == "wide_addressing") *v = R.tuning.wide_addressing;
+        else if (n == "kernel_wide") {
+            vr::SceneParams P; R.fill_params(P);
+            *v = (vr::pathtrace_wide_of(R.tuning, P) || vr::pathtrace_variant_of(P, nullptr) >= 2) ? 1 : 0;
         }
         else if (n == "env_div_safe") *v = R.environment && R.environment->cdf_div_safe ? 1 : 0;
         else if (n == "env_compact") *v = R.environment && R.environment->envmap_rgbe ? 1 : 0;
diff --git a/volren_amd/csrc/renderer.cpp b/volren_amd/csrc/renderer.cpp
--- a/volren_amd/csrc/renderer.cpp
+++ b/volren_amd/csrc/renderer.cpp
@@ -475,7 +475,7 @@
 bool RendererHIP::LaunchInputs::same_launch_as(const LaunchInputs& o) const {
     return memcmp(&P, &o.P, sizeof P) == 0 && frame == o.frame && maj.density_scale == o.maj.density_scale && maj.tf_version == o.maj.tf_version &&
            maj.wl == o.maj.wl && maj.ww == o.maj.ww && maj.blocked == o.maj.blocked && memcmp(tuning.thr, o.tuning.thr, sizeof tuning.thr) == 0 && tuning.stats == o.tuning.stats &&
-           tuning.samples_per_unit == o.tuning.samples_per_unit && tuning.blocks_per_cu == o.tuning.blocks_per_cu && order_tiles == o.order_tiles &&
+           tuning.samples_per_unit == o.tuning.samples_per_unit && tuning.blocks_per_cu == o.tuning.blocks_per_cu && tuning.wide_addressing == o.tuning.wide_addressing && order_tiles == o.order_tiles &&
            launch_target_ms == o.launch_target_ms && fast_math == o.fast_math && variance == o.variance && sample_pool_bytes == o.sample_pool_bytes && stream == o.stream;
 }
 
diff --git a/volren_amd/csrc/vr_device.h b/volren_amd/csrc/vr_device.h
--- a/volren_amd/csrc/vr_device.h
+++ b/volren_amd/csrc/vr_device.h
@@ -15,6 +15,7 @@
     unsigned long long* stats = nullptr;
     int32_t samples_per_unit = 0;
     int32_t blocks_per_cu = 0;
+    int32_t wide_addressing = 0;
 };
 PathtraceTuning default_tuning();
 size_t pathtrace_pool_floats(const PathtraceTuning& T, int32_t n_tiles, int32_t n_samples);
@@ -32,6 +33,7 @@
     VR_VARIANT_GRID_FORMS = 8
 };
 int pathtrace_variant_of(const SceneParams& P, int* why);
+bool pathtrace_wide_of(const PathtraceTuning& T, const SceneParams& P);
 void launch_denoise_prepare(const float* moments, const float* features, int32_t W, int32_t H, int32_t n, float vscale, const int32_t* counts, float* v, float* guide,
                             hipStream_t stream);
 void launch_denoise_atrous(const float* cin, const float* vin, const float* guide, int32_t W, int32_t H, int32_t step, const DenoiseSigma& sg,
diff --git a/volren_amd/csrc/vr_launch.hip b/volren_amd/csrc/vr_launch.hip
--- a/volren_amd/csrc/vr_launch.hip
+++ b/volren_amd/csrc/vr_launch.hip
@@ -108,14 +108,19 @@
     int vr_pt_occupancy_##N(int tf, int stats); \
     void vr_pt_launch_##N(int tf, int stats, unsigned grid, hipStream_t stream, const void* P, float* sbuf, float* cold_ws, const void* D, const void* S, uint32_t* status, unsigned long long* stats_buf);
 VR_PT_DECL(0) VR_PT_DECL(1) VR_PT_DECL(2) VR_PT_DECL(3) VR_PT_DECL(4) VR_PT_DECL(0_fast) VR_PT_DECL(1_fast) VR_PT_DECL(2_fast) VR_PT_DECL(3_fast) VR_PT_DECL(4_fast)
+VR_PT_DECL(0w) VR_PT_DECL(1w) VR_PT_DECL(0w_fast) VR_PT_DECL(1w_fast)
 #undef VR_PT_DECL
 }
 typedef int (*PtOccupancy)(int, int);
 typedef void (*PtLaunch)(int, int, unsigned, hipStream_t, const void*, float*, float*, const void*, const void*, uint32_t*, unsigned long long*);
-static const PtOccupancy kPtOccupancy[2][kPtVariants] = { { vr_pt_occupancy_0, vr_pt_occupancy_1, vr_pt_occupancy_2, vr_pt_occupancy_3, vr_pt_occupancy_4 },
-                                                          { vr_pt_occupancy_0_fast, vr_pt_occupancy_1_fast, vr_pt_occupancy_2_fast, vr_pt_occupancy_3_fast, vr_pt_occupancy_4_fast } };
-static const PtLaunch kPtLaunch[2][kPtVariants] = { { vr_pt_launch_0, vr_pt_launch_1, vr_pt_launch_2, vr_pt_launch_3, vr_pt_launch_4 },
-                                                    { vr_pt_launch_0_fast, vr_pt_launch_1_fast, vr_pt_launch_2_fast, vr_pt_launch_3_fast, vr_pt_launch_4_fast } };
+static const PtOccupancy kPtOccupancy[2][2][kPtVariants] = { { { vr_pt_occupancy_0, vr_pt_occupancy_1, vr_pt_occupancy_2, vr_pt_occupancy_3, vr_pt_occupancy_4 },
+                                                               { vr_pt_occupancy_0w, vr_pt_occupancy_1w, vr_pt_occupancy_2, vr_pt_occupancy_3, vr_pt_occupancy_4 } },
+                                                             { { vr_pt_occupancy_0_fast, vr_pt_occupancy_1_fast, vr_pt_occupancy_2_fast, vr_pt_occupancy_3_fast, vr_pt_occupancy_4_fast },
+                                                               { vr_pt_occupancy_0w_fast, vr_pt_occupancy_1w_fast, vr_pt_occupancy_2_fast, vr_pt_occupancy_3_fast, vr_pt_occupancy_4_fast } } };
+static const PtLaunch kPtLaunch[2][2][kPtVariants] = { { { vr_pt_launch_0, vr_pt_launch_1, vr_pt_launch_2, vr_pt_launch_3, vr_pt_launch_4 },
+                                                         { vr_pt_launch_0w, vr_pt_launch_1w, vr_pt_launch_2, vr_pt_launch_3, vr_pt_launch_4 } },
+                                                       { { vr_pt_launch_0_fast, vr_pt_launch_1_fast, vr_pt_launch_2_fast, vr_pt_launch_3_fast, vr_pt_launch_4_fast },
+                                                         { vr_pt_launch_0w_fast, vr_pt_launch_1w_fast, vr_pt_launch_2_fast, vr_pt_launch_3_fast, vr_pt_launch_4_fast } } };
 
 int pathtrace_variant_of(const SceneParams& P, int* why) {
     const bool scale_ok = P.u.vol_density_scale >= 1.0f / 65536.0f && P.u.vol_density_scale <= 16777216.0f;
@@ -133,6 +138,12 @@
     if (why) *why = reason;
     return variant;
 }
+bool pathtrace_wide_of(const PathtraceTuning& T, const SceneParams& P) {
+    if (T.wide_addressing) return true;
+    uint64_t m = grid_largest_table_bytes(P.density, P.paired != 0, P.u.use_tf != 0);
+    if (P.u.has_emission) m = std::max(m, grid_largest_table_bytes(P.emission, P.paired != 0, false));
+    return m >= (1ull << 32);
+}
 static int pathtrace_variant(const SceneParams& P) {
     int why = 0;
     const int variant = pathtrace_variant_of(P, &why);
@@ -147,19 +158,19 @@
     return variant;
 }
 
-static int resident_blocks(const PathtraceTuning& T, int mode, int variant, bool tf, bool stats) {
+static int resident_blocks(const PathtraceTuning& T, int mode, int wide, int variant, bool tf, bool stats) {
     int dev = 0, cus = 0;
     if (hipGetDevice(&dev) != hipSuccess) return 1024;
     static std::mutex mu;
     static std::map<uint32_t, std::pair<int, int>> cache;
-    const uint32_t key = ((uint32_t)dev << 8) | ((uint32_t)mode << 5) | ((uint32_t)variant << 2) | (tf ? 2u : 0u) | (stats ? 1u : 0u);
+    const uint32_t key = ((uint32_t)dev << 8) | ((uint32_t)wide << 6) | ((uint32_t)mode << 5) | ((uint32_t)variant << 2) | (tf ? 2u : 0u) | (stats ? 1u : 0u);
     std::pair<int, int> v;
     {
         std::lock_guard<std::mutex> lock(mu);
         auto it = cache.find(key);
         if (it == cache.end()) {
             if (hipDeviceGetAttribute(&cus, hipDeviceAttributeMultiprocessorCount, dev) != hipSuccess || cus <= 0) cus = 256;
-            it = cache.emplace(key, std::make_pair(cus, kPtOccupancy[mode][variant](tf, stats))).first;
+            it = cache.emplace(key, std::make_pair(cus, kPtOccupancy[mode][wide][variant](tf, stats))).first;
         }
         v = it->second;
     }
@@ -189,8 +200,8 @@
     S.max_iters = kMaxIdleIters;
     if (S.thr[ST_COLLIDE] <= 0) S.thr[ST_COLLIDE] = (P.u.use_tf || P.u.has_emission) ? 32 : 24;
     const bool tf = P.u.use_tf != 0, stats = T.stats != nullptr;
-    const int mode = fast_math ? 1 : 0;
-    const int blocks = resident_blocks(T, mode, variant, tf, stats);
+    const int mode = fast_math ? 1 : 0, wide = pathtrace_wide_of(T, P) ? 1 : 0;
+    const int blocks = resident_blocks(T, mode, wide, variant, tf, stats);
     const uint32_t groups_needed = (D.n_units + (uint32_t)kWgWaves - 1u) / (uint32_t)kWgWaves;
     const dim3 grid((unsigned)std::min<uint32_t>((uint32_t)blocks, groups_needed > 0 ? groups_needed : 1u)), block(256);
     if (P.u.integrator == 3 || (P.u.integrator == 2 && P.u.use_tf)) {
@@ -200,7 +211,7 @@
     } else {
         (void)hipMemsetAsync(unit_counter, 0, kQueueSegments * sizeof(uint32_t), stream);
         if (ev_kernel_begin) (void)hipEventRecord(ev_kernel_begin, stream);
-        kPtLaunch[mode][variant](tf, stats, grid.x, stream, &P, sample_pool, workspace, &D, &S, status, T.stats);
+        kPtLaunch[mode][wide][variant](tf, stats, grid.x, stream, &P, sample_pool, workspace, &D, &S, status, T.stats);
         if (ev_kernel_end) (void)hipEventRecord(ev_kernel_end, stream);
     }
     const auto accumulate = moments ? accumulate_kernel<true> : accumulate_kernel<false>;
diff --git a/volren_amd/csrc/vr_pathtrace.h b/volren_amd/csrc/vr_pathtrace.h
--- a/volren_amd/csrc/vr_pathtrace.h
+++ b/volren_amd/csrc/vr_pathtrace.h
@@ -587,9 +587,9 @@
             else {
             march_idle(mio);
             if (is_m) march_prep<K::dense, K::majb, CLEAN>(l, P, mio);
-            if constexpr (kMajCells > 0) march_load_lds<K::tf, MajT>(P, mio, lds_maj, maj_first);
-            else if constexpr (K::maj_reuse) march_load_reuse<K::tf>(P, mio, l);
-            else march_load<K::tf>(P, mio);
+            if constexpr (kMajCells > 0) march_load_lds<K::tf, MajT, K::a32>(P, mio, lds_maj, maj_first);
+            else if constexpr (K::maj_reuse) march_load_reuse<K::tf, K::a32>(P, mio, l);
+            else march_load<K::tf, K::a32>(P, mio);
 #if VR_MARCH_LOADS_PINNED
             asm volatile("" : "+v"(mio.maj1), "+v"(mio.maj2));
 #endif
@@ -635,7 +635,7 @@
                     ls.mipq = spec ? (l.mipq > 8 ? l.mipq - 8 : 0) : l.mipq;
                     march_idle(pre);
                     if (slot >= 0 && (l.state == ST_MARCH || spec)) march_prep<K::dense, K::majb, CLEAN>(ls, P, pre);
-                    march_load<K::tf>(P, pre);
+                    march_load<K::tf, K::a32>(P, pre);
                     if (VR_EARLY_MARCH == 1) asm volatile("" : "+v"(cio.d.raw), "+v"(cio.d.rmin), "+v"(cio.d.rdiff));
                 }
                 if (run_c) {
diff --git a/volren_amd/csrc/vr_pathtrace.hip b/volren_amd/csrc/vr_pathtrace.hip
--- a/volren_amd/csrc/vr_pathtrace.hip
+++ b/volren_amd/csrc/vr_pathtrace.hip
@@ -9,6 +9,16 @@
 #define VR_PT_SUFFIX _fast
 #else
 #define VR_PT_SUFFIX
+#endif
+#if defined(VR_PT_WIDE) && VR_PT_WIDE
+#if VR_PT_VARIANT >= 2
+#error "variants 2, 3 and 4 have no wide build: they always form 64-bit addresses"
+#endif
+#define VR_PT_WIDTH w
+#define VR_PT_A32 false
+#else
+#define VR_PT_WIDTH
+#define VR_PT_A32 (VR_PT_VARIANT < 2)
 #endif
 
 #if VR_PT_VARIANT == 3 && !defined(VR_BATCH_REGS)
@@ -25,15 +35,15 @@
 namespace vr {
 
 #if VR_PT_VARIANT == 0
-template <bool TF> using Cfg = TraceCfg<TF, 0, 0, 0>;
+template <bool TF> using Cfg = TraceCfg<TF, 0, 0, 0, 0, VR_PT_A32>;
 #elif VR_PT_VARIANT == 1
-template <bool TF> using Cfg = TraceCfg<TF, 0, 0, 1>;
+template <bool TF> using Cfg = TraceCfg<TF, 0, 0, 1, 0, VR_PT_A32>;
 #elif VR_PT_VARIANT == 2
-template <bool TF> using Cfg = TraceCfg<TF, 0, 1, 0>;
+template <bool TF> using Cfg = TraceCfg<TF, 0, 1, 0, 0, VR_PT_A32>;
 #elif VR_PT_VARIANT == 4
-template <bool TF> using Cfg = TraceCfg<TF, 0, 1, 0, 1>;
+template <bool TF> using Cfg = TraceCfg<TF, 0, 1, 0, 1, VR_PT_A32>;
 #else
-template <bool TF> using Cfg = TraceCfg<TF, 2, 2, 2, 2>;
+template <bool TF> using Cfg = TraceCfg<TF, 2, 2, 2, 2, false>;
 #endif
 
 typedef void (*PtKernel)(const KernelArgs);
@@ -44,8 +54,9 @@
 
 }
 
-#define VR_PT_CAT3(a, b, c) a##b##c
-#define VR_PT_CAT(a, b, c) VR_PT_CAT3(a, b, c)
+#define VR_PT_CAT4(a, b, c, d) a##b##c##d
+#define VR_PT_CAT5(a, b, c, d) VR_PT_CAT4(a, b, c, d)
+#define VR_PT_CAT(a, b, c) VR_PT_CAT5(a, b, VR_PT_WIDTH, c)
 
 extern "C" int VR_PT_CAT(vr_pt_occupancy_, VR_PT_VARIANT, VR_PT_SUFFIX)(int tf, int stats) {
     int per_cu = 0;
diff --git a/volren_amd/csrc/vr_scene.h b/volren_amd/csrc/vr_scene.h
--- a/volren_amd/csrc/vr_scene.h
+++ b/volren_amd/csrc/vr_scene.h
@@ -92,6 +92,18 @@
     int32_t dblk[2];
 };
 
+VR_SCENE_HD uint64_t grid_largest_table_bytes(const GridView& g, bool paired, bool tf) {
+    uint64_t m = (uint64_t)majorant_table_cells((uint32_t)(g.mshift[0] + g.mshift[1] + g.mshift[2])) * (tf ? 4u : 2u);
+    uint64_t a;
+    if (g.dense) a = (uint64_t)g.dblk[0] * (uint64_t)g.dblk[1] * (uint64_t)((g.dim[2] + 3) / 4) * 128u;
+    else {
+        const uint64_t records = (uint64_t)g.nb[0] * (uint64_t)g.nb[1] * (uint64_t)g.nb[2];
+        a = records * (paired ? kPairBlockBytes : kBrickBlockBytes);
+        if (g.atlas_f32 && records * 2048u > a) a = records * 2048u;
+    }
+    return a > m ? a : m;
+}
+
 struct Uniforms {
     int32_t bounces, seed, show_environment;
     float cam_pos[3], cam_fov, cam_transform[9];
diff --git a/volren_amd/csrc/vr_trace.h b/volren_amd/csrc/vr_trace.h
--- a/volren_amd/csrc/vr_trace.h
+++ b/volren_amd/csrc/vr_trace.h
@@ -33,9 +33,9 @@
 #ifndef VR_MAJ_REUSE
 #define VR_MAJ_REUSE 0
 #endif
-template <bool TF, int GLOBAL, int EMISSION, int DENSE, int MAJB = 0>
+template <bool TF, int GLOBAL, int EMISSION, int DENSE, int MAJB = 0, bool A32 = true>
 struct TraceCfg {
-    static constexpr bool tf = TF;
+    static constexpr bool tf = TF, a32 = A32;
     static constexpr int global = GLOBAL, emission = EMISSION, dense = DENSE, majb = MAJB;
     static constexpr int edense = EMISSION == 1 ? DENSE : 2;
     static constexpr int pair_d = (VR_PAIRED_ATLAS && EMISSION == 1 && DENSE == 0) ? 1 : 0, pair_e = pair_d ? 2 : 0;
@@ -119,6 +119,16 @@
 
 template <int DENSE>
 VR_HD bool grid_is_dense(const GridView& g) { return DENSE == 2 ? g.dense != nullptr : DENSE == 1; }
+template <bool A32, class T>
+VR_HD T table_load(const T* base, uint32_t i) {
+    if (A32) return *reinterpret_cast<const T*>(reinterpret_cast<const char*>(base) + (uint32_t)(i * (uint32_t)sizeof(T)));
+    return base[(size_t)i];
+}
+template <bool A32, class T>
+VR_HD T line_load(const uint8_t* base, uint32_t line, uint32_t byte) {
+    if (A32) return *reinterpret_cast<const T*>(base + (uint32_t)((line << 7) + byte));
+    return *reinterpret_cast<const T*>(base + ((size_t)line << 7) + byte);
+}
 struct TapAddr { uint32_t cell, off; bool in; };
 struct TapData { float rmin, rdiff; uint32_t raw; };
 template <int DENSE = 2>
@@ -144,10 +154,27 @@
 #ifndef VR_TAP_LINE_INDEX
 #define VR_TAP_LINE_INDEX 1
 #endif
-template <int DENSE = 2, int PAIR = 0>
+#if VR_TAP_LINE_INDEX && VR_BRICK_HEADERS && !defined(VR_TAP_NT) && !defined(VR_DENSE_TAP_NT)
+#define VR_TAP_A32(A32) (A32)
+#else
+#define VR_TAP_A32(A32) false
+#endif
+template <int DENSE = 2, int PAIR = 0, bool A32 = false>
 VR_HD TapData tap_load(const GridView& g, TapAddr a) {
     TapData d;
     VR_TRACE(1, g.atlas ? (const void*)g.atlas : (const void*)g.dense, a.cell, a.off);
+    static_assert(!(A32 && PAIR != 0), "the kernels that read a paired atlas form 64-bit addresses (vr_pathtrace.hip)");
+    if (VR_TAP_A32(A32)) {
+        if (grid_is_dense<DENSE>(g)) {
+            d.rmin = 0.0f; d.rdiff = 0.0f;
+            d.raw = table_load<true>(g.dense, a.cell * 64u + a.off);
+        } else {
+            const uint32_t line = brick_voxel_line(a.off), ln = a.cell * (kBrickBlockBytes / 128u) + line;
+            d.rmin = line_load<true, float>(g.atlas, ln, 0u); d.rdiff = line_load<true, float>(g.atlas, ln, 4u);
+            d.raw = line_load<true, uint8_t>(g.atlas, ln, kBrickLineHeader + a.off - line * kBrickLineVoxels);
+        }
+        return d;
+    }
     if (PAIR != 0) {
         const uint32_t line = pair_voxel_line(a.off);
 #if VR_TAP_LINE_INDEX
@@ -244,14 +271,14 @@
     const uint32_t bx = (uint32_t)(int32_t)ipos.x >> sh, by = (uint32_t)(int32_t)ipos.y >> sh, bz = (uint32_t)(int32_t)ipos.z >> sh;
     return inside ? (int32_t)(off + majorant_cell_index(bx, by, bz, sx, sy, (uint32_t)mip, blocked)) : (VR_MAJ_OUTSIDE_CELL ? g.maj_outside : -1);
 }
-template <bool TF>
+template <bool TF, bool A32 = false>
 VR_HD uint32_t majorant_fetch(const GridView& g, int32_t idx) {
     const int32_t i = VR_MAJ_OUTSIDE_CELL ? idx : (idx < 0 ? 0 : idx);
 #if VR_MAJ_OUTSIDE_CELL && defined(__clang__)
     __builtin_assume(i >= 0);
 #endif
     VR_TRACE(0, g.majorant16, i, TF ? 4 : 2);
-    return TF ? f2u(g.majorant[i]) : (uint32_t)g.majorant16[i];
+    return TF ? f2u(table_load<A32>(g.majorant, (uint32_t)i)) : (uint32_t)table_load<A32>(g.majorant16, (uint32_t)i);
 }
 template <bool TF>
 VR_HD float majorant_value(const SceneParams& P, uint32_t raw) { return TF ? u2f(raw) : P.u.vol_density_scale * half2float(raw); }
@@ -317,15 +344,15 @@
             }
         }
 }
-template <int DENSE = 2, int PAIR = 0>
+template <int DENSE = 2, int PAIR = 0, bool A32 = false>
 VR_HD void trilinear_load(const GridView& g, TriIO& io) {
     if (!grid_is_dense<DENSE>(g) && g.atlas_f32) {
 #pragma unroll
-        for (int n = 0; n < 8; ++n) { io.d[n].rmin = 0.0f; io.d[n].rdiff = 0.0f; io.d[n].raw = f2u(g.atlas_f32[(size_t)io.a[n].cell * 512u + io.a[n].off]); }
+        for (int n = 0; n < 8; ++n) { io.d[n].rmin = 0.0f; io.d[n].rdiff = 0.0f; io.d[n].raw = f2u(A32 ? table_load<true>(g.atlas_f32, io.a[n].cell * 512u + io.a[n].off) : g.atlas_f32[(size_t)io.a[n].cell * 512u + io.a[n].off]); }
         return;
     }
 #pragma unroll
-    for (int n = 0; n < 8; ++n) io.d[n] = tap_load<DENSE, PAIR>(g, io.a[n]);
+    for (int n = 0; n < 8; ++n) io.d[n] = tap_load<DENSE, PAIR, A32>(g, io.a[n]);
 }
 VR_HD void trilinear_idle(TriIO& io) {
 #pragma unroll
@@ -918,33 +945,33 @@
     io.i2 = majorant_index<DENSE, MAJB, CLEAN>(P.density, c2, m2);
     io.dt2 = step_dda<CLEAN>(c2, h.ri, m2);
 }
-template <bool TF>
+template <bool TF, bool A32 = false>
 VR_HD void march_load(const SceneParams& P, MarchIO& io) {
-    io.maj1 = majorant_fetch<TF>(P.density, io.i1);
-    io.maj2 = majorant_fetch<TF>(P.density, io.i2);
-}
-template <bool TF>
+    io.maj1 = majorant_fetch<TF, A32>(P.density, io.i1);
+    io.maj2 = majorant_fetch<TF, A32>(P.density, io.i2);
+}
+template <bool TF, bool A32 = false>
 VR_HD void march_load_reuse(const SceneParams& P, MarchIO& io, const Hot& h) {
     const bool same = io.i1 == h.maj_idx;
-    const uint32_t m1 = majorant_fetch<TF>(P.density, same ? 0 : io.i1);
+    const uint32_t m1 = majorant_fetch<TF, A32>(P.density, same ? 0 : io.i1);
     io.maj1 = same ? h.maj_raw : m1;
-    io.maj2 = majorant_fetch<TF>(P.density, io.i2);
-}
-template <bool TF, class T>
+    io.maj2 = majorant_fetch<TF, A32>(P.density, io.i2);
+}
+template <bool TF, class T, bool A32 = false>
 VR_HD uint32_t majorant_fetch_lds(const GridView& g, int32_t idx, const T* lds, int32_t first, bool all_resident) {
     const int32_t i = idx < 0 ? 0 : idx;
     const bool in_lds = i >= first;
     const T s = lds[in_lds ? i - first : 0];
     const uint32_t sv = TF ? f2u((float)s) : (uint32_t)s;
     if (all_resident) return sv;
-    const uint32_t gv = majorant_fetch<TF>(g, in_lds ? 0 : i);
+    const uint32_t gv = majorant_fetch<TF, A32>(g, in_lds ? 0 : i);
     return in_lds ? sv : gv;
 }
-template <bool TF, class T>
+template <bool TF, class T, bool A32 = false>
 VR_HD void march_load_lds(const SceneParams& P, MarchIO& io, const T* lds, int32_t first) {
     const bool all_resident = first == 0;
-    io.maj1 = majorant_fetch_lds<TF, T>(P.density, io.i1, lds, first, all_resident);
-    io.maj2 = majorant_fetch_lds<TF, T>(P.density, io.i2, lds, first, all_resident);
+    io.maj1 = majorant_fetch_lds<TF, T, A32>(P.density, io.i1, lds, first, all_resident);
+    io.maj2 = majorant_fetch_lds<TF, T, A32>(P.density, io.i2, lds, first, all_resident);
 }
 template <bool TF, bool REUSE = false, bool CLEAN = false>
 VR_HD void march_finish(Hot& h, const SceneParams& P, const MarchIO& io) {
@@ -995,15 +1022,15 @@
         q = q < 12 ? q + 1 : 12;
     }
 }
-template <bool TF>
+template <bool TF, bool A32 = false>
 VR_HD void march_load(const SceneParams& P, MarchIO& io) {
 #pragma unroll
-    for (int k = 0; k < kMarchSteps; ++k) io.maj[k] = majorant_fetch<TF>(P.density, io.idx[k]);
-}
-template <bool TF, class T>
+    for (int k = 0; k < kMarchSteps; ++k) io.maj[k] = majorant_fetch<TF, A32>(P.density, io.idx[k]);
+}
+template <bool TF, class T, bool A32 = false>
 VR_HD void march_load_lds(const SceneParams&, MarchIO&, const T*, int32_t) { static_assert(sizeof(T) == 0, "VR_MAJ_LDS is written for VR_MARCH_STEPS == 2"); }
-template <bool TF>
-VR_HD void march_load_reuse(const SceneParams& P, MarchIO& io, const Hot&) { march_load<TF>(P, io); }
+template <bool TF, bool A32 = false>
+VR_HD void march_load_reuse(const SceneParams& P, MarchIO& io, const Hot&) { march_load<TF, A32>(P, io); }
 template <bool TF, bool REUSE = false, bool CLEAN = false>
 VR_HD void march_finish(Hot& h, const SceneParams& P, const MarchIO& io) {
     static_assert(!REUSE, "majorant reuse is written for VR_MARCH_STEPS == 2");
@@ -1082,12 +1109,15 @@
 VR_HD void collide_prep(Hot& h, const SceneParams& P, CollideIO<K>& io) { collide_prep<K, CLEAN>(h, P, P, io); }
 template <class K>
 VR_HD void collide_load(const SceneParams& P, const SceneParams& PE, CollideIO<K>& io) {
-    if (K::tf) trilinear_load<K::dense, K::pair_d>(P.density, io.tri);
-    else io.d = tap_load<K::dense, K::pair_d>(P.density, io.a);
-    if (K::emission == 2 ? P.u.has_emission != 0 : K::emission == 1) io.ed = tap_load<K::edense, K::pair_e>(PE.emission, io.ea);
+    if (K::tf) trilinear_load<K::dense, K::pair_d, K::a32>(P.density, io.tri);
+    else io.d = tap_load<K::dense, K::pair_d, K::a32>(P.density, io.a);
+    if (K::emission == 2 ? P.u.has_emission != 0 : K::emission == 1) io.ed = tap_load<K::edense, K::pair_e, K::a32>(PE.emission, io.ea);
 }
 template <class K>
 VR_HD void collide_load(const SceneParams& P, CollideIO<K>& io) { collide_load<K>(P, P, io); }
+#ifndef VR_SHADOW_BLOCKED_SHORTCUT
+#define VR_SHADOW_BLOCKED_SHORTCUT (!VR_FAST_DEVICE)
+#endif
 template <class K, class Cold, bool CACHED = false>
 VR_HD void collide_finish(Hot& h, Cold& c, const SceneParams& P, const SceneParams& PE, const CollideIO<K>& io, const float* tf_lut) {
     constexpr bool USE_TF = K::tf;
@@ -1127,6 +1157,14 @@
         }
     } else {
         if (rng(h.seed) * h.majorant < d) {
+#if VR_SHADOW_BLOCKED_SHORTCUT
+            if ((h.majorant > 0.0f) & (h.majorant <= u.vol_majorant) & (abs_(h.Tr) < inf_())) {
+                (void)rng(h.seed);
+                h.Tr = 0.0f;
+                h.state = ST_POSTNEE;
+                return;
+            }
+#endif
             const float ratio = (K::global == 0 && !K::tf) ? div_core(u.vol_majorant, h.majorant) : u.vol_majorant / h.majorant;
             h.Tr *= max_(0.0f, 1.0f - ratio);
             if (h.Tr < 0.1f) {
@@ -1359,7 +1397,7 @@
 };
 template <bool TF>
 VR_HD int32_t feature_sample(const SceneParams& P, int32_t px, int32_t py, int32_t smp, float& t, v3& albedo, v3& normal) {
-    using K = TraceCfg<TF, 0, 2, 2, 2>;
+    using K = TraceCfg<TF, 0, 2, 2, 2, false>;
     const Uniforms& u = P.u;
     const int32_t W = u.resolution[0], H = u.resolution[1];
     Hot h;
@@ -1533,7 +1571,7 @@
         do_new<K>(h, c, P, wu, next_item++);
         if (h.first) { stash.dir = h.ipos; stash.item = f2u(h.Tr); first_resume(h, P); }
         break;
-    case ST_MARCH: { MarchIO io; if (seg_clean(h)) march_prep<K::dense, K::majb, true>(h, P, io); else march_prep<K::dense, K::majb, false>(h, P, io); march_load<K::tf>(P, io); if (seg_clean(h)) march_finish<K::tf, false, true>(h, P, io); else march_finish<K::tf, false, false>(h, P, io); break; }
+    case ST_MARCH: { MarchIO io; if (seg_clean(h)) march_prep<K::dense, K::majb, true>(h, P, io); else march_prep<K::dense, K::majb, false>(h, P, io); march_load<K::tf, K::a32>(P, io); if (seg_clean(h)) march_finish<K::tf, false, true>(h, P, io); else march_finish<K::tf, false, false>(h, P, io); break; }
     case ST_COLLIDE: if (seg_clean(h)) do_collide<K, Cold, true>(h, c, P); else do_collide<K, Cold, false>(h, c, P); break;
     case ST_NEE: do_nee<K>(h, c, c, P); break;
     case ST_POSTNEE: do_postnee<K>(h, c, P, wu); break;
diff --git a/volren_amd/renderer.py b/volren_amd/renderer.py
--- a/volren_amd/renderer.py
+++ b/volren_amd/renderer.py
@@ -6,7 +6,7 @@
 
 _INT_FIELDS = ("sample", "sppx", "seed", "bounces", "show_environment", "tonemapping", "integrator", "grid_frame_counter",
                "sample_pool_mb", "gpu_encoder", "fast_math", "tf_float_atlas", "launch_target_ms", "order_tiles", "coalesce_trace", "majorant_layout",
-               "variance", "denoise_iterations")
+               "variance", "denoise_iterations", "wide_addressing")
 _FLOAT_FIELDS = {"tonemap_exposure": 1, "tonemap_gamma": 1, "albedo": 3, "phase": 1, "density_scale": 1,
                  "emission_scale": 1, "vol_clip_min": 3, "vol_clip_max": 3, "env_strength": 1, "env_transform": 9,
                  "tf_window_left": 1, "tf_window_width": 1, "cam_pos": 3, "cam_dir": 3, "cam_up": 3, "cam_fov": 1,
@@ -51,7 +51,7 @@
         return v.value
 
     def __getattr__(self, name):
-        if name in _INT_FIELDS or name in ("n_grid_frames", "last_launches", "pending_samples", "majorant_blocked", "env_div_safe", "env_compact", "kernel_variant", "kernel_variant_reason",
+        if name in _INT_FIELDS or name in ("n_grid_frames", "last_launches", "pending_samples", "majorant_blocked", "env_div_safe", "env_compact", "kernel_variant", "kernel_variant_reason", "kernel_wide",
                                               "adaptive_rounds"):
             v = C.c_int()
             _lib.check(self._L.vr_get_int(self._h, name.encode(), C.byref(v)))
```

After: 5644 Msamples/s (median of 6 runs). 2.5% higher.
